# jneem/nnnoiseless

Hardware: AMD Instinct MI355X
Metric: 480-sample frames/sec (whole node) at N concurrent streams (higher is better)
Workload: dtype f32; 1 GPU; configs[2]: 65536 concurrent streams on one GPU, built-in weights.rnn, GRU as batched MFMA GEMM, synthetic 48 kHz sine+noise, 48 frame(s) per stream per step; parity=oracle pinned by the reference's golden pair (built-in model), model=built-in weights.rnn, boundary_format=f32 planar (process_frame's own), streams_per_gpu=65536, streams_total=65536, inputs_ready=True, schedule=stages, lanes=2, parallelism=streams sharded x1, one process per GPU, no data-path collective

## Files before the change

### include/nnn_batch.h

```cpp
#ifndef NNN_BATCH_H
#define NNN_BATCH_H

#include <stddef.h>
#include <stdint.h>

#ifdef __cplusplus
extern "C" {
#endif

typedef struct nnn_batch nnn_batch;
#ifndef RNNOISE_H
typedef struct RNNModel RNNModel;
#endif

#define NNN_FRAME_SIZE 480

RNNModel *nnn_model_from_bytes(const uint8_t *bytes, size_t len);
RNNModel *nnn_model_default(void);
long nnn_convert_rnnoise_text(const char *text, size_t len, uint8_t *out, size_t cap);
RNNModel *nnn_model_from_rnnoise_text(const char *text, size_t len);
void nnn_model_free(RNNModel *m);
RNNModel *nnn_model_clone(const RNNModel *m);
void nnn_model_shape(const RNNModel *m, int32_t shape[12]);

nnn_batch *nnn_batch_create(const RNNModel *model, int n_streams, int device);
nnn_batch *nnn_batch_create_grouped(const RNNModel *const *models, const int *group_streams, int n_groups, int device);
typedef struct nnn_batch_opts {
    int max_group_frames;
    int reserved[7];
} nnn_batch_opts;
nnn_batch *nnn_batch_create_opts(const RNNModel *const *models, const int *group_streams, int n_groups, int device,
                                 const nnn_batch_opts *opts);
int nnn_batch_max_group_frames(const nnn_batch *b);
size_t nnn_batch_device_bytes(const nnn_batch *b);
void nnn_batch_destroy(nnn_batch *b);
int nnn_batch_num_streams(const nnn_batch *b);
int nnn_batch_reset(nnn_batch *b);

nnn_batch *nnn_batch_clone(nnn_batch *b);
size_t nnn_batch_state_bytes(const nnn_batch *b);
int nnn_batch_save_state(nnn_batch *b, void *host_dst, size_t dst_bytes);
int nnn_batch_load_state(nnn_batch *b, const void *host_src, size_t src_bytes);

#define NNN_STREAM_STATE_BYTES 11232
#define NNN_STREAM_STATE_VERSION 1
#define NNN_STREAM_STATE_MAGIC 0x3153534Eu
#define NNN_STREAM_STATE_OFF_MAGIC 0
#define NNN_STREAM_STATE_OFF_VERSION 4
#define NNN_STREAM_STATE_OFF_SIZE 8
#define NNN_STREAM_STATE_OFF_GRU_SIZES 12
#define NNN_STREAM_STATE_OFF_MEM_ID 24
#define NNN_STREAM_STATE_OFF_LAST_PERIOD 28
#define NNN_STREAM_STATE_OFF_LAST_GAIN 32
#define NNN_STREAM_STATE_OFF_MEM_HP_X 36
#define NNN_STREAM_STATE_OFF_INPUT_MEM 64
#define NNN_STREAM_STATE_OFF_SYNTHESIS_MEM 6976
#define NNN_STREAM_STATE_OFF_CEPSTRAL_MEM 8896
#define NNN_STREAM_STATE_OFF_LASTG 9600
#define NNN_STREAM_STATE_OFF_VAD_GRU 9696
#define NNN_STREAM_STATE_OFF_NOISE_GRU 10208
#define NNN_STREAM_STATE_OFF_DENOISE_GRU 10720
int nnn_batch_reset_streams(nnn_batch *b, const int *streams, int n);
int nnn_batch_export_streams(nnn_batch *b, const int *streams, int n, void *host_dst, size_t dst_bytes);
int nnn_batch_import_streams(nnn_batch *b, const int *streams, int n, const void *host_src, size_t src_bytes);
int nnn_batch_export_streams_device(nnn_batch *b, const int *streams, int n, void *d_dst, void *hip_stream);
int nnn_batch_import_streams_device(nnn_batch *b, const int *streams, int n, const void *d_src, void *hip_stream);

int nnn_batch_hold_streams(nnn_batch *b, const int *streams, int n);
int nnn_batch_resume_streams(nnn_batch *b, const int *streams, int n);
int nnn_batch_num_held(const nnn_batch *b);
int nnn_batch_held_mask(const nnn_batch *b, uint8_t *held, size_t n);

int nnn_batch_set_gain_floor(nnn_batch *b, const int *streams, int n, const float *floors, int bands);
int nnn_batch_get_gain_floor(nnn_batch *b, const int *streams, int n, float *floors );
int nnn_batch_num_floored(const nnn_batch *b);

enum nnn_link_mode { NNN_LINK_OFF = 0, NNN_LINK_MAX = 1, NNN_LINK_MIN = 2 };
int nnn_batch_set_channel_link(nnn_batch *b, int channels, int mode);
int nnn_batch_get_channel_link(const nnn_batch *b, int *channels, int *mode);

int nnn_batch_process_device(nnn_batch *b, const float *d_in, float *d_out, float *d_vad, int n_frames,
                             size_t stream_stride, size_t frame_stride, void *hip_stream);
int nnn_batch_process_host(nnn_batch *b, const float *in, float *out, float *vad, int n_frames,
                           size_t stream_stride, size_t frame_stride);
void *nnn_host_alloc(size_t bytes);
void nnn_host_free(void *p);

enum nnn_pcm_format { NNN_PCM_F32 = 0, NNN_PCM_I16 = 1, NNN_PCM_F32_UNIT = 2 };
typedef struct nnn_pcm_layout {
    int format;
    int channels;
    int discard_first;
    int reserved;
    size_t group_stride;
    size_t frame_stride;
} nnn_pcm_layout;
int nnn_batch_process_pcm_device(nnn_batch *b, const void *d_in, void *d_out, float *d_vad, int n_frames,
                                 const nnn_pcm_layout *layout, void *hip_stream);
int nnn_batch_process_pcm_host(nnn_batch *b, const void *in, void *out, float *vad, int n_frames,
                               const nnn_pcm_layout *layout);
int nnn_batch_analyze_device(nnn_batch *b, const void *d_in, float *d_features, int32_t *d_silence, int n_frames,
                             const nnn_pcm_layout *layout, void *hip_stream);
int nnn_batch_synthesize_device(nnn_batch *b, const float *d_gains, const float *d_vad, void *d_out, int n_frames,
                                const nnn_pcm_layout *layout, void *hip_stream);
int nnn_batch_analyze_host(nnn_batch *b, const void *in, float *features, int32_t *silence, int n_frames, const nnn_pcm_layout *layout);
int nnn_batch_synthesize_host(nnn_batch *b, const float *gains, const float *vad, void *out, int n_frames, const nnn_pcm_layout *layout);
int nnn_batch_pending_frames(const nnn_batch *b);
int nnn_batch_vad_device(nnn_batch *b, const void *d_in, float *d_vad, int n_frames, const nnn_pcm_layout *layout, void *hip_stream);
int nnn_batch_vad_host(nnn_batch *b, const void *in, float *vad, int n_frames, const nnn_pcm_layout *layout);
int nnn_batch_network_device(nnn_batch *b, const float *d_features, const int32_t *d_silence, float *d_gains, float *d_vad, int n_frames,
                             void *hip_stream);
int nnn_batch_network_host(nnn_batch *b, const float *features, const int32_t *silence, float *gains, float *vad, int n_frames);
int nnn_batch_synchronize(nnn_batch *b);
int nnn_batch_fault(const nnn_batch *b);
int nnn_batch_debug_withhold_flag(nnn_batch *b, int frames_ahead);
int nnn_batch_debug_schedule(nnn_batch *b, int n_frames, int32_t *out, size_t cap);
int nnn_batch_debug_host_plan(nnn_batch *b, int n_frames, const nnn_pcm_layout *layout, int has_vad, int64_t out[8]);

enum nnn_tap {
    NNN_TAP_FILTERED = 0,
    NNN_TAP_XLP,
    NNN_TAP_AC,
    NNN_TAP_LPC2,
    NNN_TAP_XCORR1,
    NNN_TAP_BEST1,
    NNN_TAP_XCORR2C,
    NNN_TAP_PITCH_SEARCH,
    NNN_TAP_PITCH,
    NNN_TAP_PITCH_GAIN,
    NNN_TAP_X,
    NNN_TAP_P,
    NNN_TAP_EX, NNN_TAP_EP, NNN_TAP_EXP,
    NNN_TAP_FEATURES,
    NNN_TAP_SILENCE,
    NNN_TAP_G_RAW,
    NNN_TAP_G,
    NNN_TAP_VAD,
    NNN_TAP_BRANCH,
    NNN_TAP_COUNT
};
int nnn_tap_info(int tap, int *len, int *is_int);
int nnn_batch_set_taps(nnn_batch *b, int on);
int nnn_batch_read_tap(nnn_batch *b, int tap, void *host_dst, size_t dst_bytes);

#define NNN_FRAME_LOG_WORDS 24
int nnn_batch_set_frame_log(nnn_batch *b, void *d_log, size_t frames);

int nnn_batch_set_profiling(nnn_batch *b, int on);
int nnn_batch_num_kernels(void);
const char *nnn_batch_kernel_name(int k);
int nnn_batch_read_kernel_times(nnn_batch *b, double *total_ms, int64_t *launches, int n);

int nnn_batch_read_stamps(nnn_batch *b, long long *dst64);

int nnn_batch_set_graph(nnn_batch *b, int on);
int nnn_batch_set_pipeline(nnn_batch *b, int on);
int nnn_batch_set_inputs_ready(nnn_batch *b, int on);
int nnn_batch_set_back_end(nnn_batch *b, int mode);
int nnn_batch_set_schedule(nnn_batch *b, int mode, int lanes);

int nnn_debug_activations(int device, int act, const float *x, float *y, int n);

int nnn_device_local_cpulist(int device, char *buf, size_t cap);

const char *nnn_last_error(void);

#ifdef __cplusplus
}
#endif
#endif
```

### nnnoiseless_amd/__init__.py

```python
import ctypes as C
import os

import numpy as np


from . import _ffi
from .build import LIB_PATH, build_library

FRAME_SIZE = 480
FREQ_SIZE = 481
NB_BANDS = 22
NB_FEATURES = 42
from ._ffi import STREAM_STATE_BYTES, STREAM_STATE_VERSION, stream_state_field

_lib = None


def attenuation_limit_db(db):
    return 10.0 ** (-float(db) / 20.0)


def library():
    global _lib
    if _lib is None:
# ... 48 lines not shown

    from_static_bytes = from_bytes

    @classmethod
    def from_rnnoise_text(cls, text, lib=None):
        lib = lib or library()
        data = text.encode() if isinstance(text, str) else bytes(text)
        h = lib.L.nnn_model_from_rnnoise_text(data, len(data))
        return cls(h, lib) if h else None

    @classmethod
    def default(cls, lib=None):
        lib = lib or library()
        return cls(lib.L.nnn_model_default(), lib)

    def clone(self):
        h = self._lib.L.nnn_model_clone(self._h)
        if not h:
            raise RuntimeError(self._lib.error())
        return RnnModel(h, self._lib)

    __copy__ = clone

    def shape(self):
        s = (C.c_int32 * 12)()
        self._lib.L.nnn_model_shape(self._h, s)
        return list(s)

    def __del__(self):
        if getattr(self, "_h", None):
            self._lib.L.nnn_model_free(self._h)
            self._h = None


class BatchDenoiser:

    def __init__(self, n_streams, model=None, device=0, lib=None, groups=None, taps=False, max_group_frames=None, _handle=None):
        self._lib = lib or library()
        self._model = model
        self.n_streams = int(n_streams)
        self.frames_done = 0
        if _handle is not None:
            self._h = _handle
            return
        if max_group_frames is not None and int(max_group_frames) < 1:
            raise ValueError("max_group_frames must be at least 1")
        if groups or max_group_frames is not None:
            groups_ = groups or [(model, self.n_streams)]
            if sum(n for _, n in groups_) != self.n_streams:
                raise ValueError("group sizes must add up to n_streams")
            if groups:
                self._model = [m for m, _ in groups_]
            hs = (C.c_void_p * len(groups_))(*[m._h if m is not None else None for m, _ in groups_])
            ns = (C.c_int * len(groups_))(*[int(n) for _, n in groups_])
            if max_group_frames is not None:
                opts = _ffi.BatchOpts(max_group_frames=int(max_group_frames))
                self._h = self._lib.L.nnn_batch_create_opts(hs, ns, len(groups_), device, C.byref(opts))
            else:
                self._h = self._lib.L.nnn_batch_create_grouped(hs, ns, len(groups_), device)
        else:
            self._h = self._lib.L.nnn_batch_create(model._h if model is not None else None, self.n_streams, device)
        if not self._h:
            raise RuntimeError("nnnoiseless_amd: " + self._lib.error())
        if taps:
            self.set_taps(True)

    def device_bytes(self):
        return int(self._lib.L.nnn_batch_device_bytes(self._h))

    def max_group_frames(self):
        return int(self._lib.L.nnn_batch_max_group_frames(self._h))

    def clone(self):
        h = self._lib.L.nnn_batch_clone(self._h)
        if not h:
            raise RuntimeError("nnnoiseless_amd: " + self._lib.error())
        c = BatchDenoiser(self.n_streams, model=self._model, lib=self._lib, _handle=h)
        c.frames_done = self.frames_done
        return c

    def save_state(self):
        buf = np.empty(self._lib.L.nnn_batch_state_bytes(self._h), np.uint8)
        self._lib.check(self._lib.L.nnn_batch_save_state(self._h, _ffi.ptr(buf), buf.nbytes))
        return buf.tobytes()

    def load_state(self, data):
        buf = np.frombuffer(data, np.uint8)
        self._lib.check(self._lib.L.nnn_batch_load_state(self._h, _ffi.ptr(buf), buf.nbytes))

    def reset_streams(self, idx):
        a, p = _ffi.stream_list(idx)
        self._lib.check(self._lib.L.nnn_batch_reset_streams(self._h, p, a.size))

    def export_streams(self, idx):
        a, p = _ffi.stream_list(idx)
        out = np.zeros((a.size, STREAM_STATE_BYTES), np.uint8)
        self._lib.check(self._lib.L.nnn_batch_export_streams(self._h, p, a.size, _ffi.ptr(out), out.nbytes))
        return out

    def import_streams(self, idx, records):
        a, p = _ffi.stream_list(idx)
        r = _ffi.stream_records(records, a.size)
        self._lib.check(self._lib.L.nnn_batch_import_streams(self._h, p, a.size, _ffi.ptr(r), r.nbytes))

    def hold_streams(self, idx):
        a, p = _ffi.stream_list(idx)
        self._lib.check(self._lib.L.nnn_batch_hold_streams(self._h, p, a.size))

    def resume_streams(self, idx):
        a, p = _ffi.stream_list(idx)
        self._lib.check(self._lib.L.nnn_batch_resume_streams(self._h, p, a.size))

    def held(self):
        m = np.zeros(self.n_streams, np.uint8)
        self._lib.check(self._lib.L.nnn_batch_held_mask(self._h, _ffi.ptr(m), m.size))
        return m.astype(bool)

    def num_held(self):
        return int(self._lib.L.nnn_batch_num_held(self._h))

    def set_gain_floor(self, idx, floors):
        a, p = _ffi.stream_list(idx)
        f, bands = _ffi.gain_floors(floors, a.size)
        self._lib.check(self._lib.L.nnn_batch_set_gain_floor(self._h, p, a.size, f.ctypes.data_as(C.POINTER(C.c_float)), bands))

    def gain_floor(self, idx=None):
        a, p = _ffi.stream_list(range(self.n_streams) if idx is None else idx)
        out = np.zeros((a.size, NB_BANDS), np.float32)
        self._lib.check(self._lib.L.nnn_batch_get_gain_floor(self._h, p, a.size, out.ctypes.data_as(C.POINTER(C.c_float))))
        return out

    def num_floored(self):
        return int(self._lib.L.nnn_batch_num_floored(self._h))

    def set_channel_link(self, channels, mode="max"):
        self._lib.check(self._lib.L.nnn_batch_set_channel_link(self._h, int(channels), _ffi.link_mode(mode)))

    def channel_link(self):
        ch, md = C.c_int32(0), C.c_int32(0)
        self._lib.check(self._lib.L.nnn_batch_get_channel_link(self._h, C.byref(ch), C.byref(md)))
        return ch.value, _ffi.link_mode_name(md.value)

    def export_streams_device(self, idx, d_dst, hip_stream=0):
        a, p = _ffi.stream_list(idx)
        self._lib.check(self._lib.L.nnn_batch_export_streams_device(self._h, p, a.size, d_dst, hip_stream))

    def import_streams_device(self, idx, d_src, hip_stream=0):
        a, p = _ffi.stream_list(idx)
        self._lib.check(self._lib.L.nnn_batch_import_streams_device(self._h, p, a.size, d_src, hip_stream))

    def set_taps(self, on):
        self._lib.check(self._lib.L.nnn_batch_set_taps(self._h, int(on)))

    def set_schedule(self, mode, lanes=0):
        self._lib.check(self._lib.L.nnn_batch_set_schedule(self._h, {"seq": 0, "lanes": 1, "stages": 2}[mode], int(lanes)))

    def process(self, x, out=None, vad=None):
        x = _ffi.as_f32(x)
        if x.ndim != 3 or x.shape[0] != self.n_streams or x.shape[2] != FRAME_SIZE:
            raise ValueError(f"process needs x of shape [{self.n_streams}, n_frames, {FRAME_SIZE}], got {x.shape}")
        S, T, F = x.shape
        out = np.empty_like(x) if out is None else out
        vad = np.empty((T, S), np.float32) if vad is None else vad
        if not (isinstance(out, np.ndarray) and out.shape == x.shape and out.dtype == np.float32 and out.flags.c_contiguous and out.flags.writeable):
            raise ValueError("process: `out` must be a writable C-contiguous float32 array of x's shape")
        if not (isinstance(vad, np.ndarray) and vad.shape == (T, S) and vad.dtype == np.float32 and vad.flags.c_contiguous and vad.flags.writeable):
            raise ValueError("process: `vad` must be a writable C-contiguous float32 array of shape [n_frames, n_streams]")
        self._lib.check(self._lib.L.nnn_batch_process_host(self._h, _ffi.ptr(x), _ffi.ptr(out), _ffi.ptr(vad), T,
                                                           T * FRAME_SIZE, FRAME_SIZE))
        self.frames_done += T
        return out, vad

    def process_pcm(self, x, fmt, channels=1, discard_first=False, out=None, vad=None):
        x = np.ascontiguousarray(x, dtype=_ffi.PCM_DTYPE[fmt])
        if x.ndim != 3 or x.shape[2] != channels or x.shape[0] * channels != self.n_streams or x.shape[1] % FRAME_SIZE:
            raise ValueError(f"process_pcm needs x of shape [n_streams / channels, n_frames * {FRAME_SIZE}, channels], got {x.shape}")
        G, N, Cc = x.shape
        T = N // FRAME_SIZE
        out = np.zeros_like(x) if out is None else out
        vad = np.empty((T, self.n_streams), np.float32) if vad is None else vad
        if not (isinstance(out, np.ndarray) and out.shape == x.shape and out.dtype == x.dtype and out.flags.c_contiguous and out.flags.writeable):
            raise ValueError("process_pcm: `out` must be a writable C-contiguous array of x's shape and dtype")
        if not (isinstance(vad, np.ndarray) and vad.shape == (T, self.n_streams) and vad.dtype == np.float32 and vad.flags.c_contiguous and vad.flags.writeable):
            raise ValueError("process_pcm: `vad` must be a writable C-contiguous float32 array of shape [n_frames, n_streams]")
        L = _ffi.PcmLayout(fmt, channels, int(bool(discard_first)), 0, N * channels, FRAME_SIZE * channels)
        fresh = self.frames_done == 0
        self._lib.check(self._lib.L.nnn_batch_process_pcm_host(self._h, _ffi.ptr(x), _ffi.ptr(out), _ffi.ptr(vad), T, C.byref(L)))
        self.frames_done += T
        n_out = T - 1 if (discard_first and fresh) else T
        return out[:, :n_out * FRAME_SIZE], vad

    def process_device(self, d_in, d_out, d_vad, n_frames, stream_stride, frame_stride, hip_stream=0):
        self._lib.check(self._lib.L.nnn_batch_process_device(self._h, d_in, d_out, d_vad, n_frames, stream_stride,
                                                             frame_stride, hip_stream))
        self.frames_done += n_frames

    def process_pcm_device(self, d_in, d_out, d_vad, n_frames, fmt, channels, group_stride, frame_stride, discard_first=False,
                           hip_stream=0):
        L = _ffi.PcmLayout(fmt, channels, int(bool(discard_first)), 0, group_stride, frame_stride)
        self._lib.check(self._lib.L.nnn_batch_process_pcm_device(self._h, d_in, d_out, d_vad, n_frames, C.byref(L), hip_stream))
        self.frames_done += n_frames

    def _pcm_shape(self, what, x, fmt, channels):
        if fmt is None:
            x = _ffi.as_f32(x)
            if x.ndim != 3 or x.shape[0] != self.n_streams or x.shape[2] != FRAME_SIZE:
                raise ValueError(f"{what} needs audio of shape [{self.n_streams}, n_frames, {FRAME_SIZE}], got {x.shape}")
            return x, _ffi.PCM_F32, 1, x.shape[1], x.shape[1] * FRAME_SIZE
        x = np.ascontiguousarray(x, dtype=_ffi.PCM_DTYPE[fmt])
        if x.ndim != 3 or x.shape[2] != channels or x.shape[0] * channels != self.n_streams or x.shape[1] % FRAME_SIZE:
            raise ValueError(f"{what} needs audio of shape [n_streams / channels, n_frames * {FRAME_SIZE}, channels], got {x.shape}")
        return x, fmt, channels, x.shape[1] // FRAME_SIZE, x.shape[1] * channels

    def analyze(self, x, fmt=None, channels=1, features=None, silence=None):
        x, fmt, channels, T, gstride = self._pcm_shape("analyze", x, fmt, channels)
        S = self.n_streams
        features = np.zeros((T, S, NB_FEATURES), np.float32) if features is None else features
        silence = np.zeros((T, S), np.int32) if silence is None else silence
        for a, shp, dt, name in ((features, (T, S, NB_FEATURES), np.float32, "features"), (silence, (T, S), np.int32, "silence")):
            if not (isinstance(a, np.ndarray) and a.shape == shp and a.dtype == dt and a.flags.c_contiguous and a.flags.writeable):
                raise ValueError(f"analyze: `{name}` must be a writable C-contiguous {np.dtype(dt).name} array of shape {list(shp)}")
        L = _ffi.PcmLayout(fmt, channels, 0, 0, gstride, FRAME_SIZE * channels)
        self._lib.check(self._lib.L.nnn_batch_analyze_host(self._h, _ffi.ptr(x), _ffi.ptr(features), _ffi.ptr(silence), T, C.byref(L)))
        return features, silence

    def synthesize(self, gains, vad=None, fmt=None, channels=1, discard_first=False, out=None):
        gains = _ffi.as_f32(gains)
        S = self.n_streams
        if gains.ndim != 3 or gains.shape[1:] != (S, NB_BANDS):
            raise ValueError(f"synthesize needs gains of shape [n_frames, {S}, {NB_BANDS}], got {gains.shape}")
        T = gains.shape[0]
        if vad is not None:
            vad = _ffi.as_f32(vad)
            if vad.shape != (T, S):
                raise ValueError(f"synthesize: `vad` must have shape [{T}, {S}], got {vad.shape}")
        if fmt is None:
            fmt_, channels, shape, dt = _ffi.PCM_F32, 1, (S, T, FRAME_SIZE), np.float32
        else:
            if channels < 1 or S % channels:
                raise ValueError("n_streams must be a multiple of channels")
            fmt_, shape, dt = fmt, (S // channels, T * FRAME_SIZE, channels), _ffi.PCM_DTYPE[fmt]
        out = np.zeros(shape, dt) if out is None else out
        if not (isinstance(out, np.ndarray) and out.shape == shape and out.dtype == dt and out.flags.c_contiguous and out.flags.writeable):
            raise ValueError(f"synthesize: `out` must be a writable C-contiguous {np.dtype(dt).name} array of shape {list(shape)}")
        L = _ffi.PcmLayout(fmt_, channels, int(bool(discard_first)), 0, T * FRAME_SIZE * channels, FRAME_SIZE * channels)
        fresh = self.frames_done == 0
        self._lib.check(self._lib.L.nnn_batch_synthesize_host(self._h, _ffi.ptr(gains), _ffi.ptr(vad), _ffi.ptr(out), T, C.byref(L)))
        self.frames_done += T
        if fmt is None:
            return out
        return out[:, :(T - 1 if (discard_first and fresh) else T) * FRAME_SIZE]

    def analyze_device(self, d_in, d_features, d_silence, n_frames, fmt, channels, group_stride, frame_stride, hip_stream=0):
        L = _ffi.PcmLayout(fmt, channels, 0, 0, group_stride, frame_stride)
        self._lib.check(self._lib.L.nnn_batch_analyze_device(self._h, d_in, d_features, d_silence, n_frames, C.byref(L), hip_stream))

    def synthesize_device(self, d_gains, d_vad, d_out, n_frames, fmt, channels, group_stride, frame_stride, discard_first=False, hip_stream=0):
        L = _ffi.PcmLayout(fmt, channels, int(bool(discard_first)), 0, group_stride, frame_stride)
        self._lib.check(self._lib.L.nnn_batch_synthesize_device(self._h, d_gains, d_vad, d_out, n_frames, C.byref(L), hip_stream))
        self.frames_done += n_frames

    def pending_frames(self):
        return int(self._lib.L.nnn_batch_pending_frames(self._h))

    def vad(self, x, fmt=None, channels=1, vad=None):
        x, fmt, channels, T, gstride = self._pcm_shape("vad", x, fmt, channels)
        S = self.n_streams
        vad = np.zeros((T, S), np.float32) if vad is None else vad
        if not (isinstance(vad, np.ndarray) and vad.shape == (T, S) and vad.dtype == np.float32 and vad.flags.c_contiguous and vad.flags.writeable):
            raise ValueError(f"vad: `vad` must be a writable C-contiguous float32 array of shape [{T}, {S}]")
        L = _ffi.PcmLayout(fmt, channels, 0, 0, gstride, FRAME_SIZE * channels)
        self._lib.check(self._lib.L.nnn_batch_vad_host(self._h, _ffi.ptr(x), _ffi.ptr(vad), T, C.byref(L)))
        self.frames_done += T
        return vad

    def vad_device(self, d_in, d_vad, n_frames, fmt, channels, group_stride, frame_stride, hip_stream=0):
        L = _ffi.PcmLayout(fmt, channels, 0, 0, group_stride, frame_stride)
        self._lib.check(self._lib.L.nnn_batch_vad_device(self._h, d_in, d_vad, n_frames, C.byref(L), hip_stream))
        self.frames_done += n_frames

    def network(self, features, silence=None, gains=None, vad=None):
        features = _ffi.as_f32(features)
        S = self.n_streams
        if features.ndim != 3 or features.shape[0] < 1 or features.shape[1:] != (S, NB_FEATURES):
            raise ValueError(f"network needs features of shape [n_frames >= 1, {S}, {NB_FEATURES}], got {features.shape}")
        T = features.shape[0]
        if silence is not None:
            silence = np.ascontiguousarray(silence, dtype=np.int32)
            if silence.shape != (T, S):
                raise ValueError(f"network: `silence` must have shape [{T}, {S}], got {silence.shape}")
        gains = np.zeros((T, S, NB_BANDS), np.float32) if gains is None else gains
        vad = np.zeros((T, S), np.float32) if vad is None else vad
        for a, shp, name in ((gains, (T, S, NB_BANDS), "gains"), (vad, (T, S), "vad")):
            if not (isinstance(a, np.ndarray) and a.shape == shp and a.dtype == np.float32 and a.flags.c_contiguous and a.flags.writeable):
                raise ValueError(f"network: `{name}` must be a writable C-contiguous float32 array of shape {list(shp)}")
        self._lib.check(self._lib.L.nnn_batch_network_host(self._h, _ffi.ptr(features), _ffi.ptr(silence), _ffi.ptr(gains), _ffi.ptr(vad), T))
        return gains, vad

    def network_device(self, d_features, d_silence, d_gains, d_vad, n_frames, hip_stream=0):
        self._lib.check(self._lib.L.nnn_batch_network_device(self._h, d_features, d_silence, d_gains, d_vad, n_frames, hip_stream))

    def synchronize(self):
        self._lib.check(self._lib.L.nnn_batch_synchronize(self._h))

    def reset(self):
        self._lib.check(self._lib.L.nnn_batch_reset(self._h))
# ... 87 lines not shown
```

### nnnoiseless_amd/_ffi.py

```python
import ctypes as C
import os

import numpy as np

FRAME_SIZE = 480

TAPS = ["filtered", "xlp", "ac", "lpc2", "xcorr1", "best1", "xcorr2c", "pitch_search", "pitch", "pitch_gain",
        "X", "P", "ex", "ep", "exp", "features", "silence", "g_raw", "g", "vad", "branch"]

BATCH_SYMBOLS = [
    "nnn_model_from_bytes", "nnn_model_default", "nnn_model_free", "nnn_model_clone", "nnn_model_shape",
    "nnn_convert_rnnoise_text", "nnn_model_from_rnnoise_text",
    "nnn_batch_create", "nnn_batch_create_grouped", "nnn_batch_destroy", "nnn_batch_num_streams", "nnn_batch_reset",
    "nnn_batch_process_device", "nnn_batch_process_host", "nnn_batch_process_pcm_device", "nnn_batch_process_pcm_host",
    "nnn_batch_synchronize", "nnn_batch_clone", "nnn_batch_state_bytes", "nnn_batch_save_state", "nnn_batch_load_state",
    "nnn_batch_set_taps", "nnn_batch_set_schedule", "nnn_batch_set_inputs_ready", "nnn_debug_activations",
    "nnn_tap_info", "nnn_batch_read_tap", "nnn_batch_set_profiling", "nnn_batch_num_kernels",
    "nnn_batch_kernel_name", "nnn_batch_read_kernel_times", "nnn_batch_set_graph", "nnn_batch_set_pipeline", "nnn_batch_read_stamps",
    "nnn_host_alloc", "nnn_host_free", "nnn_last_error", "nnn_batch_fault", "nnn_batch_debug_withhold_flag", "nnn_batch_debug_schedule", "nnn_batch_debug_host_plan", "nnn_batch_set_frame_log",
    "nnn_batch_create_opts", "nnn_batch_max_group_frames", "nnn_batch_device_bytes", "nnn_batch_set_back_end", "nnn_device_local_cpulist",
    "nnn_batch_reset_streams", "nnn_batch_export_streams", "nnn_batch_import_streams", "nnn_batch_export_streams_device",
    "nnn_batch_import_streams_device", "nnn_batch_hold_streams", "nnn_batch_resume_streams", "nnn_batch_num_held", "nnn_batch_held_mask",
    "nnn_batch_analyze_device", "nnn_batch_synthesize_device", "nnn_batch_analyze_host", "nnn_batch_synthesize_host", "nnn_batch_pending_frames",
    "nnn_batch_vad_device", "nnn_batch_vad_host", "nnn_batch_network_device", "nnn_batch_network_host",
    "nnn_batch_set_gain_floor", "nnn_batch_get_gain_floor", "nnn_batch_num_floored",
    "nnn_batch_set_channel_link", "nnn_batch_get_channel_link",
]
TRAIN_SYMBOLS = [
    "nnn_train_create", "nnn_train_destroy", "nnn_train_reset", "nnn_train_process_device", "nnn_train_process_host",
]
RESAMPLE_SYMBOLS = [
    "nnn_resampler_create", "nnn_resampler_destroy", "nnn_resampler_reset", "nnn_resampler_max_output",
    "nnn_resampler_process_device", "nnn_resampler_process_host",
]
RATE_SYMBOLS = [
    "nnn_rate_create", "nnn_rate_destroy", "nnn_rate_reset", "nnn_rate_reset_streams", "nnn_rate_max_output", "nnn_rate_max_frames",
    "nnn_rate_carried", "nnn_rate_process_device", "nnn_rate_process_host", "nnn_rate_debug_tables",
]
PACK_SYMBOLS = [
    "nnn_pack_create", "nnn_pack_destroy", "nnn_pack_plan", "nnn_pack_run_device", "nnn_pack_run_host", "nnn_pack_last_summary",
    "nnn_pack_debug_kernels",
]
SIM_SYMBOLS = [
    "nnn_sim_create", "nnn_sim_destroy", "nnn_sim_load", "nnn_sim_adopt_device", "nnn_sim_set_params", "nnn_sim_get_params", "nnn_sim_reset",
    "nnn_sim_process_device", "nnn_sim_process_host", "nnn_sim_signals_device", "nnn_sim_signals_host", "nnn_sim_fault", "nnn_sim_debug_kernel",
]
FIT_SYMBOLS = [
    "nnn_fit_create", "nnn_fit_destroy", "nnn_fit_get", "nnn_fit_set", "nnn_fit_get_step", "nnn_fit_set_step", "nnn_fit_get_settings",
    "nnn_fit_set_settings", "nnn_fit_export_rnn", "nnn_fit_forward_device", "nnn_fit_loss_device", "nnn_fit_grad_device", "nnn_fit_step",
    "nnn_fit_losses", "nnn_fit_forward_host", "nnn_fit_loss_host", "nnn_fit_grad_host", "nnn_fit_debug_recurrence",
]
SCORE_SYMBOLS = [
    "nnn_score_create", "nnn_score_destroy", "nnn_score_set_delay", "nnn_score_get_delay", "nnn_score_reset", "nnn_score_accumulate_device",
    "nnn_score_accumulate_host", "nnn_score_totals", "nnn_score_totals_device",
]
SCORE_MAX_DELAY, SCORE_SUMS = 960, 4
GATE_SYMBOLS = [
    "nnn_gate_create", "nnn_gate_destroy", "nnn_gate_set_params", "nnn_gate_get_params", "nnn_gate_reset", "nnn_gate_apply_device",
    "nnn_gate_apply_pcm_device", "nnn_gate_apply_host", "nnn_gate_state_bytes", "nnn_gate_export_streams", "nnn_gate_import_streams",
]
GATE_MAX_LOOKBACK, GATE_MAX_GRACE, GATE_NEVER = 8, 6000, 0x7fffffff
GATE_STATE_BYTES, GATE_STATE_VERSION, GATE_STATE_MAGIC = 48 + 8 * 480 * 4, 1, 0x3147564E
GATE_PARAMS_DTYPE = np.dtype([("threshold", "<f4"), ("grace", "<i4"), ("lookback", "<i4"), ("level", "<f4")])
GATE_STATE_DTYPE = np.dtype([("magic", "<u4"), ("version", "<u4"), ("size", "<u4"), ("threshold", "<f4"), ("grace", "<i4"), ("lookback", "<i4"),
                             ("level", "<f4"), ("since", "<i4"), ("was_open", "<u4"), ("zero", "<u4", 3), ("history", "<f4", (8, 480))])
MIX_SYMBOLS = [
    "nnn_mix_create", "nnn_mix_destroy", "nnn_mix_set_rooms", "nnn_mix_get_rooms", "nnn_mix_set_gains", "nnn_mix_get_gains", "nnn_mix_reset",
    "nnn_mix_apply_device", "nnn_mix_apply_pcm_device", "nnn_mix_apply_host",
]
MIX_MAX_GAIN, MIX_TILE, MIX_REG_TALKERS = 16, 32, 8
PICK_SYMBOLS = [
    "nnn_pick_create", "nnn_pick_destroy", "nnn_pick_set_rooms", "nnn_pick_get_rooms", "nnn_pick_set_pinned", "nnn_pick_get_pinned",
    "nnn_pick_set_policy", "nnn_pick_get_policy", "nnn_pick_reset", "nnn_pick_select_device", "nnn_pick_select_pcm_device", "nnn_pick_select_host",
]
PICK_MAX_K, PICK_MAX_STICK, PICK_SEG_ROOM, PICK_WAVE_ROOM = 8, 16, 8, 64
FIT_PARAMS, FIT_RNN_BYTES, FIT_TILE = 87503, 87521, 4
FIT_SEL_PARAMS, FIT_SEL_GRAD, FIT_SEL_ADAM_M, FIT_SEL_ADAM_V = 0, 1, 2, 3
FIT_TENSORS = {
    "input_dense.W": (0, (42, 24)), "input_dense.b": (1008, (24,)),
    "vad_gru.W": (1032, (24, 72)), "vad_gru.U": (2760, (24, 72)), "vad_gru.b": (4488, (72,)),
    "noise_gru.W": (4560, (90, 144)), "noise_gru.U": (17520, (48, 144)), "noise_gru.b": (24432, (144,)),
    "denoise_gru.W": (24576, (114, 288)), "denoise_gru.U": (57408, (96, 288)), "denoise_gru.b": (85056, (288,)),
    "denoise_output.W": (85344, (96, 22)), "denoise_output.b": (87456, (22,)),
    "vad_output.W": (87478, (24, 1)), "vad_output.b": (87502, (1,)),
}
NODE_SYMBOLS = [
    "nnn_node_create", "nnn_node_destroy", "nnn_node_num_streams", "nnn_node_num_shards", "nnn_node_shard", "nnn_node_batch", "nnn_node_reset",
    "nnn_node_process_host", "nnn_node_process_pcm_host", "nnn_node_process_device", "nnn_node_process_device_streams", "nnn_node_synchronize",
    "nnn_node_fault", "nnn_node_shard_cpus", "nnn_node_reset_streams", "nnn_node_export_streams", "nnn_node_import_streams",
    "nnn_node_hold_streams", "nnn_node_resume_streams", "nnn_node_num_held",
    "nnn_node_set_gain_floor", "nnn_node_get_gain_floor", "nnn_node_num_floored",
    "nnn_node_set_channel_link", "nnn_node_get_channel_link",
]
RNNOISE_SYMBOLS = [
    "rnnoise_get_frame_size", "rnnoise_get_size", "rnnoise_init", "rnnoise_create", "rnnoise_destroy",
    "rnnoise_process_frame", "rnnoise_model_from_file", "rnnoise_model_free",
]


PCM_F32, PCM_I16, PCM_F32_UNIT = 0, 1, 2
PACK_I24, PACK_I32, PACK_F32_WAV = 16, 17, 18
PACK_ELEM_BYTES = {PCM_F32: 4, PCM_I16: 2, PACK_I24: 3, PACK_I32: 4, PACK_F32_WAV: 4}
LINK_OFF, LINK_MAX, LINK_MIN = 0, 1, 2
LINK_MODES = {"off": LINK_OFF, "max": LINK_MAX, "min": LINK_MIN}

STREAM_STATE_BYTES = 11232
STREAM_STATE_VERSION = 1
STREAM_STATE_MAGIC = 0x3153534E
STREAM_STATE_FIELDS = {
    "magic": (0, np.uint32, 1), "version": (4, np.uint32, 1), "size": (8, np.uint32, 1), "gru_sizes": (12, np.int32, 3),
    "mem_id": (24, np.int32, 1), "last_period": (28, np.int32, 1), "last_gain": (32, np.float32, 1), "mem_hp_x": (36, np.float32, 2),
    "input_mem": (64, np.float32, 1728), "synthesis_mem": (6976, np.float32, 480), "cepstral_mem": (8896, np.float32, 176),
    "lastg": (9600, np.float32, 22), "vad_gru": (9696, np.float32, 128), "noise_gru": (10208, np.float32, 128),
    "denoise_gru": (10720, np.float32, 128),
}


def stream_state_field(records, name):
    off, dt, cnt = STREAM_STATE_FIELDS[name]
    r = np.ascontiguousarray(records, dtype=np.uint8)
    a = r[..., off:off + cnt * np.dtype(dt).itemsize].view(dt)
    return a.reshape(r.shape[:-1] + (cnt,))
PCM_DTYPE = {PCM_F32: np.float32, PCM_I16: np.int16, PCM_F32_UNIT: np.float32}


class PcmLayout(C.Structure):
    _fields_ = [("format", C.c_int), ("channels", C.c_int), ("discard_first", C.c_int), ("reserved", C.c_int),
                ("group_stride", C.c_size_t), ("frame_stride", C.c_size_t)]


class PackFile(C.Structure):
    _fields_ = [("in_off", C.c_uint64), ("n_frames_samples", C.c_uint64), ("out_off", C.c_uint64), ("vad_off", C.c_uint64)]


class SimParams(C.Structure):
    _fields_ = [("signal_gain", C.c_float), ("noise_gain", C.c_float), ("sig_a", C.c_float * 2), ("sig_b", C.c_float * 2),
                ("noise_a", C.c_float * 2), ("noise_b", C.c_float * 2), ("band_lp", C.c_int32)]


SIM_PARAMS_DTYPE = np.dtype([("signal_gain", "<f4"), ("noise_gain", "<f4"), ("sig_a", "<f4", 2), ("sig_b", "<f4", 2),
                             ("noise_a", "<f4", 2), ("noise_b", "<f4", 2), ("band_lp", "<i4")])


class FitSettings(C.Structure):
    _fields_ = [("lr", C.c_float), ("beta1", C.c_float), ("beta2", C.c_float), ("epsilon", C.c_float), ("reg", C.c_float), ("clip", C.c_float)]


class FitRows(C.Structure):
    _fields_ = [("rows", C.c_void_p), ("frame_stride", C.c_size_t), ("seq_stride", C.c_size_t), ("w", C.c_void_p),
                ("w_frame_stride", C.c_size_t), ("w_seq_stride", C.c_size_t), ("n_seq", C.c_int), ("window", C.c_int)]


class BatchOpts(C.Structure):
    _fields_ = [("max_group_frames", C.c_int), ("reserved", C.c_int * 7)]


class Library:

    def __init__(self, path):
        if not os.path.exists(path):
            raise RuntimeError(
                f"nnnoiseless_amd: HIP library not found at {path}. Build it with "
                "`python -c 'import __graft_entry__ as g; g.build()'` (needs hipcc); there is no CPU fallback.")
        self.path = path
        L = self.L = C.CDLL(path)
        vp, sz, i32 = C.c_void_p, C.c_size_t, C.c_int
        L.nnn_model_from_bytes.restype = vp
        L.nnn_model_from_bytes.argtypes = [C.c_char_p, sz]
        L.nnn_model_default.restype = vp
        L.nnn_model_free.argtypes = [vp]
        L.nnn_model_clone.restype = vp
        L.nnn_model_clone.argtypes = [vp]
        L.nnn_model_shape.argtypes = [vp, C.POINTER(C.c_int32)]
        L.nnn_convert_rnnoise_text.restype = C.c_long
        L.nnn_convert_rnnoise_text.argtypes = [C.c_char_p, sz, vp, sz]
        L.nnn_model_from_rnnoise_text.restype = vp
        L.nnn_model_from_rnnoise_text.argtypes = [C.c_char_p, sz]
        L.nnn_batch_create_grouped.restype = vp
        L.nnn_batch_create_grouped.argtypes = [C.POINTER(vp), C.POINTER(i32), i32, i32]
        L.nnn_batch_create.restype = vp
        L.nnn_batch_create.argtypes = [vp, i32, i32]
        L.nnn_batch_destroy.argtypes = [vp]
        L.nnn_batch_num_streams.argtypes = [vp]
        L.nnn_batch_reset.argtypes = [vp]
        L.nnn_batch_process_device.argtypes = [vp, vp, vp, vp, i32, sz, sz, vp]
        L.nnn_batch_process_host.argtypes = [vp, vp, vp, vp, i32, sz, sz]
        L.nnn_batch_process_pcm_device.argtypes = [vp, vp, vp, vp, i32, C.POINTER(PcmLayout), vp]
        L.nnn_batch_process_pcm_host.argtypes = [vp, vp, vp, vp, i32, C.POINTER(PcmLayout)]
        L.nnn_batch_synchronize.argtypes = [vp]
        L.nnn_host_alloc.restype = vp
        L.nnn_host_alloc.argtypes = [sz]
        L.nnn_host_free.restype = None
        L.nnn_host_free.argtypes = [vp]
        L.nnn_tap_info.argtypes = [i32, C.POINTER(i32), C.POINTER(i32)]
        L.nnn_batch_read_tap.argtypes = [vp, i32, vp, sz]
        L.nnn_batch_set_profiling.argtypes = [vp, i32]
        L.nnn_batch_kernel_name.restype = C.c_char_p
        L.nnn_batch_kernel_name.argtypes = [i32]
        L.nnn_batch_read_kernel_times.argtypes = [vp, C.POINTER(C.c_double), C.POINTER(C.c_int64), i32]
        L.nnn_batch_set_graph.argtypes = [vp, i32]
        L.nnn_batch_clone.restype = vp
        L.nnn_batch_clone.argtypes = [vp]
        L.nnn_batch_state_bytes.restype = sz
        L.nnn_batch_state_bytes.argtypes = [vp]
        L.nnn_batch_save_state.argtypes = [vp, vp, sz]
        L.nnn_batch_load_state.argtypes = [vp, vp, sz]
        L.nnn_batch_set_taps.argtypes = [vp, i32]
        L.nnn_batch_set_schedule.argtypes = [vp, i32, i32]
        L.nnn_debug_activations.argtypes = [i32, i32, vp, vp, i32]
        L.nnn_batch_set_pipeline.argtypes = [vp, i32]
        L.nnn_batch_set_inputs_ready.argtypes = [vp, i32]
        for name, at in (("nnn_batch_set_frame_log", [vp, vp, sz]), ("nnn_batch_fault", [vp]), ("nnn_batch_debug_withhold_flag", [vp, i32]),
                         ("nnn_batch_debug_schedule", [vp, i32, C.POINTER(C.c_int32), sz]),
                         ("nnn_batch_debug_host_plan", [vp, i32, C.POINTER(PcmLayout), i32, C.POINTER(C.c_int64)]),
                         ("nnn_batch_create_opts", [C.POINTER(vp), C.POINTER(i32), i32, i32, C.POINTER(BatchOpts)]),
                         ("nnn_batch_max_group_frames", [vp]), ("nnn_batch_device_bytes", [vp]), ("nnn_batch_set_back_end", [vp, i32])):
            if hasattr(L, name):
                getattr(L, name).argtypes = at
        if hasattr(L, "nnn_batch_create_opts"):
            L.nnn_batch_create_opts.restype = vp
            L.nnn_batch_device_bytes.restype = sz
        if hasattr(L, "nnn_batch_reset_streams"):
            ip = C.POINTER(i32)
            L.nnn_batch_reset_streams.argtypes = [vp, ip, i32]
            L.nnn_batch_export_streams.argtypes = [vp, ip, i32, vp, sz]
            L.nnn_batch_import_streams.argtypes = [vp, ip, i32, vp, sz]
            L.nnn_batch_export_streams_device.argtypes = [vp, ip, i32, vp, vp]
            L.nnn_batch_import_streams_device.argtypes = [vp, ip, i32, vp, vp]
        if hasattr(L, "nnn_batch_hold_streams"):
            ip = C.POINTER(i32)
            L.nnn_batch_hold_streams.argtypes = [vp, ip, i32]
            L.nnn_batch_resume_streams.argtypes = [vp, ip, i32]
            L.nnn_batch_num_held.argtypes = [vp]
            L.nnn_batch_held_mask.argtypes = [vp, vp, sz]
        if hasattr(L, "nnn_batch_analyze_device"):
            lp = C.POINTER(PcmLayout)
            L.nnn_batch_analyze_device.argtypes = [vp, vp, vp, vp, i32, lp, vp]
            L.nnn_batch_synthesize_device.argtypes = [vp, vp, vp, vp, i32, lp, vp]
            L.nnn_batch_analyze_host.argtypes = [vp, vp, vp, vp, i32, lp]
            L.nnn_batch_synthesize_host.argtypes = [vp, vp, vp, vp, i32, lp]
            L.nnn_batch_pending_frames.argtypes = [vp]
        if hasattr(L, "nnn_batch_vad_device"):
            L.nnn_batch_vad_device.argtypes = [vp, vp, vp, i32, C.POINTER(PcmLayout), vp]
            L.nnn_batch_vad_host.argtypes = [vp, vp, vp, i32, C.POINTER(PcmLayout)]
        if hasattr(L, "nnn_batch_network_device"):
            L.nnn_batch_network_device.argtypes = [vp, vp, vp, vp, vp, i32, vp]
            L.nnn_batch_network_host.argtypes = [vp, vp, vp, vp, vp, i32]
        if hasattr(L, "nnn_batch_set_gain_floor"):
            ip, fp = C.POINTER(i32), C.POINTER(C.c_float)
            L.nnn_batch_set_gain_floor.argtypes = [vp, ip, i32, fp, i32]
            L.nnn_batch_get_gain_floor.argtypes = [vp, ip, i32, fp]
            L.nnn_batch_num_floored.argtypes = [vp]
        for name in ("nnn_batch_set_channel_link", "nnn_node_set_channel_link"):
            if hasattr(L, name):
                getattr(L, name).argtypes = [vp, i32, i32]
                getattr(L, name.replace("_set_", "_get_")).argtypes = [vp, C.POINTER(i32), C.POINTER(i32)]
        if hasattr(L, "nnn_node_set_gain_floor"):
            ip, fp = C.POINTER(i32), C.POINTER(C.c_float)
            L.nnn_node_set_gain_floor.argtypes = [vp, ip, i32, fp, i32]
            L.nnn_node_get_gain_floor.argtypes = [vp, ip, i32, fp]
            L.nnn_node_num_floored.argtypes = [vp]
        if hasattr(L, "nnn_node_hold_streams"):
            ip = C.POINTER(i32)
            L.nnn_node_hold_streams.argtypes = [vp, ip, i32]
            L.nnn_node_resume_streams.argtypes = [vp, ip, i32]
            L.nnn_node_num_held.argtypes = [vp]
        if hasattr(L, "nnn_node_reset_streams"):
            ip = C.POINTER(i32)
            L.nnn_node_reset_streams.argtypes = [vp, ip, i32]
            L.nnn_node_export_streams.argtypes = [vp, ip, i32, vp, sz]
            L.nnn_node_import_streams.argtypes = [vp, ip, i32, vp, sz]
        if hasattr(L, "nnn_node_create"):
            L.nnn_node_create.restype = vp
            L.nnn_node_create.argtypes = [vp, i32, C.POINTER(i32), i32, C.POINTER(BatchOpts)]
            L.nnn_node_destroy.argtypes = [vp]
            L.nnn_node_num_streams.argtypes = [vp]
            L.nnn_node_num_shards.argtypes = [vp]
            L.nnn_node_shard.argtypes = [vp, i32, C.POINTER(i32), C.POINTER(i32), C.POINTER(i32)]
            L.nnn_node_batch.restype = vp
            L.nnn_node_batch.argtypes = [vp, i32]
            L.nnn_node_reset.argtypes = [vp]
            L.nnn_node_process_host.argtypes = [vp, vp, vp, vp, i32, sz, sz]
            L.nnn_node_process_pcm_host.argtypes = [vp, vp, vp, vp, i32, C.POINTER(PcmLayout)]
            L.nnn_node_process_device.argtypes = [vp, C.POINTER(vp), C.POINTER(vp), C.POINTER(vp), i32, sz, sz]
            L.nnn_node_process_device_streams.argtypes = [vp, C.POINTER(vp), C.POINTER(vp), C.POINTER(vp), C.POINTER(vp), i32, i32, sz, sz]
            L.nnn_node_shard_cpus.restype = C.c_char_p
            L.nnn_node_shard_cpus.argtypes = [vp, i32]
            L.nnn_node_synchronize.argtypes = [vp]
            L.nnn_node_fault.argtypes = [vp]
        L.nnn_train_create.restype = vp
        L.nnn_train_create.argtypes = [i32, i32]
        L.nnn_train_destroy.argtypes = [vp]
        L.nnn_train_reset.argtypes = [vp]
        L.nnn_train_process_device.argtypes = [vp, vp, vp, vp, vp, vp, vp, i32, sz, sz, vp]
        L.nnn_train_process_host.argtypes = [vp, vp, vp, vp, vp, vp, vp, i32]
        L.nnn_resampler_create.restype = vp
        L.nnn_resampler_create.argtypes = [i32, C.c_double, i32]
        L.nnn_resampler_destroy.argtypes = [vp]
        L.nnn_resampler_reset.argtypes = [vp]
        L.nnn_resampler_max_output.restype = C.c_long
        L.nnn_resampler_max_output.argtypes = [vp, C.c_long]
        L.nnn_resampler_process_device.argtypes = [vp, vp, C.c_long, sz, vp, C.c_long, sz, C.POINTER(C.c_long), vp]
        L.nnn_resampler_process_host.argtypes = [vp, vp, C.c_long, vp, C.c_long, C.POINTER(C.c_long)]
        if hasattr(L, "nnn_rate_create"):
            lp = C.POINTER(C.c_long)
            L.nnn_rate_create.restype = vp
            L.nnn_rate_create.argtypes = [vp, C.c_double, C.c_long]
            L.nnn_rate_destroy.restype = None
            L.nnn_rate_destroy.argtypes = [vp]
            L.nnn_rate_reset.argtypes = [vp]
            L.nnn_rate_reset_streams.argtypes = [vp, C.POINTER(i32), i32]
            L.nnn_rate_max_output.restype = C.c_long
            L.nnn_rate_max_output.argtypes = [vp, C.c_long]
            L.nnn_rate_max_frames.argtypes = [vp, C.c_long]
            L.nnn_rate_carried.restype = C.c_long
            L.nnn_rate_carried.argtypes = [vp]
            L.nnn_rate_process_device.argtypes = [vp, vp, C.c_long, sz, vp, C.c_long, sz, lp, vp, i32, C.POINTER(i32), i32, vp]
            L.nnn_rate_process_host.argtypes = [vp, vp, C.c_long, vp, C.c_long, lp, vp, i32, C.POINTER(i32), i32]
            L.nnn_rate_debug_tables.argtypes = [vp, lp, C.POINTER(C.c_double)]
        if hasattr(L, "nnn_pack_create"):
            u64, fp_ = C.c_uint64, C.POINTER(PackFile)
            L.nnn_pack_create.restype = vp
            L.nnn_pack_create.argtypes = [vp, i32, i32]
            L.nnn_pack_destroy.restype = None
            L.nnn_pack_destroy.argtypes = [vp]
            L.nnn_pack_plan.argtypes = [i32, i32, C.POINTER(u64), i32, C.POINTER(C.c_int32), C.POINTER(C.c_int32), C.POINTER(C.c_int64)]
            L.nnn_pack_run_device.argtypes = [vp, vp, u64, i32, vp, u64, i32, vp, u64, fp_, i32, vp]
            L.nnn_pack_run_host.argtypes = [vp, vp, u64, i32, vp, u64, i32, vp, u64, fp_, i32]
            L.nnn_pack_last_summary.argtypes = [vp, C.POINTER(C.c_int64)]
            L.nnn_pack_debug_kernels.argtypes = [vp, i32, vp, i32, vp, i32, i32, i32, vp]
        if hasattr(L, "nnn_sim_create"):
            u64, ip = C.c_uint64, C.POINTER(i32)
            L.nnn_sim_create.restype = vp
            L.nnn_sim_create.argtypes = [vp]
            L.nnn_sim_destroy.restype = None
            L.nnn_sim_destroy.argtypes = [vp]
            L.nnn_sim_load.argtypes = [vp, i32, vp, u64]
            L.nnn_sim_adopt_device.argtypes = [vp, i32, vp, u64]
            L.nnn_sim_set_params.argtypes = [vp, ip, i32, vp]
            L.nnn_sim_get_params.argtypes = [vp, ip, i32, vp]
            L.nnn_sim_reset.argtypes = [vp]
            L.nnn_sim_process_device.argtypes = [vp, vp, vp, vp, i32, vp]
            L.nnn_sim_process_host.argtypes = [vp, vp, vp, vp, i32]
            L.nnn_sim_signals_device.argtypes = [vp, vp, vp, vp, vp, vp, vp, vp, i32, sz, sz, vp]
            L.nnn_sim_signals_host.argtypes = [vp, vp, vp, vp, vp, vp, vp, vp, i32]
            L.nnn_sim_fault.argtypes = [vp]
            L.nnn_sim_debug_kernel.argtypes = [vp, vp, vp, i32, i32, vp]
        if hasattr(L, "nnn_fit_create"):
            rp, fp = C.POINTER(FitRows), C.POINTER(C.c_float)
            L.nnn_fit_create.restype = vp
            L.nnn_fit_create.argtypes = [C.c_char_p, sz, i32, i32, i32]
            L.nnn_fit_destroy.restype = None
            L.nnn_fit_destroy.argtypes = [vp]
            L.nnn_fit_get.argtypes = [vp, i32, vp]
            L.nnn_fit_set.argtypes = [vp, i32, vp]
            L.nnn_fit_get_step.argtypes = [vp, C.POINTER(C.c_int64)]
            L.nnn_fit_set_step.argtypes = [vp, C.c_int64]
            L.nnn_fit_get_settings.argtypes = [vp, C.POINTER(FitSettings)]
            L.nnn_fit_set_settings.argtypes = [vp, C.POINTER(FitSettings)]
            L.nnn_fit_export_rnn.argtypes = [vp, vp, sz]
            L.nnn_fit_forward_device.argtypes = [vp, rp, vp, vp, vp]
            L.nnn_fit_loss_device.argtypes = [vp, rp, vp]
            L.nnn_fit_grad_device.argtypes = [vp, rp, vp]
            L.nnn_fit_step.argtypes = [vp, vp]
            L.nnn_fit_losses.argtypes = [vp, fp]
            L.nnn_fit_forward_host.argtypes = [vp, vp, i32, i32, vp, vp]
            L.nnn_fit_loss_host.argtypes = [vp, vp, vp, i32, i32]
            L.nnn_fit_grad_host.argtypes = [vp, vp, vp, i32, i32]
            L.nnn_fit_debug_recurrence.argtypes = [vp, i32, i32, i32, i32, i32, vp]
# ... 120 lines not shown
```

### nnnoiseless_amd/build.py

```python
import os
import subprocess

HERE = os.path.dirname(os.path.abspath(__file__))
CSRC = os.path.join(HERE, "csrc")
INCLUDE = os.path.join(os.path.dirname(HERE), "include")
LIB_DIR = os.path.join(HERE, "lib")
LIB_PATH = os.path.join(LIB_DIR, "libnnnoiseless_mi355x.so")
WEIGHTS = os.path.join(HERE, "data", "weights.rnn")
SOURCES = ["nnn_batch.hip", "nnn_resample.hip", "nnn_model.cpp", "rnnoise_capi.cpp", "nnn_node.cpp"]
HP_SOURCE = "nnn_hp.hip"


def _stale():
    if not os.path.exists(LIB_PATH):
        return True
    t = os.path.getmtime(LIB_PATH)
    deps = [os.path.join(d, f) for d in (CSRC, INCLUDE) for f in os.listdir(d) if f.endswith((".hip", ".h", ".hpp", ".cpp"))]
    deps += [WEIGHTS, os.path.abspath(__file__)]
    return any(os.path.getmtime(d) > t for d in deps)


def build_library(force=False, verbose=False):
    if not force and not _stale():
        return LIB_PATH
    os.makedirs(LIB_DIR, exist_ok=True)
    hipcc = os.environ.get("HIPCC", "/opt/rocm/bin/hipcc")
    common = [hipcc, "--offload-arch=gfx950", "-O3", "-std=c++17", "-ffp-contract=off", "-fPIC", "-Wno-unused-value", "-I", CSRC,
              f'-DNNN_WEIGHTS_PATH="{WEIGHTS}"']
    hp_obj = os.path.join(LIB_DIR, f"nnn_hp.{os.getpid()}.o")
    tmp_lib = os.path.join(LIB_DIR, f"libnnnoiseless_mi355x.{os.getpid()}.so")
    cmds = [common + ["-DNNN_HP_UNIT", "-Wno-pragma-once-outside-header", "-c", "-x", "hip", os.path.join(CSRC, HP_SOURCE), "-o", hp_obj],
            common + ["-fno-slp-vectorize", "-DNNN_HP_EXTERN", "-shared", "-x", "hip"] + [os.path.join(CSRC, s) for s in SOURCES]
            + ["-x", "none", hp_obj, "-o", tmp_lib]]
    try:
        for cmd in cmds:
            if verbose:
                print(" ".join(cmd))
            subprocess.check_call(cmd)
        os.replace(tmp_lib, LIB_PATH)
    finally:
        for f in (hp_obj, tmp_lib):
            if os.path.exists(f):
                os.remove(f)
    return LIB_PATH
```

### nnnoiseless_amd/csrc/nnn_batch_core.hip

```cpp
#pragma once

static thread_local std::string g_err;
static std::recursive_mutex g_rt_mu;
constexpr int MARK_DEVICES = 64;
static std::atomic<uint64_t> g_call_mark[MARK_DEVICES];
static std::atomic<uint64_t> g_next_batch_id{1};
#define NNN_RT_LOCK std::lock_guard<std::recursive_mutex> rt_lock_(g_rt_mu)
extern "C" const char *nnn_last_error(void) { return g_err.c_str(); }
extern "C" int nnn_device_local_cpulist(int device, char *buf, size_t cap)
{
    if (!buf || cap < 2) return 1;
    buf[0] = 0;
    char id[64] = {0};
    if (hipDeviceGetPCIBusId(id, (int)sizeof(id), device) != hipSuccess || !id[0]) return 1;
    for (char *p = id; *p; p++)
        if (*p >= 'A' && *p <= 'F') *p = (char)(*p - 'A' + 'a');
    char path[160];
    snprintf(path, sizeof(path), "/sys/bus/pci/devices/%s/local_cpulist", id);
    FILE *f = fopen(path, "r");
    if (!f) return 1;
    const bool ok = fgets(buf, (int)cap, f) != nullptr;
    fclose(f);
    if (!ok) { buf[0] = 0; return 1; }
    for (char *p = buf; *p; p++)
        if (*p == '\n' || *p == '\r') *p = 0;
    return buf[0] ? 0 : 1;
}
static int fail(const char *fmt, ...)
{
    char buf[512];
    va_list ap;
    va_start(ap, fmt);
    vsnprintf(buf, sizeof(buf), fmt, ap);
    va_end(ap);
    g_err = buf;
    return 1;
}
int nnn_set_error(const char *msg) { return fail("%s", msg); }
#define HIPCHK(expr)                                                                       \
    do {                                                                                   \
        hipError_t e_ = (expr);                                                            \
        if (e_ != hipSuccess) return fail("%s failed: %s", #expr, hipGetErrorString(e_));  \
    } while (0)


static const char *knob(const char *name) { return getenv(name); }
#ifdef NNN_DEV_KNOBS
static const char *dev_knob(const char *name) { return getenv(name); }
#else
static const char *dev_knob(const char *) { return nullptr; }
#endif

enum KernelId { K_HP, K_LPC, K_PITCH, K_FFT_XP, K_RNN, K_SYNTH, K_BACK, K_COUNT };
static const char *kKernelNames[K_COUNT] = {"k_hp", "k_lpc", "k_pitch", "k_fft_xp", "k_rnn", "k_synth", "k_back"};

enum Stage { ST_HP, ST_PITCH, ST_FFT, ST_RNN, ST_SYN, ST_COUNT };
enum SplitStage { ST_FEAT = ST_COUNT, ST_GAINS, ST_FFT_FEAT, ST_VAD };
struct SplitIo {
    float *features = nullptr;
    int *silence = nullptr;
    const float *gains = nullptr;
    const float *vad = nullptr;
};
constexpr int NSTREAMS = 5;
constexpr int EVR = 16;
enum SchedMode { SCHED_SEQ = 0, SCHED_LANES = 1, SCHED_STAGES = 2 };
constexpr int AUTO_BIG = 16384;
constexpr long long HANDOFF_TICKS = 10000ll * 100000ll;

struct Paths {
    int sched = SCHED_LANES;
    bool sched_auto = true;
    int n_lanes = 1;
    int host_chunk = -1;
    int wf_min_g = 0;
    int rnn_rows = 0;
    int hp_split = -1;
    int lpc_head = -1;
    int pitch_chain = 1;
    int hp_tpb = 0;
    int x_rides = -1;
    int lpc_wide = -1;
    int lpc_fc = 0;
    int back_mode = -1;
    bool use_pipeline = true;
    bool inputs_ready = false;
};
static Paths read_paths()
{
    Paths p;
    if (const char *e = knob("NNN_HOST_CHUNK")) p.host_chunk = atoi(e);
    if (const char *e = knob("NNN_RNN_WF_MIN_G")) p.wf_min_g = atoi(e);
    if (const char *e = knob("NNN_HP_SPLIT")) p.hp_split = atoi(e);
    if (const char *e = dev_knob("NNN_HP_TPB")) p.hp_tpb = atoi(e);
    if (const char *e = knob("NNN_LPC_HEAD")) p.lpc_head = atoi(e);
    if (const char *e = dev_knob("NNN_X_RIDES")) p.x_rides = atoi(e);
    if (const char *e = knob("NNN_PITCH_CHAIN")) p.pitch_chain = atoi(e);
    if (const char *e = dev_knob("NNN_LPC_WIDE")) p.lpc_wide = atoi(e);
    if (const char *e = dev_knob("NNN_LPC_FC")) p.lpc_fc = atoi(e);
    if (const char *e = knob("NNN_SCHED")) {
        if (!strcmp(e, "seq")) p.sched = SCHED_SEQ;
        else if (!strcmp(e, "lanes")) p.sched = SCHED_LANES;
        else if (!strcmp(e, "stages")) p.sched = SCHED_STAGES;
        p.sched_auto = false;
    }
    if (const char *e = knob("NNN_LANES")) {
        const int v = atoi(e);
        if (v >= 1 && v <= NSTREAMS - 1) p.n_lanes = v;
        p.sched_auto = false;
    }
    if (const char *e = knob("NNN_RNN_ROWS")) {
        const int v = atoi(e);
        if (v == 16 || v == 32) p.rnn_rows = v;
    }
    return p;
}

enum BackEnd { BACK_UNFUSED = 0, BACK_RNN_ALONE = 1, BACK_FUSED = 2 };
enum RnnKernel : uint8_t { RK_BACK, RK_WF_BUILTIN, RK_WF_ANY, RK_PLAIN };
struct GroupPlan {
    int g = 0;
    BackEnd back = BACK_UNFUSED;
    int hp = 0;
    bool held = false;
    bool floor = false;
    bool link = false;
    bool head = false;
    bool lpc_in_pitch = false;
    int lpc_fc = 0;
    bool chain = false;
    bool riders = false;
    uint8_t *rnn = nullptr;
};

enum MemKind : uint8_t { MEM_DEVICE, MEM_PINNED, MEM_MAPPED };
template <class T> struct GrowBuf {
    T *p = nullptr;
    size_t cap = 0;
    MemKind kind = MEM_DEVICE;
    int release()
    {
        if (p) HIPCHK(kind == MEM_DEVICE ? hipFree(p) : hipHostFree(p));
        p = nullptr, cap = 0;
        return 0;
    }
    hipError_t alloc(size_t n) { return kind == MEM_DEVICE ? hipMalloc((void **)&p, n) : hipHostMalloc((void **)&p, n, kind == MEM_MAPPED ? hipHostMallocMapped : 0); }
};

struct nnn_batch {
    Buffers b[NSET];
    ModelDims md;
    struct ModelGroup {
        RnnPlan plan;
        const uint4 *wq = nullptr;
        const float *fpar = nullptr;
        size_t rnn_lds = 0;
        bool wf = false;
        bool shape_builtin = false;
        WfPlan wp;
        size_t wf_lds = 0;
        int rows = 32;
        int tile0 = 0, ntiles = 0;
        size_t back_lds = 0, rnn16_lds = 0;
        BkActs acts = {};
        int vad_rows = 0, vad_mb = 0;
        size_t vad_lds = 0;
        int net_rows = 0;
        size_t net_lds = 0;
    };
    Paths paths;
    Paths created;
    GroupPlan plan;
    std::vector<ModelGroup> groups;
    std::vector<RNNModel> models;
    std::vector<int> group_streams;
    int device = 0;
    int S = 0, S_pad = 0, NT = 0;
    uint64_t frame_count = 0;
    int depth = 1;
    int gmax = GROUP;
    int nset = GROUP, nslot = slots_for(GROUP, 1);
    size_t device_bytes = 0;
    uint64_t group_count = 0;
    int last_set = 0;
    std::vector<void *> allocs;
    std::vector<std::pair<void *, size_t>> state_bufs;
    GrowBuf<char> stage;
    GrowBuf<float> stage_vad;
    std::vector<char> stage_host;
    GrowBuf<char> zc_host{nullptr, 0, MEM_MAPPED};
    char *zc_dev = nullptr;
    hipStream_t copy_in = nullptr, copy_out = nullptr;
    std::vector<hipEvent_t> ev_up, ev_run;
    GrowBuf<StepParams> sp_tab;
    hipStream_t stream = nullptr;
    hipStream_t pool[NSTREAMS] = {};
    hipEvent_t ev[2][ST_COUNT][EVR] = {};
    hipEvent_t ev_done[2] = {};
    bool have_done[2] = {false, false};
    bool prev_pipe = false;
    hipStream_t prev_st = nullptr;
    uint64_t prev_frame0 = 0;
    int prev_par = 0;
    std::vector<int> prev_first;
    volatile int *fault_host = nullptr;
    unsigned tickets = 0;
    unsigned *frame_log = nullptr;
    size_t frame_log_left = 0;
    uint64_t id = 0, other_seen_us = 0;
    bool beside_others = false;
    bool host_call = false;
    hipEvent_t ev_in = nullptr;
    hipEvent_t ev_last = nullptr;
    hipStream_t last_stream = nullptr;
    bool have_last = false;
    uint64_t call_count = 0;
    bool taps_alloc = false;
    bool profiling = false;
    std::vector<hipEvent_t> evp;
    std::vector<int> evp_kernel;
    double k_ms[K_COUNT] = {0};
    int64_t k_launches[K_COUNT] = {0};
    int *ss_dims = nullptr;
    int *ss_flag = nullptr;
    volatile int *ss_bad_host = nullptr;
    int *ss_bad_dev = nullptr;
    GrowBuf<int> ss_idx;
    GrowBuf<int> ss_idx_pin{nullptr, 0, MEM_PINNED};
    hipEvent_t ev_ss_idx = nullptr;
    bool ss_idx_busy = false;
    GrowBuf<char> ss_stage;
    unsigned *park = nullptr;
    unsigned long long *live = nullptr;
    std::vector<uint8_t> held;
    int n_held = 0;
    float *gfloor = nullptr;
    std::vector<float> gfloor_host;
    int n_floored = 0;
    GrowBuf<char> fl_stage;
    GrowBuf<char> fl_pin{nullptr, 0, MEM_PINNED};
    hipEvent_t ev_fl = nullptr;
    bool fl_busy = false;
    int link_ch = 1, link_mode = 0;
    int pending = 0, pending_set0 = 0, pending_slot = 0;
    GrowBuf<float> split_stage;
};

static int refuse_pending(const nnn_batch *h, const char *what)
{
    if (!h || !h->pending) return 0;
    return fail("%s refused: %d frames are pending (analysed by nnn_batch_analyze_* and not yet synthesised); "
                "nnn_batch_synthesize_* of the same n_frames comes first (nnn_batch_reset drops them)", what, h->pending);
}

extern "C" int nnn_batch_fault(const nnn_batch *h) { return h && h->fault_host && *h->fault_host ? 1 : 0; }
static int report_fault(const nnn_batch *h)
{
    if (!nnn_batch_fault(h)) return 0;
    return fail("a pitch workgroup gave up waiting for the previous frame's result (frame hand-off flag never set): the state of the "
                "affected streams is invalid from that frame on; nnn_batch_reset or nnn_batch_load_state clears the condition "
                "(NNN_PITCH_CHAIN=0 runs the frames of a group in a loop instead of side by side)");
}

static int quiesce(nnn_batch *h)
{
    HIPCHK(hipSetDevice(h->device));
    if (h->have_last) HIPCHK(hipEventSynchronize(h->ev_last));
    HIPCHK(hipStreamSynchronize(h->stream));
    for (int i = 0; i < NSTREAMS; i++)
        if (h->pool[i]) HIPCHK(hipStreamSynchronize(h->pool[i]));
    return 0;
}

template <class A, class B = char> static int grow(nnn_batch *h, bool drain, GrowBuf<A> &a, size_t a_bytes, size_t cap, GrowBuf<B> *b = nullptr, size_t b_bytes = 0)
{
    NNN_RT_LOCK;
    if (int rc = drain ? quiesce(h) : 0) return rc;
    if (int rc = a.release()) return rc;
    if (int rc = b ? b->release() : 0) return rc;
    HIPCHK(a.alloc(a_bytes));
    if (b) HIPCHK(b->alloc(b_bytes));
    a.cap = cap;
    if (b) b->cap = cap;
    return 0;
}

template <class T> static hipError_t dalloc(nnn_batch *h, T **p, size_t count, bool is_state)
{
    size_t bytes = count * sizeof(T);
    hipError_t e = hipMalloc((void **)p, bytes ? bytes : 4);
    if (e != hipSuccess) return e;
    h->allocs.push_back(*p);
    h->device_bytes += bytes ? bytes : 4;
    e = hipMemset(*p, 0, bytes);
    if (is_state) h->state_bufs.push_back({(void *)*p, bytes});
    return e;
}
template <class T> static hipError_t upload(nnn_batch *h, const T **p, const std::vector<T> &v)
{
    T *d = nullptr;
    hipError_t e = dalloc(h, &d, v.size(), false);
    if (e != hipSuccess) return e;
    *p = d;
    return hipMemcpy(d, v.data(), v.size() * sizeof(T), hipMemcpyHostToDevice);
}

extern "C" void *nnn_host_alloc(size_t bytes)
{
    void *p = nullptr;
    if (hipHostMalloc(&p, bytes ? bytes : 1, hipHostMallocDefault) != hipSuccess) {
        fail("nnn_host_alloc: %zu bytes of page-locked memory not available", bytes);
        return nullptr;
    }
    return p;
}
extern "C" void nnn_host_free(void *p)
{
    if (p) hipHostFree(p);
}
```

### nnnoiseless_amd/csrc/nnn_batch_create.hip

```cpp
#pragma once

static void make_tables(std::vector<float> &window, std::vector<float> &dct, std::vector<float2> &tw,
                        std::vector<float> &tansig, std::vector<float> &bin_frac, std::vector<int> &bin_band, float &wnorm)
{
    const double pi = 3.14159265358979323846;
    window.resize(WINDOW);
    for (int i = 0; i < FRAME; i++) {
        double s = sin(0.5 * pi * ((double)i + 0.5) / (double)FRAME);
        float w = (float)sin(0.5 * pi * s * s);
        window[i] = w;
        window[WINDOW - 1 - i] = w;
    }
    float acc = 0.0f;
    for (int i = 0; i < WINDOW; i++) acc += window[i] * window[i];
    wnorm = 1.0f / acc;
    dct.resize(NB * NB);
    for (int i = 0; i < NB; i++)
        for (int j = 0; j < NB; j++) {
            float v = (float)cos(((double)i + 0.5) * (double)j * pi / (double)NB);
            if (j == 0) v *= sqrtf(0.5f);
            dct[i * NB + j] = v;
        }
    tw.resize(WINDOW);
    for (int k = 0; k < WINDOW; k++) {
        tw[k].x = (float)cos(-2.0 * pi * k / (double)WINDOW);
        tw[k].y = (float)sin(-2.0 * pi * k / (double)WINDOW);
    }
    tansig.resize(201);
    for (int i = 0; i <= 200; i++) tansig[i] = (float)(floor(tanh(0.04 * (double)i) * 1e6 + 0.5) / 1e6);
    tansig[70] = 0.992631f;
    tansig[170] = 0.999997f;
    tansig[190] = 1.000000f;
    const int *E = kEbandHost;
    bin_frac.assign(400, 0.0f);
    bin_band.assign(400, 0);
    for (int i = 0; i < NB - 1; i++) {
        int band_size = (E[i + 1] - E[i]) << 2;
        for (int j = 0; j < band_size; j++) {
            bin_frac[(E[i] << 2) + j] = (float)j / (float)band_size;
            bin_band[(E[i] << 2) + j] = i;
        }
    }
}

extern "C" void nnn_batch_destroy(nnn_batch *h)
{
    if (!h) return;
    NNN_RT_LOCK;
    hipSetDevice(h->device);
    hipDeviceSynchronize();
    for (int p = 0; p < 2; p++) {
        for (int s = 0; s < ST_COUNT; s++)
            for (int i = 0; i < EVR; i++)
                if (h->ev[p][s][i]) hipEventDestroy(h->ev[p][s][i]);
        if (h->ev_done[p]) hipEventDestroy(h->ev_done[p]);
    }
    if (h->ev_in) hipEventDestroy(h->ev_in);
    if (h->ev_last) hipEventDestroy(h->ev_last);
    for (hipEvent_t e : h->evp) hipEventDestroy(e);
    for (void *p : h->allocs) hipFree(p);
    if (h->fault_host) hipHostFree((void *)h->fault_host);
    h->sp_tab.release();
    for (hipEvent_t e : h->ev_up) hipEventDestroy(e);
    for (hipEvent_t e : h->ev_run) hipEventDestroy(e);
    if (h->copy_in) hipStreamDestroy(h->copy_in);
    if (h->copy_out) hipStreamDestroy(h->copy_out);
    h->stage.release();
    h->stage_vad.release();
    h->split_stage.release();
    h->zc_host.release();
    if (h->ss_dims) hipFree(h->ss_dims);
    if (h->ss_flag) hipFree(h->ss_flag);
    if (h->ss_bad_host) hipHostFree((void *)h->ss_bad_host);
    h->ss_idx.release();
    h->ss_idx_pin.release();
    if (h->ev_ss_idx) hipEventDestroy(h->ev_ss_idx);
    h->ss_stage.release();
    h->fl_stage.release();
    h->fl_pin.release();
    if (h->ev_fl) hipEventDestroy(h->ev_fl);
    delete[] h->plan.rnn;
    for (int i = 0; i < NSTREAMS; i++)
        if (h->pool[i]) hipStreamDestroy(h->pool[i]);
    if (h->stream) hipStreamDestroy(h->stream);
    delete h;
}

constexpr size_t kLdsMax = 160 * 1024;
constexpr int RNN_SMALL_BATCH_BLOCKS = 128;

static nnn_batch::ModelGroup plan_model_group(const RnnPlan &pl, int ntiles, const Paths &paths)
{
    nnn_batch::ModelGroup G;
    G.plan = pl;
    G.ntiles = ntiles;
    G.rows = 0;
    for (int rows = 32; rows >= 16 && !G.rows; rows /= 2)
        if ((size_t)rnn_lds(G.plan, rows).total <= kLdsMax) G.rows = rows;
    if (!G.rows) return G;
    while (G.rows > 16 && G.ntiles * (TILE / G.rows) < RNN_SMALL_BATCH_BLOCKS) G.rows /= 2;
    if (paths.rnn_rows && (size_t)rnn_lds(G.plan, paths.rnn_rows).total <= kLdsMax) G.rows = paths.rnn_rows;
    G.rnn_lds = (size_t)rnn_lds(G.plan, G.rows).total;
    for (int half = 2; half >= 1 && !G.vad_rows; half--)
        for (int rows = TILE; rows >= 16 && !G.vad_rows; rows /= 2)
            if ((size_t)vad_lds(vad_plan_view(G.plan), rows).total <= kLdsMax / half && vad_gru_mb(G.plan, rows)) G.vad_rows = rows;
    if (G.vad_rows) {
        G.vad_mb = vad_gru_mb(G.plan, G.vad_rows);
        G.vad_lds = (size_t)vad_lds(vad_plan_view(G.plan), G.vad_rows).total;
    }
    G.net_rows = paths.rnn_rows && (size_t)net_lds(G.plan, paths.rnn_rows).total <= kLdsMax ? paths.rnn_rows : 16;
    G.net_lds = (size_t)net_lds(G.plan, G.net_rows).total;
    G.wp = wf_plan_of(G.plan);
    G.wf_lds = (size_t)wf_lds(G.wp).total;
    {
        constexpr RnnPlan cls = BkShapeBuiltin::plan();
        const bool shape_ok = pl.dense.n == cls.dense.n && pl.vad.n == cls.vad.n && pl.noise.n == cls.noise.n && pl.dn.n == cls.dn.n;
        G.shape_builtin = shape_ok;
        const size_t fb = (size_t)back_lds(G.plan, true).total, rb = (size_t)back_lds(G.plan, false).total;
        G.back_lds = shape_ok && fb <= kLdsMax ? fb : 0;
        G.rnn16_lds = shape_ok && rb <= kLdsMax ? rb : 0;
        G.acts = BkActs{G.plan.dense.act, G.plan.vad.act, G.plan.noise.act, G.plan.dn.act, G.plan.out.act, G.plan.act_vo};
    }
    G.wf = !paths.rnn_rows && G.plan.dense.nb <= 2 && G.plan.vad.nb <= 2 && G.plan.noise.nb <= 3 && G.plan.dn.nb <= 6 && G.plan.vad.rec.ksteps <= WF_KS_REC &&
           G.plan.noise.rec.ksteps <= WF_KS_REC && G.plan.dn.rec.ksteps <= WF_KS_REC && G.wf_lds <= kLdsMax;
    return G;
}

static int create_check_args(nnn_batch *h, const int *group_streams, int n_groups, int device, int gmax, int &n_streams)
{
    h->gmax = gmax < 1 ? 1 : (gmax > GROUP ? GROUP : gmax);
    n_streams = 0;
    for (int g = 0; g < n_groups; g++) {
        if (group_streams[g] <= 0) return fail("group %d: stream count must be positive", g);
        if (g + 1 < n_groups && group_streams[g] % TILE) return fail("group %d: every group but the last must be a multiple of %d streams", g, TILE);
        n_streams += group_streams[g];
    }
    int ndev = 0;
    HIPCHK(hipGetDeviceCount(&ndev));
    if (device < 0 || device >= ndev) return fail("no HIP device %d (found %d)", device, ndev);
    if (device >= MARK_DEVICES) return fail("device %d: the library keeps per-device call marks for devices 0 .. %d only", device, MARK_DEVICES - 1);
    HIPCHK(hipSetDevice(device));
    h->device = device;
    return 0;
}
static int create_streams_and_events(nnn_batch *h)
{
    HIPCHK(hipStreamCreateWithFlags(&h->stream, hipStreamNonBlocking));
    HIPCHK(hipEventCreateWithFlags(&h->ev_in, hipEventDisableTiming));
    HIPCHK(hipEventCreateWithFlags(&h->ev_last, hipEventDisableTiming));
    for (int p = 0; p < 2; p++) {
        for (int s = 0; s < ST_COUNT; s++)
            for (int i = 0; i < EVR; i++) HIPCHK(hipEventCreateWithFlags(&h->ev[p][s][i], hipEventDisableTiming));
        HIPCHK(hipEventCreateWithFlags(&h->ev_done[p], hipEventDisableTiming));
    }
    return 0;
}
static int create_model_groups(nnn_batch *h, const RNNModel *const *models, const int *group_streams, int n_groups, const Paths &paths,
                               std::vector<std::vector<uint16_t>> &wqs, std::vector<std::vector<float>> &fpars)
{
    wqs.resize(n_groups);
    fpars.resize(n_groups);
    h->groups.resize(n_groups);
    h->group_streams.assign(group_streams, group_streams + n_groups);
    memset(&h->md, 0, sizeof(h->md));
    for (int g = 0, tile0 = 0; g < n_groups; g++) {
        const RNNModel *model = models ? models[g] : nullptr;
        RNNModel *own = nullptr;
        if (!model) {
            size_t len;
            const uint8_t *w = nnn_builtin_weights(&len);
            own = nnn_model_parse(w, len);
            if (!own) return fail("built-in weights failed to parse");
            model = own;
        }
        h->models.push_back(*model);
        RnnPlan plan;
        ModelDims md;
        nnn_model_pack(*model, wqs[g], fpars[g], plan, md);
        delete own;
        nnn_batch::ModelGroup &G = h->groups[g];
        G = plan_model_group(plan, (group_streams[g] + TILE - 1) / TILE, paths);
        if (!G.rows) return fail("model too large for the RNN kernel's LDS operand matrices");
        G.tile0 = tile0;
        tile0 += G.ntiles;
        h->md.nd = md.nd > h->md.nd ? md.nd : h->md.nd;
        h->md.nv = md.nv > h->md.nv ? md.nv : h->md.nv;
        h->md.nn = md.nn > h->md.nn ? md.nn : h->md.nn;
        h->md.ndn = md.ndn > h->md.ndn ? md.ndn : h->md.ndn;
    }
    h->plan.rnn = new uint8_t[n_groups]();
    return 0;
}
static int create_state_arrays(nnn_batch *h)
{
    const size_t Sp = (size_t)h->S_pad;
    const ModelDims &md = h->md;
    Buffers &b = h->b[0];
    memset(&b, 0, sizeof(b));
    b.S = h->S; b.S_pad = h->S_pad; b.NT = h->NT;
    b.nslot = h->nslot;
    b.gru_v_w = md.nv; b.gru_n_w = md.nn; b.gru_dn_w = md.ndn;
    HIPCHK(dalloc(h, &b.hist, Sp * hist_stride(h->nslot), true));
    HIPCHK(dalloc(h, &b.hp_mem, Sp * 2, true));
    HIPCHK(dalloc(h, &b.hp_last, Sp, true));
    HIPCHK(dalloc(h, &b.dec, Sp * dec_len(h->nslot), true));
    HIPCHK(dalloc(h, &b.xlp0, Sp * h->nslot, true));
    HIPCHK(dalloc(h, &b.lpc_head, (size_t)h->NT * 5 * TILE, false));
    HIPCHK(dalloc(h, &b.lpc, Sp * h->nslot * 10, false));
    HIPCHK(dalloc(h, &b.ceps_mem, Sp * CEPS_MEM * NB, true));
    HIPCHK(dalloc(h, &b.mem_id, Sp, true));
    HIPCHK(dalloc(h, &b.synth_mem, Sp * FRAME, true));
    HIPCHK(dalloc(h, &b.lastg, Sp * NB, true));
    HIPCHK(dalloc(h, &b.last_period, Sp, true));
    HIPCHK(dalloc(h, &b.last_gain, Sp, true));
    HIPCHK(dalloc(h, &b.gru_v, Sp * md.nv, true));
    HIPCHK(dalloc(h, &b.gru_n, Sp * md.nn, true));
    HIPCHK(dalloc(h, &b.gru_dn, Sp * md.ndn, true));
    HIPCHK(dalloc(h, &b.stamps, 64, false));
    {
        void *hp = nullptr, *dp = nullptr;
        HIPCHK(hipHostMalloc(&hp, sizeof(int), hipHostMallocMapped));
        *(volatile int *)hp = 0;
        HIPCHK(hipHostGetDevicePointer(&dp, hp, 0));
        h->fault_host = (volatile int *)hp;
        b.fault = (int *)dp;
    }
    HIPCHK(dalloc(h, &b.ticket, 1, false));
    b.handoff_ticks = HANDOFF_TICKS;
    return grow(h, false, h->sp_tab, 2 * 64 * sizeof(StepParams), 64);
}
static int create_tables(nnn_batch *h, const std::vector<std::vector<uint16_t>> &wqs, const std::vector<std::vector<float>> &fpars)
{
    Buffers &b = h->b[0];
    std::vector<float> window, dct, tansig, bin_frac;
    std::vector<float2> tw;
    std::vector<int> bin_band;
    make_tables(window, dct, tw, tansig, bin_frac, bin_band, b.wnorm);
    HIPCHK(upload(h, &b.window, window));
    {
        std::vector<float> wa(WINDOW), ws(WINDOW);
        for (int i = 0; i < WINDOW; i++) { wa[i] = window[i] * 0.5f; ws[i] = window[i] * 0.5f; }
        HIPCHK(upload(h, &b.window_a, wa));
        HIPCHK(upload(h, &b.window_s, ws));
    }
    HIPCHK(upload(h, &b.dct, dct));
    HIPCHK(upload(h, &b.tw960, tw));
    HIPCHK(upload(h, &b.tansig, tansig));
    HIPCHK(upload(h, &b.bin_frac, bin_frac));
    HIPCHK(upload(h, &b.bin_band, bin_band));
    {
        const int *E = kEbandHost;
        std::vector<int> seg(192, 0);
        int ns = 0;
        for (int i = 0; i < NB - 1; i++) {
            int k = E[i] << 2, end = E[i + 1] << 2;
            const int need = (end - k + 7) / 8;
            if (need > 16) return fail("band interval too long for a row of lanes");
            if ((ns & 15) + need > 16) ns = (ns + 15) & ~15;
            seg[128 + i] = ns;
            while (k < end) {
                int c = end - k < 8 ? end - k : 8;
                if (ns >= 64) return fail("band segmentation overflow");
                seg[ns] = k;
                seg[64 + ns] = c;
                ns++;
                k += c;
            }
            seg[160 + i] = ns - seg[128 + i];
        }
        if (ns > 64) return fail("band segmentation overflow");
        HIPCHK(upload(h, &b.seg, seg));
        std::vector<FftLds> img(1);
        fft_tables_image(img[0], tw.data(), bin_frac.data(), bin_band.data(), seg.data(), dct.data());
        const FftLds *dimg = nullptr;
        HIPCHK(upload(h, &dimg, img));
        b.fft_img = dimg;
    }
    for (size_t g = 0; g < h->groups.size(); g++) {
        const uint16_t *dq = nullptr;
        HIPCHK(upload(h, &dq, wqs[g]));
        h->groups[g].wq = (const uint4 *)dq;
        HIPCHK(upload(h, &h->groups[g].fpar, fpars[g]));
    }
    return 0;
}
#define NNN_ALLOC_ONE(name, len) HIPCHK(dalloc(h, &h->b[0].name, (size_t)h->S_pad * (size_t)(len) * h->nset, false));
#define NNN_ALLOC_SETS(FIELDS)                                                              \
    do {                                                                                    \
        FIELDS(NNN_ALLOC_ONE)                                                               \
        for (int set = 1; set < h->nset; set++) h->b[set] = frame_view(h->b[0], set);       \
    } while (0)
static int create_scratch_sets(nnn_batch *h)
{
    NNN_ALLOC_SETS(NNN_WORK_FIELDS);
    h->state_bufs.push_back({(void *)h->b[0].pflag, (size_t)h->S_pad * h->nset * sizeof(int)});
// ... 123 lines not shown
```

### nnnoiseless_amd/csrc/nnn_batch_debug.hip

```cpp
#pragma once

struct TapDesc { int len; int is_int; int layout;  int sub_ofs; int sub_len; int needs_taps; };
static int last_slot(const nnn_batch *h) { return h ? (int)((h->frame_count + h->nslot - 1) % h->nslot) : 0; }
static bool tap_desc(const nnn_batch *h, int tap, TapDesc &d, const void **ptr)
{
    const Buffers *b = h ? &h->b[h->last_set] : nullptr;
#define TP(field) (b ? (const void *)b->field : nullptr)
    switch (tap) {
    case NNN_TAP_FILTERED: d = {FRAME, 0, 3, 0, FRAME, 0}; *ptr = TP(hist); return true;
    case NNN_TAP_XLP: d = {XLP, 0, 0, 0, XLP, 1}; *ptr = TP(xlp_ti); return true;
    case NNN_TAP_AC: d = {5, 0, 0, last_slot(h) * 10, (h ? h->nslot : 0) * 10, 0}; *ptr = TP(lpc); return true;
    case NNN_TAP_LPC2: d = {5, 0, 0, last_slot(h) * 10 + 5, (h ? h->nslot : 0) * 10, 0}; *ptr = TP(lpc); return true;
    case NNN_TAP_XCORR1: d = {NLAG1, 0, 0, 0, NLAG1, 1}; *ptr = TP(xc1); return true;
    case NNN_TAP_BEST1: d = {2, 1, 0, 0, 2, 1}; *ptr = TP(best1); return true;
    case NNN_TAP_XCORR2C: d = {10, 0, 0, 0, 10, 1}; *ptr = TP(xc2); return true;
    case NNN_TAP_PITCH_SEARCH: d = {1, 1, 0, 0, 1, 1}; *ptr = TP(psearch); return true;
    case NNN_TAP_PITCH: d = {1, 1, 0, 0, 1, 0}; *ptr = TP(pitch); return true;
    case NNN_TAP_PITCH_GAIN: d = {1, 0, 0, 0, 1, 0}; *ptr = TP(pgain); return true;
    case NNN_TAP_X: d = {2 * FREQ, 0, 2, 0, 2 * FREQ, 1}; *ptr = TP(X); return true;
    case NNN_TAP_P: d = {2 * FREQ, 0, 4, 0, 2 * FREQ, 1}; *ptr = TP(P); return true;
    case NNN_TAP_EX: d = {NB, 0, 0, 0, NB, 0}; *ptr = TP(ex); return true;
    case NNN_TAP_EP: d = {NB, 0, 0, 0, NB, 0}; *ptr = TP(ep); return true;
    case NNN_TAP_EXP: d = {NB, 0, 0, 0, NB, 0}; *ptr = TP(exp_); return true;
    case NNN_TAP_FEATURES: d = {NFEAT, 0, 0, 0, NFEAT, 1}; *ptr = TP(feat); return true;
// ... 41 lines not shown
    if (d.needs_taps && !h->b[0].taps) return fail("tap %d is only stored after nnn_batch_set_taps(batch, 1)", tap);
    if (dst_bytes < (size_t)h->S * d.len * 4) return fail("tap buffer too small");
    if (int rc = quiesce(h)) return rc;
    HIPCHK(hipDeviceSynchronize());
    uint32_t *dst = (uint32_t *)host_dst;
    const size_t Sp = (size_t)h->S_pad;
    if (d.layout == 0) {
        std::vector<uint32_t> tmp(Sp * d.sub_len);
        HIPCHK(hipMemcpy(tmp.data(), p, tmp.size() * 4, hipMemcpyDeviceToHost));
        for (int s = 0; s < h->S; s++)
            for (int i = 0; i < d.len; i++)
                dst[(size_t)s * d.len + i] = tmp[((size_t)(s / TILE) * d.sub_len + d.sub_ofs + i) * TILE + s % TILE];
    } else if (d.layout == 2 || d.layout == 4) {
        std::vector<uint32_t> tmp(Sp * 2 * FSTR);
        HIPCHK(hipMemcpy(tmp.data(), p, tmp.size() * 4, hipMemcpyDeviceToHost));
        for (int s = 0; s < h->S; s++)
            for (int k = 0; k < FREQ; k++) {
                const size_t at = (size_t)s * 2 * FSTR + 2 * (size_t)(d.layout == 4 ? spectrum_index_p(k) : spectrum_index(k));
                dst[(size_t)s * d.len + 2 * k] = tmp[at];
                dst[(size_t)s * d.len + 2 * k + 1] = tmp[at + 1];
            }
    } else {
        const size_t hstr = (size_t)hist_stride(h->nslot);
        std::vector<uint32_t> tmp(Sp * hstr);
        HIPCHK(hipMemcpy(tmp.data(), p, tmp.size() * 4, hipMemcpyDeviceToHost));
        int slot = last_slot(h);
        for (int s = 0; s < h->S; s++) memcpy(dst + (size_t)s * FRAME, tmp.data() + (size_t)s * hstr + slot * FRAME, FRAME * 4);
    }
    return 0;
}

extern "C" int nnn_batch_read_stamps(nnn_batch *h, long long *dst64)
{
    NNN_RT_LOCK;
    if (!h) return fail("null batch");
    HIPCHK(hipSetDevice(h->device));
    HIPCHK(hipDeviceSynchronize());
    HIPCHK(hipMemcpy(dst64, h->b[0].stamps, 64 * sizeof(long long), hipMemcpyDeviceToHost));
    return 0;
}

extern "C" int nnn_debug_activations(int device, int act, const float *x, float *y, int n)
{
    NNN_RT_LOCK;
    if (!x || !y || n < 0 || act < 0 || act > 2) return fail("bad argument");
    HIPCHK(hipSetDevice(device));
    std::vector<float> window, dct, tansig, bin_frac;
    std::vector<float2> tw;
    std::vector<int> bin_band;
    float wnorm;
    make_tables(window, dct, tw, tansig, bin_frac, bin_band, wnorm);
    float *d = nullptr;
    HIPCHK(hipMalloc((void **)&d, (size_t)(2 * n + 256) * sizeof(float)));
    float *dx = d + 256, *dy = dx + n;
    hipError_t e = hipMemcpy(d, tansig.data(), 201 * sizeof(float), hipMemcpyHostToDevice);
    if (e == hipSuccess) e = hipMemcpy(dx, x, (size_t)n * sizeof(float), hipMemcpyHostToDevice);
    if (e == hipSuccess && n) {
        hipLaunchKernelGGL(k_activation_kat, dim3((n + 255) / 256), dim3(256), 0, (hipStream_t) nullptr, (const float *)d, (const float *)dx, dy, act, n);
        e = hipDeviceSynchronize();
    }
    if (e == hipSuccess) e = hipMemcpy(y, dy, (size_t)n * sizeof(float), hipMemcpyDeviceToHost);
    hipFree(d);
    if (e != hipSuccess) return fail("activation sweep failed: %s", hipGetErrorString(e));
    return 0;
}

extern "C" int nnn_batch_set_profiling(nnn_batch *h, int on)
{
    if (!h) return fail("null batch");
    h->profiling = on != 0;
    return 0;
}
extern "C" int nnn_batch_num_kernels(void) { return K_COUNT; }
extern "C" const char *nnn_batch_kernel_name(int k) { return (k >= 0 && k < K_COUNT) ? kKernelNames[k] : ""; }
extern "C" int nnn_batch_read_kernel_times(nnn_batch *h, double *total_ms, int64_t *launches, int n)
{
    if (!h) return fail("null batch");
    for (int k = 0; k < n && k < K_COUNT; k++) {
        total_ms[k] = h->k_ms[k];
        launches[k] = h->k_launches[k];
        h->k_ms[k] = 0;
        h->k_launches[k] = 0;
    }
    return 0;
}
extern "C" int nnn_batch_set_graph(nnn_batch *h, int on)
{
    (void)on;
    if (!h) return fail("null batch");
    return 0;
}
extern "C" int nnn_batch_set_inputs_ready(nnn_batch *h, int on)
{
    if (!h) return fail("null batch");
    h->paths.inputs_ready = on != 0;
    return 0;
}
extern "C" int nnn_batch_set_frame_log(nnn_batch *h, void *d_log, size_t frames)
{
    if (!h) return fail("null batch");
    h->frame_log = (unsigned *)d_log;
    h->frame_log_left = d_log ? frames : 0;
    return 0;
}
extern "C" int nnn_batch_debug_withhold_flag(nnn_batch *h, int frames_ahead)
{
    if (!h) return fail("null batch");
    const int seq = frames_ahead < 0 ? 0 : (int)((h->frame_count + (uint64_t)frames_ahead) & 0x3fffffffu) + 1;
    for (int set = 0; set < h->nset; set++) {
        h->b[set].dbg_withhold = seq;
        h->b[set].handoff_ticks = seq ? 20000000ll : HANDOFF_TICKS;
    }
    return 0;
}
extern "C" int nnn_batch_debug_schedule(nnn_batch *h, int n_frames, int32_t *out, size_t cap)
{
    if (!h || !out) return fail("null argument");
    if (n_frames < 1) return fail("n_frames must be at least 1");
    CallPlan cp = plan_call(h, n_frames, h->stream);
    if ((size_t)n_frames > h->sp_tab.cap) cp.early_hp = false;
    const Schedule sc = plan_schedule(h, cp);
    constexpr size_t HEAD = 8, PER_NODE = 8 + 3 * MAX_WAITS;
    if (cap < HEAD + PER_NODE * sc.nodes.size()) return fail("schedule buffer too small: %zu entries needed", HEAD + PER_NODE * sc.nodes.size());
    const int32_t head[HEAD] = {(int32_t)sc.nodes.size(), (int32_t)cp.sizes.size(), cp.pipe, cp.sched, cp.lanes, sc.fill, sc.fill_after_done, sc.last_syn};
    memcpy(out, head, sizeof(head));
    out += HEAD;
    for (const Node &n : sc.nodes) {
        const int32_t v[8] = {n.stage, n.group, n.frames, n.first, n.stream, n.first_use, n.record, n.n_waits};
        memcpy(out, v, sizeof(v));
        for (int w = 0; w < MAX_WAITS; w++) {
            const Wait x = w < n.n_waits ? n.waits[w] : Wait{-1, -1, -1};
            out[8 + 3 * w] = x.origin, out[9 + 3 * w] = x.stage, out[10 + 3 * w] = x.group;
        }
        out += PER_NODE;
    }
    return 0;
}
extern "C" int nnn_batch_debug_host_plan(nnn_batch *h, int n_frames, const nnn_pcm_layout *L, int has_vad, int64_t out[8])
{
    if (!h || !out || n_frames < 1) return fail("null argument or no frames");
    if (int rc = check_layout(h, L)) return rc;
    const HostPlan p = plan_host_call(h, n_frames, *L, has_vad != 0);
    const int64_t v[8] = {p.route, p.chunk, p.n_chunks, (int64_t)p.span, (int64_t)p.vbytes, (int64_t)p.vofs, p.drop, p.vad_masked};
    memcpy(out, v, sizeof(v));
    return 0;
}
extern "C" int nnn_batch_set_back_end(nnn_batch *h, int mode)
{
    if (!h) return fail("null batch");
    if (mode < -1 || mode > 4) return fail("unknown back-end mode %d", mode);
    h->paths.back_mode = mode;
    return 0;
}
extern "C" int nnn_batch_set_pipeline(nnn_batch *h, int on)
{
    if (!h) return fail("null batch");
    h->paths.use_pipeline = on != 0;
    return 0;
}
extern "C" int nnn_batch_set_schedule(nnn_batch *h, int mode, int lanes)
{
    if (!h) return fail("null batch");
    if (mode < SCHED_SEQ || mode > SCHED_STAGES) return fail("unknown schedule %d", mode);
    h->paths.sched = mode;
    if (lanes >= 1 && lanes <= NSTREAMS - 1) h->paths.n_lanes = lanes;
    h->paths.sched_auto = false;
    return 0;
}
```

### nnnoiseless_amd/csrc/nnn_batch_launch.hip

```cpp
#pragma once

struct Launcher {
    nnn_batch *h;
    hipStream_t st;
    bool prof;
    template <class K, class... A> void go(int id, K kern, dim3 grid, dim3 block, size_t lds, A... args)
    {
        hipEvent_t e0 = nullptr, e1 = nullptr;
        if (prof) {
            hipEventCreate(&e0);
            hipEventCreate(&e1);
            hipEventRecord(e0, st);
        }
        hipLaunchKernelGGL(kern, grid, block, lds, st, args...);
        if (prof) {
            hipEventRecord(e1, st);
            h->evp.push_back(e0);
            h->evp.push_back(e1);
            h->evp_kernel.push_back(id);
        }
    }
};


static int lpc_launch(const nnn_batch *h, int g)
{
    const Paths &p = h->paths;
    const unsigned NT = (unsigned)h->NT, ug = (unsigned)g;
    if (p.lpc_wide >= 0 ? p.lpc_wide != 0 : NT * ug < 512u) return 0;
    int fc = LPC_FC;
    while (fc > 1 && NT * ((ug + fc - 1) / fc) < 2048u) fc /= 2;
    if (p.lpc_fc > 0) fc = p.lpc_fc < LPC_FC ? p.lpc_fc : LPC_FC;
    return fc;
}
static bool pitch_chained(const nnn_batch *h, int g)
{
    const int pc = h->paths.pitch_chain;
    return pc > 0 && g > 1 && (pc > 1 || (unsigned)h->S_pad / PK_SPB < 1024u);
}

static void plan_group(const nnn_batch *h, int g, GroupPlan &p)
{
    const Paths &k = h->paths;
    p.g = g;
    const int m = k.back_mode >= 0 ? k.back_mode : g > 1 ? 0 : ((h->S_pad <= 8192 && !h->beside_others) ? 1 : 3);
    const bool fused = m == 1 || m == 2, all_g = m == 2 || m == 4;
    p.back = m == 0 || (g > 1 && !all_g) ? BACK_UNFUSED : (fused ? BACK_FUSED : BACK_RNN_ALONE);
    for (const nnn_batch::ModelGroup &G : h->groups)
        if ((fused ? G.back_lds : G.rnn16_lds) == 0) p.back = BACK_UNFUSED;
    const bool split = k.hp_split >= 0 ? k.hp_split != 0 : h->NT <= 256;
    p.hp = !split ? 0 : ((k.hp_tpb ? k.hp_tpb == 2 : (g > 1 && h->NT >= 8)) ? 2 : 1);
    p.floor = h->n_floored > 0;
    p.link = h->link_ch > 1;
    p.held = h->n_held > 0;
    p.lpc_in_pitch = g == 1 && h->S_pad <= (split ? 8192 : 6144) && k.lpc_wide < 0 && k.lpc_fc == 0;
    p.head = p.lpc_in_pitch && split && k.lpc_head != 0;
    p.lpc_fc = p.lpc_in_pitch ? 0 : lpc_launch(h, g);
    p.chain = pitch_chained(h, g);
    p.riders = g == 1 && p.back == BACK_FUSED && (k.x_rides >= 0 ? k.x_rides != 0 : h->S_pad <= 8192);
    for (size_t i = 0; i < h->groups.size(); i++) {
        const nnn_batch::ModelGroup &G = h->groups[i];
        const int min_g = k.wf_min_g > 0 ? k.wf_min_g : ((G.ntiles * (TILE / WF_ROWS) >= 1024 || h->beside_others) ? 2 : 1);
        p.rnn[i] = p.back == BACK_RNN_ALONE ? RK_BACK : !(G.wf && g >= min_g) ? RK_PLAIN : G.shape_builtin ? RK_WF_BUILTIN : RK_WF_ANY;
    }
}

using RnnWfKernel = decltype(&k_rnn_wf<WfShapeAny>);
using BackKernel = decltype(&k_back<true, BkShapeBuiltin>);
using RnnPlainKernel = decltype(&k_rnn<false>);
static const RnnPlainKernel kRnnKernels[2] = {k_rnn<false>, k_rnn<true>};
static const auto kVadKernel = &k_vad;
static const auto kNetKernel = &k_net;
static const RnnWfKernel kRnnWfKernels[2] = {k_rnn_wf<WfShapeAny>, k_rnn_wf<BkShapeBuiltin>};
#define NNN_BK(F, XR, HELD, FLOOR) {k_back<F, BkShapeBuiltin, XR, HELD, FLOOR, false>, k_back<F, BkShapeBuiltin, XR, HELD, FLOOR, true>}
static const BackKernel kBackFused[2][2][2][2] = {
    {{NNN_BK(true, false, false, false), NNN_BK(true, false, false, true)}, {NNN_BK(true, false, true, false), NNN_BK(true, false, true, true)}},
    {{NNN_BK(true, true, false, false), NNN_BK(true, true, false, true)}, {NNN_BK(true, true, true, false), NNN_BK(true, true, true, true)}}};
static const BackKernel kBackRnnAlone[2][2][2] = {
    {NNN_BK(false, false, false, false), NNN_BK(false, false, false, true)},
    {NNN_BK(false, false, true, false), NNN_BK(false, false, true, true)}};
#undef NNN_BK
static std::vector<const void *> big_lds_kernels()
{
    std::vector<const void *> v;
    for (RnnPlainKernel k : kRnnKernels) v.push_back((const void *)k);
    for (RnnWfKernel k : kRnnWfKernels) v.push_back((const void *)k);
    for (const auto &by_held : kBackFused)
        for (const auto &by_floor : by_held)
            for (const auto &by_link : by_floor)
                for (BackKernel k : by_link) v.push_back((const void *)k);
    for (const auto &by_floor : kBackRnnAlone)
        for (const auto &by_link : by_floor)
            for (BackKernel k : by_link) v.push_back((const void *)k);
    v.push_back((const void *)kVadKernel);
    v.push_back((const void *)kNetKernel);
    return v;
}

static void launch_stage(nnn_batch *h, int s, int set0, const GroupPlan &p, const StepParams *sp0, hipStream_t st, bool prof, bool plain_out, const StepParams *call = nullptr, int fill = 0,
                         const SplitIo *io = nullptr)
{
    const int g = p.g;
    if (g <= 0) return;
    const unsigned NT = (unsigned)h->NT, Sp = (unsigned)h->S_pad, ug = (unsigned)g;
    const Buffers &b = h->b[set0];
    Launcher L{h, st, prof};
    switch (s) {
    case ST_HP:
        if (p.hp == 2)
            L.go(K_HP, p.held ? k_hp2<2, true> : k_hp2<2, false>, dim3((NT + 1) / 2 + (p.head ? (5 * NT + 3) / 4 : 0)), dim3(256), 0, b, sp0, g, call ? *call : StepParams{}, call ? fill : 0, p.head ? 1 : 0);
        else if (p.hp == 1)
            L.go(K_HP, p.held ? k_hp2<1, true> : k_hp2<1, false>, dim3(NT + (p.head ? (5 * NT + 1) / 2 : 0)), dim3(128), 0, b, sp0, g, call ? *call : StepParams{}, call ? fill : 0, p.head ? 1 : 0);
        else L.go(K_HP, p.held ? k_hp<true> : k_hp<false>, dim3(NT), dim3(64), 0, b, sp0, g, call ? *call : StepParams{}, call ? fill : 0);
        if (p.lpc_in_pitch) break;
        if (!p.lpc_fc) L.go(K_LPC, k_lpc_wide, dim3(NT * ug), dim3(320), 0, b, sp0, g);
        else L.go(K_LPC, k_lpc, dim3(NT * ((ug + p.lpc_fc - 1) / p.lpc_fc)), dim3(64), 0, b, sp0, g, p.lpc_fc);
        break;
    case ST_PITCH: {
        const int chain = p.chain ? 1 : 0, seq0 = (int)(h->frame_count & 0x3fffffffu) + 1;
        const unsigned grid = Sp / PK_SPB * (chain ? ug : 1u);
        if (p.lpc_in_pitch)
            L.go(K_PITCH, p.held ? k_pitch<true, true> : k_pitch<true, false>, dim3(grid + (p.riders ? Sp / 8 : 0u)), dim3(PK_T), 0, b, sp0, g, chain, seq0, h->tickets, p.head ? 2 : 1, p.riders ? (int)grid : 0);
        else
            L.go(K_PITCH, p.held ? k_pitch<false, true> : k_pitch<false, false>, dim3(grid + (p.riders ? Sp / 8 : 0u)), dim3(PK_T), 0, b, sp0, g, chain, seq0, h->tickets, 0, p.riders ? (int)grid : 0);
        if (chain) h->tickets += grid;
        break;
    }
    case ST_FFT:
        if (p.back == BACK_FUSED) {
            for (const nnn_batch::ModelGroup &G : h->groups)
                L.go(K_BACK, kBackFused[p.riders][p.held][p.floor][p.link], dim3((unsigned)(G.ntiles * (TILE / BK_ROWS))), dim3(BK_T), G.back_lds, b, sp0, G.acts, G.wq, G.fpar, G.tile0, g);
            break;
        }
        L.go(K_FFT_XP, k_fft_xp, dim3(Sp * ug / FFT_SPB), dim3(64 * FFT_SPB), 0, b, sp0, g);
        break;
    case ST_RNN:
        if (p.back == BACK_FUSED) break;
        for (size_t i = 0; i < h->groups.size(); i++) {
            const nnn_batch::ModelGroup &G = h->groups[i];
            if (p.rnn[i] == RK_BACK)
                L.go(K_RNN, kBackRnnAlone[p.held][p.floor][p.link], dim3((unsigned)(G.ntiles * (TILE / BK_ROWS))), dim3(BK_T), G.rnn16_lds, b, sp0, G.acts, G.wq, G.fpar, G.tile0, g);
            else if (p.rnn[i] == RK_WF_BUILTIN || p.rnn[i] == RK_WF_ANY)
                L.go(K_RNN, kRnnWfKernels[p.rnn[i] == RK_WF_BUILTIN], dim3((unsigned)(G.ntiles * (TILE / WF_ROWS))), dim3(64 * WF_WAVES), G.wf_lds, b, G.plan, G.wp,
                     G.wq, G.fpar, G.tile0, g);
            else
                L.go(K_RNN, kRnnKernels[p.link], dim3((unsigned)(G.ntiles * (TILE / G.rows))), dim3(64 * RNN_WAVES), G.rnn_lds, b, G.plan, G.wq, G.fpar,
                     G.tile0, G.rows, g);
        }
        break;
    case ST_SYN:
        if (p.back == BACK_FUSED) break;
        if (plain_out) L.go(K_SYNTH, k_synth<true>, dim3(Sp / FFT_SPB), dim3(64 * FFT_SPB), 0, b, sp0, g);
        else L.go(K_SYNTH, k_synth<false>, dim3(Sp / FFT_SPB), dim3(64 * FFT_SPB), 0, b, sp0, g);
        break;
    case ST_FEAT:
        hipLaunchKernelGGL(k_features, dim3(NT), dim3(64 * FEAT_WAVES), 0, st, b, g);
        hipLaunchKernelGGL(k_features_out, dim3(NT * ug), dim3(FOUT_T), 0, st, b, io->features, io->silence, g);
        break;
    case ST_GAINS:
        hipLaunchKernelGGL(k_gains_in, dim3(NT), dim3(GIN_T), 0, st, b, io->gains, io->vad, g);
        break;
    case ST_FFT_FEAT:
        if (b.taps) hipLaunchKernelGGL(k_fft_xp, dim3(Sp * ug / FFT_SPB), dim3(64 * FFT_SPB), 0, st, b, sp0, g);
        else hipLaunchKernelGGL(k_fft_feat, dim3(Sp * ug / FFT_SPB), dim3(64 * FFT_SPB), 0, st, b, sp0, g);
        break;
    case ST_VAD:
        hipLaunchKernelGGL(k_features, dim3(NT), dim3(64 * FEAT_WAVES), 0, st, b, g);
        for (const nnn_batch::ModelGroup &G : h->groups)
            hipLaunchKernelGGL(kVadKernel, dim3((unsigned)(G.ntiles * (TILE / G.vad_rows))), dim3(64 * RNN_WAVES), G.vad_lds, st, b, sp0, G.plan, G.wq,
                               G.fpar, G.tile0, G.vad_rows, G.vad_mb, g);
        break;
    }
}

static int drain_profile(nnn_batch *h)
{
    for (size_t i = 0; i < h->evp_kernel.size(); i++) {
        float ms = 0.0f;
        HIPCHK(hipEventSynchronize(h->evp[2 * i + 1]));
        HIPCHK(hipEventElapsedTime(&ms, h->evp[2 * i], h->evp[2 * i + 1]));
        h->k_ms[h->evp_kernel[i]] += ms;
        h->k_launches[h->evp_kernel[i]] += 1;
        hipEventDestroy(h->evp[2 * i]);
        hipEventDestroy(h->evp[2 * i + 1]);
    }
    h->evp.clear();
    h->evp_kernel.clear();
    return 0;
}

struct CallPlan {
    std::vector<int> sizes;
    bool pipe;
    int sched, lanes;
    bool fold_fill, early_hp, hp_after;
    bool idle;
};
static CallPlan plan_call(const nnn_batch *h, int n_frames, hipStream_t st)
{
    const Paths &k = h->paths;
    CallPlan c;
    constexpr int PIPE_MIN = 32;
    const bool auto_big = k.sched_auto && h->S_pad > AUTO_BIG;
    c.idle = h->n_held == h->S;
    c.pipe = !c.idle && k.use_pipeline && k.sched != SCHED_SEQ && !h->profiling && n_frames >= PIPE_MIN && !(auto_big && h->depth < 2);
    if (c.pipe) {
        int n = 2;
        while ((n_frames + n - 1) / n > h->gmax) n += 2;
        if (n > n_frames) n = n_frames;
        for (int i = 0; i < n; i++) c.sizes.push_back(n_frames / n + (i < n_frames % n ? 1 : 0));
    } else {
        for (int rem = n_frames; rem > 0; rem -= c.sizes.back()) c.sizes.push_back(rem < h->gmax ? rem : h->gmax);
    }
    c.sched = auto_big ? (c.sizes.size() <= 2 ? SCHED_STAGES : SCHED_LANES) : k.sched;
    c.lanes = auto_big ? 2 : k.n_lanes;
    c.fold_fill = (!c.pipe && !h->profiling) || c.idle;
    c.early_hp = c.pipe && k.inputs_ready && !h->host_call && h->prev_pipe && h->prev_st == st && c.sched == SCHED_LANES && h->pool[0];
    c.hp_after = c.sched == SCHED_LANES && c.lanes == 1 && h->S_pad >= 8192;
    return c;
}

constexpr int MAX_WAITS = 1 + 1 + 1;
static_assert(MAX_WAITS >= 1 + 1, "hp: the pitch kernel before it (hp_after) and the ring edge; rnn, synth: previous stage and previous group; fft_xp: previous stage");
enum WaitOrigin { W_THIS = 0, W_PREV = 1, W_DONE = 2 };
enum FillWhere { FILL_FOLDED = 0, FILL_CALLER = 1, FILL_POOL0 = 2 };
struct Wait { int origin, stage, group; };
struct Node {
    int stage, group, frames, first;
    int stream;
    bool first_use;
    bool record;
    bool fill;
    int n_waits;
    Wait waits[MAX_WAITS];
};
struct Schedule {
    std::vector<Node> nodes;
    int fill = FILL_FOLDED;
    bool fill_after_done = false;
    int last_syn = -1;
};

static Schedule plan_schedule(const nnn_batch *h, const CallPlan &cp)
{
    Schedule sc;
    const int n_groups = (int)cp.sizes.size(), par = (int)((h->call_count + 1) & 1);
    sc.fill = cp.early_hp ? FILL_POOL0 : (cp.fold_fill ? FILL_FOLDED : FILL_CALLER);
    sc.fill_after_done = cp.early_hp && h->have_done[par];
    if (cp.idle) return sc;
    auto stream_of = [&](int s, int k) -> int {
        if (!cp.pipe) return -1;
        if (cp.sched == SCHED_STAGES) return s == ST_HP ? 0 : (s == ST_PITCH ? 1 : (s == ST_FFT ? 2 : (s == ST_RNN ? 3 : -1)));
        return s == ST_HP ? 0 : (k % cp.lanes) - (k % cp.lanes == 0 ? 1 : 0);
    };
    auto consumers_elsewhere = [&](int s, int k) {
        const int me = stream_of(s, k);
        if (s + 1 < ST_COUNT && stream_of(s + 1, k) != me) return true;
        if ((s == ST_HP || s == ST_PITCH || s == ST_RNN || s == ST_SYN) && k + 1 < n_groups && stream_of(s, k + 1) != me) return true;
        if (s == ST_SYN) return true;
        if (cp.hp_after && s == ST_PITCH) return true;
        return false;
    };
    bool used[NSTREAMS] = {cp.early_hp};
    const int pn = (int)h->prev_first.size();
    sc.nodes.reserve((size_t)n_groups * ST_COUNT);
    for (int k = 0, t = 0; k < n_groups; t += cp.sizes[k++]) {
        const int g = cp.sizes[k];
        for (int s = 0; s < ST_COUNT; s++) {
            Node n = {};
            const int si = stream_of(s, k);
            n.stage = s, n.group = k, n.frames = g, n.first = t, n.stream = si;
            n.first_use = si >= 0 && !used[si];
            if (si >= 0) used[si] = true;
            n.fill = cp.fold_fill && k == 0 && s == ST_HP;
            n.record = cp.pipe && consumers_elsewhere(s, k);
            auto wait = [&](int origin, int ds, int dk) { n.waits[n.n_waits++] = Wait{origin, ds, dk}; };
            auto wait_for = [&](int ds, int dk) {
                if (dk < 0 || dk < k - EVR + 1) return;
                if (stream_of(ds, dk) != si) wait(W_THIS, ds, dk);
            };
            if (s > 0) wait_for(s - 1, k);
            if (s == ST_HP || s == ST_PITCH || s == ST_RNN || s == ST_SYN) wait_for(s, k - 1);
            if (s == ST_PITCH) wait_for(ST_SYN, k - h->depth);
            if (s == ST_HP && cp.hp_after) {
                if (k > 0) wait_for(ST_PITCH, k - 1);
                else if (cp.early_hp && pn > 0) wait(W_PREV, ST_PITCH, pn - 1);
            }
            if (s == ST_HP && cp.pipe) {
                const int need = t + g - 1 + 3 - h->nslot;
                int dk = -1;
                for (int j = 0; j < k; j++)
                    if (sc.nodes[(size_t)j * ST_COUNT].first <= need) dk = j;
                wait_for(ST_SYN, dk);
                if (cp.early_hp && need < 0) {
                    const long long pf = (long long)h->frame_count + need - (long long)h->prev_frame0;
                    int pj = -1;
                    for (int j = 0; j < pn; j++)
                        if (h->prev_first[j] <= pf) pj = j;
                    if (pf >= 0 && pj >= 0 && pn - pj < EVR) wait(W_PREV, ST_SYN, pj);
                    else if (h->have_done[par]) wait(W_DONE, 0, 0);
                }
            }
            sc.nodes.push_back(n);
        }
    }
    if (stream_of(ST_SYN, n_groups - 1) >= 0) sc.last_syn = n_groups - 1;
    return sc;
}
static hipEvent_t wait_event(const nnn_batch *h, int par, const Wait &w)
{
    return w.origin == W_DONE ? h->ev_done[par] : h->ev[w.origin == W_PREV ? h->prev_par : par][w.stage][w.group % EVR];
}

static int process_frames(nnn_batch *h, const void *d_in, void *d_out, float *d_vad, int n_frames, int fmt, int channels,
                          long long group_stride, long long frame_stride, int drop, void *hip_stream)
{
    HIPCHK(hipSetDevice(h->device));
    if (int rc = report_fault(h)) return rc;
    const bool plain_out = fmt == PCM_F32 && channels == 1;
    {
        const uint64_t mask = (1ull << 44) - 1;
        const uint64_t now = (uint64_t)std::chrono::duration_cast<std::chrono::microseconds>(std::chrono::steady_clock::now().time_since_epoch()).count() & mask;
        const uint64_t prev = g_call_mark[h->device].exchange((h->id << 44) | now, std::memory_order_relaxed);
        if ((prev >> 44) != h->id && (prev >> 44) != 0 && now - (prev & mask) < 5000) h->other_seen_us = now | (1ull << 63);
        h->beside_others = (h->other_seen_us >> 63) && now - (h->other_seen_us & mask) < 20000;
        if (h->beside_others) {
            static std::atomic<bool> told{false};
            if (!getenv("GPU_MAX_HW_QUEUES") && !told.exchange(true))
                fprintf(stderr, "nnnoiseless_mi355x: several batches are being driven side by side on device %d and GPU_MAX_HW_QUEUES is not set; "
                                "the HIP runtime then maps their streams onto 4 hardware queues and they largely serialise "
                                "(export GPU_MAX_HW_QUEUES=8 before the process starts -- INTEGRATION.md; any value of the variable silences this note)\n", h->device);
        }
    }
    hipError_t e;
    hipStream_t st = call_begin(h, hip_stream, e);
    if (e != hipSuccess) return fail("hipStreamWaitEvent(st, h->ev_last, 0) failed: %s", hipGetErrorString(e));
    StepParams v0;
    v0.in = (const char *)d_in;
    v0.out = (char *)d_out;
    v0.vad = d_vad;
    v0.group_stride = group_stride;
    v0.frame_stride = frame_stride;
    v0.fmt = fmt;
    v0.channels = channels;
    v0.discard = drop;
    v0.slot = (int)(h->frame_count % h->nslot);
    v0.n_streams = h->S;
    v0.log = h->frame_log_left ? h->frame_log : nullptr;
    v0.log_frames = (int)(h->frame_log_left < (size_t)n_frames ? h->frame_log_left : (size_t)n_frames);
    if (v0.log) {
        h->frame_log += (size_t)v0.log_frames * h->S * FRAME_LOG_WORDS;
        h->frame_log_left -= (size_t)v0.log_frames;
    }
    if ((size_t)n_frames > h->sp_tab.cap) {
        const size_t cap = n_frames < 64 ? 64 : (size_t)n_frames;
        if (int rc = grow(h, true, h->sp_tab, 2 * cap * sizeof(StepParams), cap)) return rc;
        h->prev_pipe = false;
    }
    const CallPlan cp = plan_call(h, n_frames, st);
    const Schedule sc = plan_schedule(h, cp);
    const int n_groups = (int)cp.sizes.size();
    h->call_count += 1;
    const int par = (int)(h->call_count & 1);
    StepParams *const tab = h->sp_tab.p + (size_t)par * h->sp_tab.cap;
    const uint64_t frame0 = h->frame_count;
    bool ok = true;
    if (sc.fill != FILL_FOLDED) {
        hipStream_t fs = sc.fill == FILL_POOL0 ? h->pool[0] : st;
        if (sc.fill_after_done) ok &= hipStreamWaitEvent(fs, h->ev_done[par], 0) == hipSuccess;
        hipLaunchKernelGGL(k_fill_params, dim3((n_frames + 63) / 64), dim3(64), 0, fs, tab, v0, n_frames, h->nslot);
    }
    if (cp.pipe) ok &= hipEventRecord(h->ev_in, st) == hipSuccess;
    size_t i = 0;
    for (int k = 0; k < n_groups; k++) {
        const int g = cp.sizes[k], set0 = (int)(h->group_count % h->depth) * h->gmax;
        plan_group(h, g, h->plan);
        for (; i < sc.nodes.size() && sc.nodes[i].group == k; i++) {
            const Node &n = sc.nodes[i];
            if (n.stream >= 0 && !h->pool[n.stream]) ok &= hipStreamCreateWithFlags(&h->pool[n.stream], hipStreamNonBlocking) == hipSuccess;
            hipStream_t ss = n.stream < 0 ? st : h->pool[n.stream];
            if (n.first_use) ok &= hipStreamWaitEvent(ss, h->ev_in, 0) == hipSuccess;
            for (int w = 0; w < n.n_waits; w++) ok &= hipStreamWaitEvent(ss, wait_event(h, par, n.waits[w]), 0) == hipSuccess;
            launch_stage(h, n.stage, set0, h->plan, tab + n.first, ss, h->profiling, plain_out, n.fill ? &v0 : nullptr, n_frames);
            if (n.record) ok &= hipEventRecord(h->ev[par][n.stage][k % EVR], ss) == hipSuccess;
        }
        h->group_count += 1;
        h->frame_count += g;
        h->last_set = set0 + g - 1;
    }
    if (sc.last_syn >= 0) ok &= hipStreamWaitEvent(st, h->ev[par][ST_SYN][sc.last_syn % EVR], 0) == hipSuccess;
    h->prev_pipe = cp.pipe;
    if (cp.pipe) {
        h->prev_st = st;
        h->prev_frame0 = frame0;
        h->prev_par = par;
        h->prev_first.clear();
        for (int k = 0; k < n_groups; k++) h->prev_first.push_back(sc.nodes[(size_t)k * ST_COUNT].first);
    }
    ok &= hipEventRecord(h->ev_done[par], st) == hipSuccess;
    h->have_done[par] = true;
    ok &= call_end(h, st) == hipSuccess;
    if (!ok) return fail("stream/event call failed while enqueueing frames: %s", hipGetErrorString(hipGetLastError()));
    HIPCHK(hipGetLastError());
    if (h->profiling) {
        HIPCHK(hipStreamSynchronize(st));
        return drain_profile(h);
    }
    return 0;
}

static int check_layout(const nnn_batch *h, const nnn_pcm_layout *L)
{
    if (!L) return fail("null layout");
    if (L->format != NNN_PCM_F32 && L->format != NNN_PCM_I16 && L->format != NNN_PCM_F32_UNIT) return fail("unknown sample format %d", L->format);
    if (L->channels < 1 || h->S % L->channels) return fail("n_streams (%d) is not a multiple of channels (%d)", h->S, L->channels);
    if (L->frame_stride < (size_t)FRAME * L->channels) return fail("frame_stride smaller than one frame of all channels");
    return 0;
}

extern "C" int nnn_batch_process_device(nnn_batch *h, const float *d_in, float *d_out, float *d_vad, int n_frames,
                                        size_t stream_stride, size_t frame_stride, void *hip_stream)
{
    if (!h) return fail("null batch");
    if (int rc = refuse_pending(h, "nnn_batch_process_device")) return rc;
    if (n_frames <= 0) return 0;
    if (!d_in || !d_out) return fail("null buffer");
    if (n_frames > 1 && frame_stride < (size_t)FRAME) return fail("frame_stride smaller than one frame");
    return process_frames(h, d_in, d_out, d_vad, n_frames, PCM_F32, 1, (long long)stream_stride * 4, (long long)frame_stride * 4, 0,
                          hip_stream);
}

extern "C" int nnn_batch_process_pcm_device(nnn_batch *h, const void *d_in, void *d_out, float *d_vad, int n_frames,
                                            const nnn_pcm_layout *L, void *hip_stream)
{
    if (!h) return fail("null batch");
    if (int rc = refuse_pending(h, "nnn_batch_process_pcm_device")) return rc;
    if (n_frames <= 0) return 0;
    if (!d_in || !d_out) return fail("null buffer");
    if (int rc = check_layout(h, L)) return rc;
    const long long e = pcm_elem_bytes(L->format);
    const int drop = (L->discard_first && h->frame_count == 0) ? 1 : 0;
    return process_frames(h, d_in, d_out, d_vad, n_frames, L->format, L->channels, (long long)L->group_stride * e,
                          (long long)L->frame_stride * e, drop, hip_stream);
}
```

### nnnoiseless_amd/csrc/nnn_fft.hip

```cpp
#pragma once

namespace nnn {

constexpr int NFFT = 480;

__device__ __forceinline__ float2 cmulf(float2 a, float2 w)
{
    return make_float2(fmaf(a.x, w.x, -a.y * w.y), fmaf(a.x, w.y, a.y * w.x));
}
__device__ __forceinline__ float2 cadd(float2 a, float2 c) { return make_float2(a.x + c.x, a.y + c.y); }
__device__ __forceinline__ float2 csub(float2 a, float2 c) { return make_float2(a.x - c.x, a.y - c.y); }
__device__ __forceinline__ float2 mul_mi(float2 a) { return make_float2(a.y, -a.x); }

__device__ __forceinline__ void bfly2(float2 &a, float2 &c) { float2 t = csub(a, c); a = cadd(a, c); c = t; }

__device__ __forceinline__ void dft8(float2 *v)
{
    const float h = 0.70710678118654752440f;
    float2 a0 = v[0], a1 = v[1], a2 = v[2], a3 = v[3], a4 = v[4], a5 = v[5], a6 = v[6], a7 = v[7];
    bfly2(a0, a4); bfly2(a1, a5); bfly2(a2, a6); bfly2(a3, a7);
    a5 = make_float2((a5.x + a5.y) * h, (a5.y - a5.x) * h);
    a6 = mul_mi(a6);
    a7 = make_float2((a7.y - a7.x) * h, (-a7.x - a7.y) * h);
    bfly2(a0, a2); bfly2(a1, a3); bfly2(a4, a6); bfly2(a5, a7);
// ... 197 lines not shown
{
    const int e_lo = bnd >= 1 ? kEband[bnd - 1] : 0, e_mid = kEband[bnd], e_hi = bnd < NB - 1 ? kEband[bnd + 1] : 0;
    float acc = 0.0f;
    if (bnd >= 1)
        for (int k = 4 * e_lo; k < 4 * e_mid; k++) acc += bin_frac[k] * v[k];
    if (bnd < NB - 1)
        for (int k = 4 * e_mid; k < 4 * e_hi; k++) acc += (1.0f - bin_frac[k]) * v[k];
    if (bnd == 0 || bnd == NB - 1) acc *= 2.0f;
    return acc;
}

template <int NQ>
__device__ __forceinline__ void band_sums_par(const FftLds &t, const float *const (&v)[NQ], float (&out)[NQ], int lane)
{
    const short *seg = t.seg;
    const int k0 = seg[lane], cnt = seg[64 + lane], rem = seg[192 + lane];
    const int ks0 = bsk(k0);
    float pa[NQ], pb[NQ];
#pragma unroll
    for (int q = 0; q < NQ; q++) { pa[q] = 0.0f; pb[q] = 0.0f; }
#pragma unroll
    for (int u = 0; u < 8; u++) {
        const float fr = t.frac[ks0 + u], om = 1.0f - fr;
#pragma unroll
        for (int q = 0; q < NQ; q++) {
            float x = v[q][ks0 + u];
            x = u < cnt ? x : 0.0f;
            pa[q] = fmaf(om, x, pa[q]);
            pb[q] = fmaf(fr, x, pb[q]);
        }
    }
#define NNN_SUFFIX_ROUND(D)                                                          \
    _Pragma("unroll") for (int q = 0; q < NQ; q++) {                                 \
        const float ta = dpp_row_down<D>(pa[q]), tb = dpp_row_down<D>(pb[q]);        \
        pa[q] += rem >= D ? ta : 0.0f;                                               \
        pb[q] += rem >= D ? tb : 0.0f;                                               \
    }
    NNN_SUFFIX_ROUND(1) NNN_SUFFIX_ROUND(2) NNN_SUFFIX_ROUND(4) NNN_SUFFIX_ROUND(8)
#undef NNN_SUFFIX_ROUND
    const int bnd = lane < NB ? lane : 0;
    const int lo = seg[128 + (bnd >= 1 ? bnd - 1 : 0)], hi = seg[128 + (bnd < NB - 1 ? bnd : 0)];
#pragma unroll
    for (int q = 0; q < NQ; q++) {
        const float fb = wave_read(pb[q], lo), fa = wave_read(pa[q], hi);
        float o = (bnd >= 1 ? fb : 0.0f) + (bnd < NB - 1 ? fa : 0.0f);
        if (bnd == 0 || bnd == NB - 1) o *= 2.0f;
        out[q] = lane < NB ? o : 0.0f;
    }
}

__device__ __forceinline__ float dct_out(const float *x, const float *dct, int i)
{
    float sum = 0.0f;
#pragma unroll
    for (int j = 0; j < NB; j++) sum += x[j] * dct[j * NB + i];
    return (float)((double)sum * 0.30151134457776363 );
}

struct __attribute__((packed, aligned(4))) SamplePair { float x, y; };
__device__ __forceinline__ void window_load(const float *h, int ring, int rb, int lag, int lane, SamplePair (&sm)[8])
{
    int start = rb + (HIST - WINDOW) - lag;
    if (start >= ring) start -= ring;
    const int j = lane < FFT_P1 ? lane : FFT_P1 - 1;
    const unsigned x0 = 4u * (unsigned)(start + 2 * j), ring4 = 4u * (unsigned)ring;
#pragma unroll
    for (int r = 0; r < 8; r++) {
        const unsigned x = x0 + (unsigned)(8 * FFT_P1 * r), y = x - ring4;
        sm[r] = *(const SamplePair *)((const char *)h + (x < y ? x : y));
    }
}
template <bool RL = false>
__device__ __forceinline__ void window_rfft(const Buffers &b, const SamplePair (&sm)[8], const float2 (&w)[8], const FftLds &t,
                                            float2 *Z, float2 (&Y)[8], int lane, bool first)
{
    float2 v[8];
#pragma unroll
    for (int r = 0; r < 8; r++) v[r] = make_float2(sm[r].x * w[r].x, sm[r].y * w[r].y);
    if (first) __syncthreads();
    fft480_regs<RL>(v, Z, t.tw, lane);
    if (RL) lane = launder_v(lane);
    const float wn = b.wnorm;
#pragma unroll
    for (int u = 0; u < 4; u++) {
        const int k = lane + 64 * u;
        if (k <= NFFT / 2) {
            const float2 zk = Z[k], zn = Z[k ? NFFT - k : 0];
            const float2 e = make_float2(zk.x + zn.x, zk.y - zn.y);
            const float2 o = make_float2(zk.y + zn.y, -(zk.x - zn.x));
            const float2 wo = cmulf(o, t.tw[k]);
            Y[u] = make_float2((e.x + wo.x) * wn, (e.y + wo.y) * wn);
            Y[4 + u] = make_float2((e.x - wo.x) * wn, -(e.y - wo.y) * wn);
        }
    }
    wave_lds_sync();
}
__device__ __forceinline__ int rfft_slot_bin(int lane, int u)
{
    const int k = lane + 64 * (u & 3);
    if (u < 4) return k <= NFFT / 2 ? k : -1;
    return k < NFFT / 2 ? NFFT - k : -1;
}

struct XpKeep {
    float2 X[8], P[8];
    float ex, ep, xn;
    int silent;
    int sl;
    float *cnw;
    int *flag;
};
__device__ __forceinline__ void spectrum_store(float2 *row, const float2 (&S)[8], int lane)
{
#pragma unroll
    for (int u = 0; u < 4; u++)
        if (lane + 64 * u <= NFFT / 2) ((float4 *)row)[64 * u + lane] = make_float4(S[u].x, S[u].y, S[4 + u].x, S[4 + u].y);
}
__device__ __forceinline__ void spectrum_load(const float2 *row, float2 (&S)[8], int lane)
{
#pragma unroll
    for (int u = 0; u < 4; u++) {
        const float4 v = lane + 64 * u <= NFFT / 2 ? ((const float4 *)row)[64 * u + lane] : make_float4(0.0f, 0.0f, 0.0f, 0.0f);
        S[u] = make_float2(v.x, v.y);
        S[4 + u] = make_float2(v.z, v.w);
    }
}

constexpr int P_PAIRS0 = 64, P_TAIL = 64 + 2 * 177;
__device__ __forceinline__ void spectrum_store_p(float2 *row, const float2 (&S)[8], int lane, bool taps)
{
    row[lane] = S[0];
    if (taps) row[P_TAIL + lane] = S[4];
#pragma unroll
    for (int u = 1; u < 4; u++)
        if (lane + 64 * u <= NFFT / 2) ((float4 *)(row + P_PAIRS0))[64 * (u - 1) + lane] = make_float4(S[u].x, S[u].y, S[4 + u].x, S[4 + u].y);
}
__device__ __forceinline__ void spectrum_load_p(const float2 *row, float2 (&S)[8], int lane)
{
    S[0] = row[lane];
    S[4] = make_float2(0.0f, 0.0f);
#pragma unroll
    for (int u = 1; u < 4; u++) {
        const float4 v = lane + 64 * u <= NFFT / 2 ? ((const float4 *)(row + P_PAIRS0))[64 * (u - 1) + lane] : make_float4(0.0f, 0.0f, 0.0f, 0.0f);
        S[u] = make_float2(v.x, v.y);
        S[4 + u] = make_float2(v.z, v.w);
    }
}

#ifndef NNN_FH_STRIDE
#define NNN_FH_STRIDE 24
#endif
constexpr int FH_STRIDE = NNN_FH_STRIDE;
static_assert(FH_STRIDE >= NB, "");
template <bool WITH_P, bool FUSED = false, bool XR = false, bool SPECTRA = true>
__device__ __forceinline__ void transform_inputs(const Buffers &b, const StepParams *sp, int tile_in, int sub, FftLds &t, float2 *Z, float *part,
                                                 XpKeep *keep = nullptr)
{
    int tile = tile_in;
    int lane = threadIdx.x & 63;
    int sl = FUSED ? keep->sl : sub * FFT_SPB + (int)(threadIdx.x >> 6), s = tile * TILE + sl;
#define NNN_FUSED_RELAUNDER() do { if (FUSED) { lane = launder_v(lane); tile = launder_s(tile); sl = launder_s(sl); s = tile * TILE + sl; } } while (0)
    const int ring = ring_len(b.nslot), rb = ring_base(sp->slot, b.nslot);
    float2 w[8];
#pragma unroll
    for (int r = 0; r < 8; r++) w[r] = ((const float2 *)b.window_a)[(lane < FFT_P1 ? lane : FFT_P1 - 1) + FFT_P1 * r];
    const int lag = WITH_P ? NNN_TI(b.pitch, 1, tile, sl)[0] : 0;
    if (!FUSED) fft_tables_load(t, b);
    const float *h = b.hist + (size_t)__builtin_amdgcn_readfirstlane(s) * hist_stride(b.nslot);
    SamplePair sx[8], spw[8];
    if (!XR) window_load(h, ring, rb, 0, lane, sx);
    if (WITH_P && !FUSED) window_load(h, ring, rb, lag, lane, spw);
    float2 X[8];
    float2 *dx = b.X + (size_t)s * FSTR;
    if (XR) spectrum_load(dx, X, lane);
    else window_rfft<FUSED>(b, sx, w, t, Z, X, lane, !FUSED);
    if (SPECTRA && !XR && (!FUSED || b.taps)) spectrum_store(dx, X, lane);
    NNN_FUSED_RELAUNDER();
    float *vv = (float *)Z, *vc = vv + BSK_LEN;
    float exv;
    if (XR) {
        exv = lane < NB ? NNN_TI(b.ex, NB, tile, sl)[(size_t)lane * TILE] : 0.0f;
    } else {
#pragma unroll
        for (int u = 0; u < 8; u++) {
            const int k = rfft_slot_bin(lane, u);
            if (k >= 0 && k < 400) vv[bsk(k)] = fmaf(X[u].y, X[u].y, X[u].x * X[u].x);
        }
        wave_lds_sync();
        const float *const v[1] = {vv};
        float o[1];
        band_sums_par<1>(t, v, o, lane);
        exv = o[0];
        if (lane < NB) NNN_TI(b.ex, NB, tile, sl)[(size_t)lane * TILE] = exv;
    }
    if (!WITH_P) return;
    wave_lds_sync();
    NNN_FUSED_RELAUNDER();
    float2 Y[8];
    if (FUSED) window_load(b.hist + (size_t)__builtin_amdgcn_readfirstlane(s) * hist_stride(b.nslot), ring, rb, lag, lane, spw);
    if (FUSED || !SPECTRA) {
#pragma unroll
        for (int r = 0; r < 8; r++) w[r] = ((const float2 *)b.window_a)[(lane < FFT_P1 ? lane : FFT_P1 - 1) + FFT_P1 * r];
    }
    window_rfft<FUSED>(b, spw, w, t, Z, Y, lane, false);
    float2 *dp = b.P + (size_t)s * FSTR;
    if (SPECTRA && (!FUSED || b.taps)) spectrum_store_p(dp, Y, lane, b.taps != 0);
#pragma unroll
    for (int u = 0; u < 8; u++) {
        const int k = rfft_slot_bin(lane, u);
        if (k >= 0 && k < 400) {
            vv[bsk(k)] = fmaf(Y[u].y, Y[u].y, Y[u].x * Y[u].x);
            vc[bsk(k)] = fmaf(X[u].y, Y[u].y, X[u].x * Y[u].x);
        }
    }
    wave_lds_sync();
    NNN_FUSED_RELAUNDER();
    const float *const v[2] = {vv, vc};
    float o[2];
    band_sums_par<2>(t, v, o, lane);
    wave_lds_sync();
    NNN_FUSED_RELAUNDER();
    float *xc = part, *ly = part + FH_STRIDE, *exl = part + 2 * FH_STRIDE;
    float lyv = -2.0f, xnv = 0.0f;
    if (lane < NB) {
        const float xn = o[1] / sqrtf(0.001f + exv * o[0]);
        xnv = xn;
        NNN_TI(b.ep, NB, tile, sl)[(size_t)lane * TILE] = o[0];
        NNN_TI(b.exp_, NB, tile, sl)[(size_t)lane * TILE] = xn;
        xc[lane] = xn;
        exl[lane] = exv;
        lyv = log10f(1e-2f + exv);
    }
    float lfl;
    {
        float pm = lyv;
#pragma unroll
        for (int d = 1; d < 32; d *= 2) {
            const float tt = wave_read(pm, lane - d);
            pm = lane >= d ? fmaxf(pm, tt) : pm;
        }
        float m = fmaxf(fmaxf(lyv, -2.0f - 7.0f), -2.0f - 1.5f * (float)(lane + 1));
#pragma unroll
        for (int d = 1; d <= 4; d++) {
            const float tt = wave_read(lyv, lane - d) - 1.5f * (float)d;
            m = lane >= d ? fmaxf(m, tt) : m;
        }
        const float t5 = wave_read(pm, lane - 5) - 7.0f;
        lfl = lane >= 5 ? fmaxf(m, t5) : m;
    }
    if (lane < NB) ly[lane] = lfl;
    wave_lds_sync();
    if (lane == 0) {
        float e = 0.0f;
#pragma unroll
        for (int i = 0; i < NB; i++) e += exl[i];
        NNN_TI(b.silence, 1, tile, sl)[0] = e < 0.04f ? 1 : 0;
        if (FUSED) keep->flag[0] = e < 0.04f ? 1 : 0;
    }
    {
        const bool second = lane >= 32;
        const int i = second ? lane - 32 : lane;
        if (i < (second ? 6 : NB)) {
            float *cn = NNN_TI(b.cn, 28, tile, sl);
            float c = dct_out(second ? xc : ly, t.dct, i);
            if (second) c -= i == 0 ? 1.3f : (i == 1 ? 0.9f : 0.0f);
            else c -= i == 0 ? 12.0f : (i == 1 ? 4.0f : 0.0f);
            if (FUSED) keep->cnw[(second ? NB : 0) + i] = c;
            else cn[(size_t)((second ? NB : 0) + i) * TILE] = c;
        }
    }
    if (FUSED) {
#pragma unroll
        for (int u = 0; u < 8; u++) { keep->X[u] = X[u]; keep->P[u] = Y[u]; }
        keep->ex = exv;
        keep->ep = o[0];
        keep->xn = xnv;
        wave_lds_sync();
        keep->silent = keep->flag[0];
    }
#undef NNN_FUSED_RELAUNDER
}

#ifndef NNN_FFT_MINWAVES
#define NNN_FFT_MINWAVES 5
#endif
__device__ __forceinline__ void fft_block(const Buffers &b, int g, int &frame, int &tile, int &sub)
{
    xcd_tile_block_units((int)blockIdx.x, b.NT, TILE / FFT_SPB, g, frame, tile, sub);
}
__global__ void __launch_bounds__(64 * FFT_SPB, NNN_FFT_MINWAVES) k_fft_xp(Buffers b, const StepParams *sp, int g)
{
    __shared__ __attribute__((aligned(16))) char tbuf[FFT_TABLES_SHORT];
    FftLds &t = *(FftLds *)tbuf;
    __shared__ float2 Z[FFT_SPB][NFFT_BUF];
    __shared__ float part[FFT_SPB][3 * FH_STRIDE];
    int frame, tile, sub;
    fft_block(b, g, frame, tile, sub);
    if (tile * TILE + sub * FFT_SPB >= b.S) return;
    if (!live_any(b, tile, sub * FFT_SPB, FFT_SPB)) return;
    b = frame_view(b, frame);
    const int wave = threadIdx.x >> 6;
    transform_inputs<true>(b, sp + frame, tile, sub, t, Z[wave], part[wave]);
}
__global__ void __launch_bounds__(64 * FFT_SPB, NNN_FFT_MINWAVES) k_fft_feat(Buffers b, const StepParams *sp, int g)
{
    __shared__ __attribute__((aligned(16))) char tbuf[FFT_TABLES_SHORT];
    FftLds &t = *(FftLds *)tbuf;
    __shared__ float2 Z[FFT_SPB][NFFT_BUF];
    __shared__ float part[FFT_SPB][3 * FH_STRIDE];
    int frame, tile, sub;
    fft_block(b, g, frame, tile, sub);
    if (tile * TILE + sub * FFT_SPB >= b.S) return;
    if (!live_any(b, tile, sub * FFT_SPB, FFT_SPB)) return;
    b = frame_view(b, frame);
    const int wave = threadIdx.x >> 6;
    transform_inputs<true, false, false, false>(b, sp + frame, tile, sub, t, Z[wave], part[wave]);
}

struct XtLds { FftLds t; float2 Z[8][NFFT_BUF]; float part[8][4]; };
template <bool HELD> __device__ __forceinline__ void xt_rider(const Buffers &b, const StepParams *sp, int rb, void *lds)
{
    static_assert(sizeof(XtLds) <= sizeof(PkLds) && PK_T == 512 && FFT_SPB == 4, "");
    XtLds &x = *(XtLds *)lds;
    const int wave = threadIdx.x >> 6;
    if ((rb >> 3) * TILE + 8 * (rb & 7) >= b.S) return;
    if (HELD && !live_any(b, rb >> 3, 16 * ((rb & 7) >> 1), 16)) return;
    transform_inputs<false>(b, sp, rb >> 3, 2 * (rb & 7), x.t, x.Z[wave], x.part[wave]);
}

__global__ void __launch_bounds__(64 * FFT_SPB) k_fft_x(Buffers b, const StepParams *sp, int g)
{
    __shared__ FftLds t;
    __shared__ float2 Z[FFT_SPB][NFFT_BUF];
    __shared__ float part[FFT_SPB][4];
    int frame, tile, sub;
    fft_block(b, g, frame, tile, sub);
    if (tile * TILE + sub * FFT_SPB >= b.S) return;
    b = frame_view(b, frame);
    const int wave = threadIdx.x >> 6;
    transform_inputs<false>(b, sp + frame, tile, sub, t, Z[wave], part[wave]);
}

#pragma clang fp contract(off)

}
```

### nnnoiseless_amd/csrc/nnn_rnn_wf.hip

```cpp
#pragma once

namespace nnn {

constexpr int WF_ROWS = 16, WF_WAVES = 12, WF_FS_W = 72;

struct WfGru {
    f32x4 acc[3][2];
    float zz[4], sold[4];
};
constexpr int WF_KS_REC = 3;
struct WfWeights {
    Frags<2, WF_KS_REC> zr;
    Frags<1, WF_KS_REC> h;
    float bias[3];
};
__device__ __forceinline__ void wf_load_weights(WfWeights &w, const LayerDesc &L, const uint4 *__restrict__ Wq, const float *__restrict__ fpar,
                                                int nbi, int lane)
{
    const uint4 *Brec = Wq + L.rec.wofs + (size_t)nbi * 3 * L.rec.ksteps * 64;
    load_frags<2, 0, WF_KS_REC>(w.zr, L.rec, Brec, lane);
    load_frags<1, 2, WF_KS_REC>(w.h, L.rec, Brec, lane);
    const int neuron = nbi * 16 + (lane & 15);
#pragma unroll
    for (int g = 0; g < 3; g++) w.bias[g] = neuron < L.n ? fpar[L.bias + g * L.n + neuron] : 0.0f;
// ... 83 lines not shown
    const float v1 = (KIND == 0 || KIND == 3) ? r1_l[RB * rm] : 0.0f;
    const float v2 = (KIND == 0 || KIND == 2 || KIND == 3) ? r2_l[RB * rm] : 0.0f;
    const float a = KIND == 0 ? v1 : (KIND == 3 ? -(2.0f * v1) : 0.0f);
    const float c = (KIND == 0 || KIND == 3) ? v2 : (KIND == 2 ? -v2 : 0.0f);
    float v = (v0 + a) + c;
    v = silent ? 0.0f : v;
    if (b.taps) NNN_TIF(b, feat, NFEAT, f, tile, trow)[(size_t)(KB + part) * TILE] = v;
    store_split(fs_l, rm * WF_FS_W, KB, v);
}

__device__ __forceinline__ void wf_features(const Buffers &b, const WfFeatIn &in, int f, int tile, int r0, int lane, float *crs, float *dc,
                                            float *cnb, unsigned short *FS, int *live_f, int &mem_id)
{
    constexpr int rm = WF_ROWS;
    const int row = lane & 15, part = lane >> 4, trow = r0 + row;
    const int pitch = in.pitch;
    const bool silent = in.silent != 0;
    NNN_STAMPW(b, 8, f == 3);
#pragma unroll
    for (int i = 0; i < 7; i++) cnb[(7 * part + i) * rm + row] = in.mine[i];
    wave_lds_sync();
    if (part == 0) live_f[row] = silent ? 0 : 1;
    const int c0 = mem_id, c1 = mem_id < 1 ? CEPS_MEM + mem_id - 1 : mem_id - 1;
    const int c2 = mem_id < 2 ? CEPS_MEM + mem_id - 2 : mem_id - 2;
    NNN_STAMPW(b, 9, f == 3);
    if (!silent) {
        float *cm = NNN_TI(b.ceps_mem, CEPS_MEM * NB, tile, trow);
        for (int k = part; k < NB; k += 4) {
            const float v = cnb[k * rm + row];
            cm[(size_t)(c0 * NB + k) * TILE] = v;
            crs[(c0 * NB + k) * rm + row] = v;
        }
        mem_id = mem_id + 1 == CEPS_MEM ? 0 : mem_id + 1;
        NNN_STAMPW(b, 10, f == 3);
        const int ia = part, ib = part + 4 < CEPS_MEM - 1 ? part + 4 : part;
        const int ja = ia < c0 ? ia : ia + 1, jb = ib < c0 ? ib : ib + 1;
        const float *ra = crs + (ja * NB) * rm + row, *rb = crs + (jb * NB) * rm + row, *nw = cnb + row;
        float da = 0.0f, db = 0.0f;
#pragma unroll
        for (int k = 0; k < NB; k++) {
            const float x = nw[k * rm];
            const float ea = x - ra[k * rm], eb = x - rb[k * rm];
            da += ea * ea;
            db += eb * eb;
        }
        dc[pair_index(ja < c0 ? ja : c0, ja < c0 ? c0 : ja) * rm + row] = da;
        if (part + 4 < CEPS_MEM - 1) dc[pair_index(jb < c0 ? jb : c0, jb < c0 ? c0 : jb) * rm + row] = db;
    }
    NNN_STAMPW(b, 11, f == 3);
    wave_lds_sync();
    {
        const float *cnb_l = cnb + part * rm + row;
        const float *r1_l = crs + (c1 * NB + part) * rm + row, *r2_l = crs + (c2 * NB + part) * rm + row;
        unsigned short *fs_l = FS + row * WF_FS_W + part;
        wf_feature_outputs<0, 0, 0, 0, false>(b, f, tile, trow, part, silent, cnb_l, r1_l, r2_l, fs_l);
        wf_feature_outputs<0, 4, 4, 4, true>(b, f, tile, trow, part, silent, cnb_l, r1_l, r2_l, fs_l);
        wf_feature_outputs<1, 6, 6, 0, false>(b, f, tile, trow, part, silent, cnb_l, r1_l, r2_l, fs_l);
        wf_feature_outputs<1, 10, 10, 0, false>(b, f, tile, trow, part, silent, cnb_l, r1_l, r2_l, fs_l);
        wf_feature_outputs<1, 14, 14, 0, false>(b, f, tile, trow, part, silent, cnb_l, r1_l, r2_l, fs_l);
        wf_feature_outputs<1, 18, 18, 0, false>(b, f, tile, trow, part, silent, cnb_l, r1_l, r2_l, fs_l);
        wf_feature_outputs<2, NB, 0, 0, false>(b, f, tile, trow, part, silent, cnb_l, r1_l, r2_l, fs_l);
        wf_feature_outputs<2, NB + 4, 4, 4, true>(b, f, tile, trow, part, silent, cnb_l, r1_l, r2_l, fs_l);
        wf_feature_outputs<3, NB + 6, 0, 0, false>(b, f, tile, trow, part, silent, cnb_l, r1_l, r2_l, fs_l);
        wf_feature_outputs<3, NB + 10, 4, 4, true>(b, f, tile, trow, part, silent, cnb_l, r1_l, r2_l, fs_l);
        wf_feature_outputs<1, NB + 12, NB, 0, false>(b, f, tile, trow, part, silent, cnb_l, r1_l, r2_l, fs_l);
        wf_feature_outputs<1, NB + 16, NB + 4, 0, true>(b, f, tile, trow, part, silent, cnb_l, r1_l, r2_l, fs_l);
    }
    NNN_STAMPW(b, 12, f == 3);
    if (part < 2) {
        float v = part == 0 ? 0.01f * ((float)pitch - 300.0f) : spectral_variability(dc, row, rm);
        v = silent ? 0.0f : v;
        if (b.taps) NNN_TIF(b, feat, NFEAT, f, tile, trow)[(size_t)(40 + part) * TILE] = v;
        store_split(FS, rm * WF_FS_W, row * WF_FS_W + 40 + part, v);
    }
    NNN_STAMPW(b, 13, f == 3);
}

template <int KS> struct WfDenseW {
    Frags<1, KS> fr;
    float bias;
};
template <int KS>
__device__ __forceinline__ void wf_dense_load(WfDenseW<KS> &w, const LayerDesc &L, const uint4 *__restrict__ Wq, const float *__restrict__ fpar,
                                              int nbi, int lane)
{
    load_frags<1, 0, KS>(w.fr, L.in, Wq + L.in.wofs + (size_t)nbi * L.in.ksteps * 64, lane);
    const int neuron = nbi * 16 + (lane & 15);
    w.bias = neuron < L.n ? fpar[L.bias + neuron] : 0.0f;
}
template <bool QUAD = false, int KS, class Sink>
__device__ __forceinline__ void wf_dense(const LayerDesc &L, const unsigned short *Ain, int in_w, const uint4 *__restrict__ Wq, const WfDenseW<KS> &w,
                                         const float *tab, int nbi, int lane, Sink &&sink)
{
    const int neuron = nbi * 16 + (lane & 15);
    const uint4 *Bnb = Wq + L.in.wofs + (size_t)nbi * L.in.ksteps * 64;
    f32x4 acc[3][2];
    acc[0][0] = f32x4{w.bias, w.bias, w.bias, w.bias};
    gemm_acc<1, 1, 0, KS>(acc, Ain, WF_ROWS * in_w, in_w, 0, L.in, Bnb, lane, w.fr);
    if (neuron < L.n) {
        if constexpr (QUAD) {
            float v[4];
#pragma unroll
            for (int q = 0; q < 4; q++) v[q] = activate(L.act, acc[0][0][q] * (1.0f / 256.0f), tab);
            sink(4 * (lane >> 4), neuron, v);
        } else {
#pragma unroll
            for (int q = 0; q < 4; q++) sink(4 * (lane >> 4) + q, neuron, activate(L.act, acc[0][0][q] * (1.0f / 256.0f), tab));
        }
    }
}

#ifndef NNN_WF_MINWAVES
#define NNN_WF_MINWAVES 3
#endif
struct WfPlan {
    int w_v, w_n, w_dn;
    int sw_v, sw_n, sw_dn;
};

__host__ __device__ constexpr WfPlan wf_plan_of(const RnnPlan &pl)
{
    return WfPlan{32 * pl.vad.in.ksteps + 8, 32 * pl.noise.in.ksteps + 8, 32 * pl.dn.in.ksteps + 8,
                  rnn_state_w(pl.vad), rnn_state_w(pl.noise), rnn_state_w(pl.dn)};
}
struct WfLds { int tab, live, Xv, Xn, Xdn, SPv, SPn, SPdn, RSv, RSn, RSdn, FS, crs, dc, cnb, total; };
__host__ __device__ constexpr WfLds wf_lds(const WfPlan &w)
{
    constexpr int plane3 = 3 * WF_ROWS * 2;
    WfLds o{};
    int at = 0;
    o.tab = lds_take(at, 256 * 4);
    o.live = lds_take(at, 8 * WF_ROWS * 4);
    o.Xv = lds_take(at, plane3 * w.w_v);
    o.Xn = lds_take(at, 2 * plane3 * w.w_n);
    o.Xdn = lds_take(at, 3 * plane3 * w.w_dn);
    o.SPv = lds_take(at, plane3 * w.sw_v);
    o.SPn = lds_take(at, plane3 * w.sw_n);
    o.SPdn = lds_take(at, plane3 * w.sw_dn);
    o.RSv = lds_take(at, plane3 * w.sw_v);
    o.RSn = lds_take(at, plane3 * w.sw_n);
    o.RSdn = lds_take(at, plane3 * w.sw_dn);
    o.FS = lds_take(at, plane3 * WF_FS_W);
    o.crs = lds_take(at, CEPS_MEM * NB * WF_ROWS * 4);
    o.dc = lds_take(at, 28 * WF_ROWS * 4);
    o.cnb = lds_take(at, 28 * WF_ROWS * 4);
    o.total = at;
    return o;
}
static_assert(wf_lds(wf_plan_of(BkShapeBuiltin::plan())).total == 127744, "k_rnn_wf's LDS for the built-in shape class");
struct WfShapeAny { static constexpr bool fixed = false; };
template <class SH> struct WfFixed { static constexpr bool value = true; };
template <> struct WfFixed<WfShapeAny> { static constexpr bool value = false; };
template <class SH>
__global__ void __launch_bounds__(64 * WF_WAVES, NNN_WF_MINWAVES) k_rnn_wf(Buffers b, RnnPlan pl_rt, WfPlan wp_rt, const uint4 *__restrict__ Wq,
                                                            const float *__restrict__ fpar, int tile0, int g)
{
    RnnPlan pl = pl_rt;
    WfPlan wp = wp_rt;
    if constexpr (WfFixed<SH>::value) {
        constexpr RnnPlan p0 = SH::plan();
        constexpr WfPlan w0 = wf_plan_of(p0);
        pl = p0;
        pl.dense.act = pl_rt.dense.act; pl.vad.act = pl_rt.vad.act; pl.noise.act = pl_rt.noise.act; pl.dn.act = pl_rt.dn.act;
        pl.out.act = pl_rt.out.act; pl.act_vo = pl_rt.act_vo;
        wp = w0;
    }
    HIP_DYNAMIC_SHARED(float, lds_raw)
    constexpr int rm = WF_ROWS;
    const int wave0 = __builtin_amdgcn_readfirstlane((int)(threadIdx.x >> 6));
    const int lane0 = threadIdx.x & 63;
    int wave = wave0, lane = lane0;
    int tile, r0;
    if (!rnn_block_rows(b, tile0, rm, tile, r0)) return;
    if (!live_any(b, tile, r0, rm)) return;
    const bool rowl = lane0 < rm;
    const int trow = r0 + (rowl ? lane0 : 0);
    NNN_STAMP(b, 50);
    const WfLds o = wf_lds(wp);
    auto planes = [&](int at) { return (unsigned short *)(lds_raw + at / 4); };
    float *tab = lds_raw + o.tab / 4;
    int *live = (int *)(lds_raw + o.live / 4);
    unsigned short *Xv = planes(o.Xv), *Xn = planes(o.Xn), *Xdn = planes(o.Xdn);
    unsigned short *SPv = planes(o.SPv), *SPn = planes(o.SPn), *SPdn = planes(o.SPdn);
    unsigned short *RSv = planes(o.RSv), *RSn = planes(o.RSn), *RSdn = planes(o.RSdn);
    unsigned short *FS = planes(o.FS);
    float *crs = lds_raw + o.crs / 4, *dc = lds_raw + o.dc / 4, *cnb = lds_raw + o.cnb / 4;
    const int cD = pl.dense.out_col, cV = pl.cV, cF = pl.cF;
    float *sv = b.gru_v + ((size_t)tile * TILE * b.gru_v_w + (size_t)r0 * pl.vad.n),
          *sn = b.gru_n + ((size_t)tile * TILE * b.gru_n_w + (size_t)r0 * pl.noise.n),
          *sdn = b.gru_dn + ((size_t)tile * TILE * b.gru_dn_w + (size_t)r0 * pl.dn.n);
    {
        uint4 *z = (uint4 *)Xv;
        const int n16 = (int)(((char *)crs - (char *)Xv) / 16);
        for (int i = (int)threadIdx.x; i < n16; i += 64 * WF_WAVES) z[i] = make_uint4(0u, 0u, 0u, 0u);
        for (int i = (int)threadIdx.x; i < 201; i += 64 * WF_WAVES) tab[i] = b.tansig[i];
        const float *cm = NNN_TI(b.ceps_mem, CEPS_MEM * NB, tile, trow);
        constexpr int PER = (CEPS_MEM * NB + WF_WAVES - 1) / WF_WAVES;
        float stg[PER];
#pragma unroll
        for (int i = 0; i < PER; i++) {
            const int r = wave + i * WF_WAVES;
            stg[i] = (rowl && r < CEPS_MEM * NB) ? cm[(size_t)r * TILE] : 0.0f;
        }
#pragma unroll
        for (int i = 0; i < PER; i++) {
            const int r = wave + i * WF_WAVES;
            if (rowl && r < CEPS_MEM * NB) crs[r * rm + lane] = stg[i];
        }
    }
    lds_barrier();
    constexpr int T = 64 * WF_WAVES;
    gru_state_io<T>(pl.vad, rm, sv, SPv, wp.sw_v, true);
    gru_state_io<T>(pl.noise, rm, sn, SPn, wp.sw_n, true);
    gru_state_io<T>(pl.dn, rm, sdn, SPdn, wp.sw_dn, true);
    if (rowl)
        for (int p = wave; p < 28; p += WF_WAVES) dc[p * rm + lane] = pair_dist(crs, p, lane, rm);
    int mem_id = wave == WF_WAVES - 1 ? NNN_TI(b.mem_id, 1, tile, r0 + (lane & 15))[0] : 0;
    const int W_N = 6, W_V = 9, W_F = 11;
    WfWeights wts;
    if (wave < W_N) wf_load_weights(wts, pl.dn, Wq, fpar, wave < pl.dn.nb ? wave : 0, lane);
    else if (wave < W_V) wf_load_weights(wts, pl.noise, Wq, fpar, wave - W_N < pl.noise.nb ? wave - W_N : 0, lane);
    else if (wave < W_F) wf_load_weights(wts, pl.vad, Wq, fpar, wave - W_V < pl.vad.nb ? wave - W_V : 0, lane);
    else wf_load_weights(wts, pl.vad, Wq, fpar, 0, lane);
    lds_barrier();
    NNN_STAMP(b, 51);
    WfGru ua;
    if (wave == WF_WAVES - 1 && g > 0) wf_features_load(wts, b, 0, tile, r0, lane);
    if (wave0 == WF_WAVES - 1) wf_setprio_high();
    for (int t = -1; t < g + 3; t++) {
        lane = launder_v(lane0);
        wave = launder_s(wave0);
        const int fv = t, fn = t - 1, fd = t - 2, fo = t - 3, ff = t + 1;
        const bool on_v = fv >= 0 && fv < g, on_n = fn >= 0 && fn < g, on_d = fd >= 0 && fd < g, on_o = fo >= 0 && fo < g,
                   on_f = ff >= 0 && ff < g;
        unsigned short *Xn_n = Xn + (fn & 1) * 3 * rm * wp.w_n;
        unsigned short *Xdn_d = Xdn + ((fd + 3) % 3) * 3 * rm * wp.w_dn;
        const int srole = wave0 == 0 ? 0 : (wave0 == 6 ? 1 : (wave0 == 9 ? 2 : (wave0 == 11 ? 3 : -1)));
        NNN_STAMPW(b, 30 + 5 * srole, t == 2 && srole >= 0);
        if (wave < W_N) {
            if (on_d && wave < pl.dn.nb) wf_gru_a(pl.dn, Xdn_d, wp.w_dn, SPdn, RSdn, wp.sw_dn, Wq, wts, tab, wave, lane, ua);
        } else if (wave < W_V) {
            if (on_n && wave - W_N < pl.noise.nb) wf_gru_a(pl.noise, Xn_n - cV, wp.w_n, SPn, RSn, wp.sw_n, Wq, wts, tab, wave - W_N, lane, ua);
        } else if (wave < W_F) {
            WfDenseW<3> dw;
            const bool mine_o = on_o && wave - W_V < pl.out.nb;
            if (on_v && wave - W_V < pl.vad.nb) wf_gru_a(pl.vad, Xv - cD, wp.w_v, SPv, RSv, wp.sw_v, Wq, wts, tab, wave - W_V, lane, ua);
            if (mine_o) {
                const int *lv = live + 16 * (fo & 7);
                wf_dense_load(dw, pl.out, Wq, fpar, wave - W_V, lane);
                wf_dense<true>(pl.out, SPdn, wp.sw_dn, Wq, dw, tab, wave - W_V, lane, [&](int lrow, int band, const float (&v)[4]) {
                    if (b.link) {
                        rnn_gain_out4(b, fo, tile, r0 + lrow, band, lv + lrow, v);
                    } else {
#pragma unroll
                        for (int q = 0; q < 4; q++) rnn_gain_out(b, fo, tile, r0 + lrow + q, band, lv[lrow + q] != 0, v[q]);
                    }
                });
            }
        } else {
            if (on_f) wf_features(b, wf_features_in(wts), ff, tile, r0, lane, crs, dc, cnb, FS, live + 16 * (ff & 7), mem_id);
            if (ff + 1 >= 0 && ff + 1 < g) wf_features_load(wts, b, ff + 1, tile, r0, lane);
        }
        NNN_STAMPW(b, 31 + 5 * srole, t == 2 && srole >= 0);
#if defined(NNN_STAMPS) && NNN_WFSTAMP_PHASE == 1
        NNN_STAMPW(b, 14 + wave0, t == 2);
#endif
        lds_barrier();
        NNN_STAMPW(b, 32 + 5 * srole, t == 2 && srole >= 0);
        if (wave < W_N) {
            WfDenseW<2> dw;
            const bool mine_d = on_f && wave < pl.dense.nb;
            if (on_d && wave < pl.dn.nb)
                wf_gru_b(pl.dn, RSdn, wp.sw_dn, Wq, wts, tab, live + 16 * (fd & 7), wave, lane, ua,
                         [&](int row, int n, float v) { store_split(SPdn, rm * wp.sw_dn, row * wp.sw_dn + n, v); });
            if (mine_d) {
                unsigned short *Xnn = Xn + (ff & 1) * 3 * rm * wp.w_n;
                wf_dense_load(dw, pl.dense, Wq, fpar, wave, lane);
                wf_dense(pl.dense, FS - cF, WF_FS_W, Wq, dw, tab, wave, lane, [&](int row, int n, float v) {
                    store_split(Xv, rm * wp.w_v, row * wp.w_v + n, v);
                    store_split(Xnn, rm * wp.w_n, row * wp.w_n + (cD - cV) + n, v);
                });
            }
        } else if (wave < W_V) {
            if (on_n && wave - W_N < pl.noise.nb) {
                unsigned short *Xd = Xdn + (fn % 3) * 3 * rm * wp.w_dn;
                wf_gru_b(pl.noise, RSn, wp.sw_n, Wq, wts, tab, live + 16 * (fn & 7), wave - W_N, lane, ua, [&](int row, int n, float v) {
                    store_split(SPn, rm * wp.sw_n, row * wp.sw_n + n, v);
                    store_split(Xd, rm * wp.w_dn, row * wp.w_dn + n, v);
                });
            }
            if (on_f) {
                unsigned short *Xnn = Xn + (ff & 1) * 3 * rm * wp.w_n, *Xd = Xdn + (ff % 3) * 3 * rm * wp.w_dn;
                for (int i = 64 * (wave - W_N) + lane; i < 3 * rm * 6; i += 64 * (W_V - W_N)) {
                    const int plx = i / (rm * 6), rem = i - plx * rm * 6, row = rem / 6, c8 = rem - row * 6;
                    const uint4 v = *(const uint4 *)(FS + (size_t)plx * rm * WF_FS_W + row * WF_FS_W + 8 * c8);
                    *(uint4 *)(Xnn + (size_t)plx * rm * wp.w_n + row * wp.w_n + (cF - cV) + 8 * c8) = v;
                    *(uint4 *)(Xd + (size_t)plx * rm * wp.w_dn + row * wp.w_dn + cF + 8 * c8) = v;
                }
            }
        } else if (wave < W_F) {
            if (on_v && wave - W_V < pl.vad.nb) {
                unsigned short *Xnn = Xn + (fv & 1) * 3 * rm * wp.w_n, *Xd = Xdn + (fv % 3) * 3 * rm * wp.w_dn;
                wf_gru_b(pl.vad, RSv, wp.sw_v, Wq, wts, tab, live + 16 * (fv & 7), wave - W_V, lane, ua, [&](int row, int n, float v) {
                    store_split(SPv, rm * wp.sw_v, row * wp.sw_v + n, v);
                    store_split(Xnn, rm * wp.w_n, row * wp.w_n + n, v);
                    store_split(Xd, rm * wp.w_dn, row * wp.w_dn + cV + n, v);
                });
            }
        } else {
            if (on_n && rowl) {
                const unsigned short *Xv1 = Xn + (fn & 1) * 3 * rm * wp.w_n;
                NNN_TIF(b, vad, 1, fn, tile, trow)[0] = rnn_vad_out(pl, fpar, Xv1, rm * wp.w_n, wp.w_n, 0, lane, live + 16 * (fn & 7), tab);
            }
        }
        NNN_STAMPW(b, 33 + 5 * srole, t == 2 && srole >= 0);
#if defined(NNN_STAMPS) && NNN_WFSTAMP_PHASE == 2
        NNN_STAMPW(b, 14 + wave0, t == 2);
#endif
        lds_barrier();
        NNN_STAMPW(b, 34 + 5 * srole, t == 2 && srole >= 0);
    }
    gru_state_io<T>(pl.vad, rm, sv, SPv, wp.sw_v, false);
    gru_state_io<T>(pl.noise, rm, sn, SPn, wp.sw_n, false);
    gru_state_io<T>(pl.dn, rm, sdn, SPdn, wp.sw_dn, false);
    if (wave0 == WF_WAVES - 1 && rowl) NNN_TI(b.mem_id, 1, tile, trow)[0] = mem_id;
    NNN_STAMP(b, 52);
}

}
```

Before: 76.27 million frames/s.

## Run spectrum FFT as a persistent kernel beside the RNN on its own stream

Adds a new schedule stage ST_XT that computes the input-window FFT spectra for the next group in a persistent, grid-capped kernel (k_fft_xg) on a fifth HIP stream. It is sized in LDS and VGPRs so its blocks can co-reside on a CU with a k_rnn_wf block. The later fft_xp pass then reads the precomputed X spectra (k_fft_xp_xr) instead of recomputing them. The built-in k_rnn_wf is capped at 152 VGPRs so the two kernels can share CUs, and build.py now checks register and scratch use from compiler remarks. This adds cross-stream event dependencies and may cause spills or contention with the RNN kernel.

```diff
diff --git a/include/nnn_batch.h b/include/nnn_batch.h
--- a/include/nnn_batch.h
+++ b/include/nnn_batch.h
@@ -158,6 +158,7 @@
 int nnn_batch_set_inputs_ready(nnn_batch *b, int on);
 int nnn_batch_set_back_end(nnn_batch *b, int mode);
 int nnn_batch_set_schedule(nnn_batch *b, int mode, int lanes);
+int nnn_batch_set_x_beside(nnn_batch *b, int mode);
 
 int nnn_debug_activations(int device, int act, const float *x, float *y, int n);
 
diff --git a/nnnoiseless_amd/__init__.py b/nnnoiseless_amd/__init__.py
--- a/nnnoiseless_amd/__init__.py
+++ b/nnnoiseless_amd/__init__.py
@@ -224,6 +224,9 @@
     def set_taps(self, on):
         self._lib.check(self._lib.L.nnn_batch_set_taps(self._h, int(on)))
 
+    def set_x_beside(self, mode):
+        self._lib.check(self._lib.L.nnn_batch_set_x_beside(self._h, int(mode)))
+
     def set_schedule(self, mode, lanes=0):
         self._lib.check(self._lib.L.nnn_batch_set_schedule(self._h, {"seq": 0, "lanes": 1, "stages": 2}[mode], int(lanes)))
 
diff --git a/nnnoiseless_amd/_ffi.py b/nnnoiseless_amd/_ffi.py
--- a/nnnoiseless_amd/_ffi.py
+++ b/nnnoiseless_amd/_ffi.py
@@ -24,7 +24,7 @@
     "nnn_batch_analyze_device", "nnn_batch_synthesize_device", "nnn_batch_analyze_host", "nnn_batch_synthesize_host", "nnn_batch_pending_frames",
     "nnn_batch_vad_device", "nnn_batch_vad_host", "nnn_batch_network_device", "nnn_batch_network_host",
     "nnn_batch_set_gain_floor", "nnn_batch_get_gain_floor", "nnn_batch_num_floored",
-    "nnn_batch_set_channel_link", "nnn_batch_get_channel_link",
+    "nnn_batch_set_channel_link", "nnn_batch_get_channel_link", "nnn_batch_set_x_beside",
 ]
 TRAIN_SYMBOLS = [
     "nnn_train_create", "nnn_train_destroy", "nnn_train_reset", "nnn_train_process_device", "nnn_train_process_host",
@@ -214,7 +214,8 @@
                          ("nnn_batch_debug_schedule", [vp, i32, C.POINTER(C.c_int32), sz]),
                          ("nnn_batch_debug_host_plan", [vp, i32, C.POINTER(PcmLayout), i32, C.POINTER(C.c_int64)]),
                          ("nnn_batch_create_opts", [C.POINTER(vp), C.POINTER(i32), i32, i32, C.POINTER(BatchOpts)]),
-                         ("nnn_batch_max_group_frames", [vp]), ("nnn_batch_device_bytes", [vp]), ("nnn_batch_set_back_end", [vp, i32])):
+                         ("nnn_batch_max_group_frames", [vp]), ("nnn_batch_device_bytes", [vp]), ("nnn_batch_set_back_end", [vp, i32]),
+                         ("nnn_batch_set_x_beside", [vp, i32])):
             if hasattr(L, name):
                 getattr(L, name).argtypes = at
         if hasattr(L, "nnn_batch_create_opts"):
diff --git a/nnnoiseless_amd/build.py b/nnnoiseless_amd/build.py
--- a/nnnoiseless_amd/build.py
+++ b/nnnoiseless_amd/build.py
@@ -1,5 +1,7 @@
 import os
+import re
 import subprocess
+import sys
 
 HERE = os.path.dirname(os.path.abspath(__file__))
 CSRC = os.path.join(HERE, "csrc")
@@ -9,6 +11,34 @@
 WEIGHTS = os.path.join(HERE, "data", "weights.rnn")
 SOURCES = ["nnn_batch.hip", "nnn_resample.hip", "nnn_model.cpp", "rnnoise_capi.cpp", "nnn_node.cpp"]
 HP_SOURCE = "nnn_hp.hip"
+REGISTER_LIMITS = {"8k_fft_xgE": 56, "8k_rnn_wfINS_14BkShapeBuiltinEEE": 152}
+
+
+def _without_remarks(text):
+    out, held = [], []
+    for line in text.splitlines(True):
+        if line.startswith("In file included from"):
+            held.append(line)
+            continue
+        if "[-Rpass-analysis=kernel-resource-usage]" not in line:
+            out += held + [line]
+        held = []
+    return "".join(out + held)
+
+
+def _check_registers(remarks):
+    use = {}
+    for blk in re.split(r"Function Name: ", remarks)[1:]:
+        name = blk.split()[0]
+        f = lambda key: int(re.search(re.escape(key) + r":\s*(\d+)", blk).group(1))
+        use[name] = (f(" VGPRs") + f(" AGPRs"), f("ScratchSize [bytes/lane]"))
+    for frag, limit in REGISTER_LIMITS.items():
+        hits = [(n, u) for n, u in use.items() if frag in n]
+        if not hits:
+            raise RuntimeError(f"no resource remark for a kernel named *{frag}*: the register check cannot be made")
+        for n, (regs, scratch) in hits:
+            if regs > limit or scratch:
+                raise RuntimeError(f"{n}: {regs} registers per wave (at most {limit}), {scratch} bytes of scratch (none allowed)")
 
 
 def _stale():
@@ -30,13 +60,18 @@
     hp_obj = os.path.join(LIB_DIR, f"nnn_hp.{os.getpid()}.o")
     tmp_lib = os.path.join(LIB_DIR, f"libnnnoiseless_mi355x.{os.getpid()}.so")
     cmds = [common + ["-DNNN_HP_UNIT", "-Wno-pragma-once-outside-header", "-c", "-x", "hip", os.path.join(CSRC, HP_SOURCE), "-o", hp_obj],
-            common + ["-fno-slp-vectorize", "-DNNN_HP_EXTERN", "-shared", "-x", "hip"] + [os.path.join(CSRC, s) for s in SOURCES]
+            common + ["-fno-slp-vectorize", "-DNNN_HP_EXTERN", "-Rpass-analysis=kernel-resource-usage", "-fno-caret-diagnostics", "-shared", "-x", "hip"] + [os.path.join(CSRC, s) for s in SOURCES]
             + ["-x", "none", hp_obj, "-o", tmp_lib]]
     try:
         for cmd in cmds:
             if verbose:
                 print(" ".join(cmd))
-            subprocess.check_call(cmd)
+            r = subprocess.run(cmd, stderr=subprocess.PIPE, text=True)
+            sys.stderr.write(_without_remarks(r.stderr))
+            if r.returncode:
+                raise subprocess.CalledProcessError(r.returncode, cmd)
+            if "-Rpass-analysis=kernel-resource-usage" in cmd:
+                _check_registers(r.stderr)
         os.replace(tmp_lib, LIB_PATH)
     finally:
         for f in (hp_obj, tmp_lib):
diff --git a/nnnoiseless_amd/csrc/nnn_batch_core.hip b/nnnoiseless_amd/csrc/nnn_batch_core.hip
--- a/nnnoiseless_amd/csrc/nnn_batch_core.hip
+++ b/nnnoiseless_amd/csrc/nnn_batch_core.hip
@@ -54,7 +54,8 @@
 enum KernelId { K_HP, K_LPC, K_PITCH, K_FFT_XP, K_RNN, K_SYNTH, K_BACK, K_COUNT };
 static const char *kKernelNames[K_COUNT] = {"k_hp", "k_lpc", "k_pitch", "k_fft_xp", "k_rnn", "k_synth", "k_back"};
 
-enum Stage { ST_HP, ST_PITCH, ST_FFT, ST_RNN, ST_SYN, ST_COUNT };
+enum Stage { ST_HP, ST_PITCH, ST_FFT, ST_RNN, ST_SYN, ST_XT, ST_COUNT };
+constexpr int XT_STREAM = 4;
 enum SplitStage { ST_FEAT = ST_COUNT, ST_GAINS, ST_FFT_FEAT, ST_VAD };
 struct SplitIo {
     float *features = nullptr;
@@ -63,6 +64,7 @@
     const float *vad = nullptr;
 };
 constexpr int NSTREAMS = 5;
+static_assert(XT_STREAM == NSTREAMS - 1, "stages: pool[0..3]; lanes: pool[0] and pool[1 .. n_lanes - 1], n_lanes <= NSTREAMS - 1");
 constexpr int EVR = 16;
 enum SchedMode { SCHED_SEQ = 0, SCHED_LANES = 1, SCHED_STAGES = 2 };
 constexpr int AUTO_BIG = 16384;
@@ -80,6 +82,7 @@
     int pitch_chain = 1;
     int hp_tpb = 0;
     int x_rides = -1;
+    int x_beside = 0;
     int lpc_wide = -1;
     int lpc_fc = 0;
     int back_mode = -1;
@@ -96,6 +99,7 @@
     if (const char *e = knob("NNN_LPC_HEAD")) p.lpc_head = atoi(e);
     if (const char *e = dev_knob("NNN_X_RIDES")) p.x_rides = atoi(e);
     if (const char *e = knob("NNN_PITCH_CHAIN")) p.pitch_chain = atoi(e);
+    if (const char *e = dev_knob("NNN_X_BESIDE")) p.x_beside = atoi(e);
     if (const char *e = dev_knob("NNN_LPC_WIDE")) p.lpc_wide = atoi(e);
     if (const char *e = dev_knob("NNN_LPC_FC")) p.lpc_fc = atoi(e);
     if (const char *e = knob("NNN_SCHED")) {
@@ -130,6 +134,7 @@
     int lpc_fc = 0;
     bool chain = false;
     bool riders = false;
+    bool xr = false;
     uint8_t *rnn = nullptr;
 };
 
@@ -176,6 +181,7 @@
     std::vector<int> group_streams;
     int device = 0;
     int S = 0, S_pad = 0, NT = 0;
+    int n_cu = 0;
     uint64_t frame_count = 0;
     int depth = 1;
     int gmax = GROUP;
diff --git a/nnnoiseless_amd/csrc/nnn_batch_create.hip b/nnnoiseless_amd/csrc/nnn_batch_create.hip
--- a/nnnoiseless_amd/csrc/nnn_batch_create.hip
+++ b/nnnoiseless_amd/csrc/nnn_batch_create.hip
@@ -141,6 +141,11 @@
     if (device >= MARK_DEVICES) return fail("device %d: the library keeps per-device call marks for devices 0 .. %d only", device, MARK_DEVICES - 1);
     HIPCHK(hipSetDevice(device));
     h->device = device;
+#ifdef __HIPCC__
+    HIPCHK(hipDeviceGetAttribute(&h->n_cu, hipDeviceAttributeMultiprocessorCount, device));
+#else
+    h->n_cu = 8;
+#endif
     return 0;
 }
 static int create_streams_and_events(nnn_batch *h)
diff --git a/nnnoiseless_amd/csrc/nnn_batch_debug.hip b/nnnoiseless_amd/csrc/nnn_batch_debug.hip
--- a/nnnoiseless_amd/csrc/nnn_batch_debug.hip
+++ b/nnnoiseless_amd/csrc/nnn_batch_debug.hip
@@ -217,6 +217,13 @@
     h->paths.back_mode = mode;
     return 0;
 }
+extern "C" int nnn_batch_set_x_beside(nnn_batch *h, int mode)
+{
+    if (!h) return fail("null batch");
+    if (mode < -1 || mode > 1) return fail("unknown x-beside mode %d", mode);
+    h->paths.x_beside = mode;
+    return 0;
+}
 extern "C" int nnn_batch_set_pipeline(nnn_batch *h, int on)
 {
     if (!h) return fail("null batch");
diff --git a/nnnoiseless_amd/csrc/nnn_batch_launch.hip b/nnnoiseless_amd/csrc/nnn_batch_launch.hip
--- a/nnnoiseless_amd/csrc/nnn_batch_launch.hip
+++ b/nnnoiseless_amd/csrc/nnn_batch_launch.hip
@@ -39,15 +39,23 @@
     return pc > 0 && g > 1 && (pc > 1 || (unsigned)h->S_pad / PK_SPB < 1024u);
 }
 
+static BackEnd plan_back(const nnn_batch *h, int g)
+{
+    const Paths &k = h->paths;
+    const int m = k.back_mode >= 0 ? k.back_mode : g > 1 ? 0 : ((h->S_pad <= 8192 && !h->beside_others) ? 1 : 3);
+    const bool fused = m == 1 || m == 2, all_g = m == 2 || m == 4;
+    BackEnd back = m == 0 || (g > 1 && !all_g) ? BACK_UNFUSED : (fused ? BACK_FUSED : BACK_RNN_ALONE);
+    for (const nnn_batch::ModelGroup &G : h->groups)
+        if ((fused ? G.back_lds : G.rnn16_lds) == 0) back = BACK_UNFUSED;
+    return back;
+}
+
 static void plan_group(const nnn_batch *h, int g, GroupPlan &p)
 {
     const Paths &k = h->paths;
     p.g = g;
-    const int m = k.back_mode >= 0 ? k.back_mode : g > 1 ? 0 : ((h->S_pad <= 8192 && !h->beside_others) ? 1 : 3);
-    const bool fused = m == 1 || m == 2, all_g = m == 2 || m == 4;
-    p.back = m == 0 || (g > 1 && !all_g) ? BACK_UNFUSED : (fused ? BACK_FUSED : BACK_RNN_ALONE);
-    for (const nnn_batch::ModelGroup &G : h->groups)
-        if ((fused ? G.back_lds : G.rnn16_lds) == 0) p.back = BACK_UNFUSED;
+    p.xr = false;
+    p.back = plan_back(h, g);
     const bool split = k.hp_split >= 0 ? k.hp_split != 0 : h->NT <= 256;
     p.hp = !split ? 0 : ((k.hp_tpb ? k.hp_tpb == 2 : (g > 1 && h->NT >= 8)) ? 2 : 1);
     p.floor = h->n_floored > 0;
@@ -132,8 +140,14 @@
                 L.go(K_BACK, kBackFused[p.riders][p.held][p.floor][p.link], dim3((unsigned)(G.ntiles * (TILE / BK_ROWS))), dim3(BK_T), G.back_lds, b, sp0, G.acts, G.wq, G.fpar, G.tile0, g);
             break;
         }
-        L.go(K_FFT_XP, k_fft_xp, dim3(Sp * ug / FFT_SPB), dim3(64 * FFT_SPB), 0, b, sp0, g);
-        break;
+        L.go(K_FFT_XP, p.xr ? k_fft_xp_xr : k_fft_xp, dim3(Sp * ug / FFT_SPB), dim3(64 * FFT_SPB), 0, b, sp0, g);
+        break;
+    case ST_XT: {
+        unsigned grid = Sp / FFT_SPB < (unsigned)h->n_cu ? Sp / FFT_SPB : (unsigned)h->n_cu;
+        if (grid > 8) grid &= ~7u;
+        L.go(K_FFT_XP, k_fft_xg, dim3(grid), dim3(64 * FFT_SPB), 0, b, sp0, g);
+        break;
+    }
     case ST_RNN:
         if (p.back == BACK_FUSED) break;
         for (size_t i = 0; i < h->groups.size(); i++) {
@@ -195,6 +209,7 @@
     int sched, lanes;
     bool fold_fill, early_hp, hp_after;
     bool idle;
+    int x_from;
 };
 static CallPlan plan_call(const nnn_batch *h, int n_frames, hipStream_t st)
 {
@@ -217,6 +232,10 @@
     c.fold_fill = (!c.pipe && !h->profiling) || c.idle;
     c.early_hp = c.pipe && k.inputs_ready && !h->host_call && h->prev_pipe && h->prev_st == st && c.sched == SCHED_LANES && h->pool[0];
     c.hp_after = c.sched == SCHED_LANES && c.lanes == 1 && h->S_pad >= 8192;
+    bool builtin = !h->groups.empty();
+    for (const nnn_batch::ModelGroup &G : h->groups) builtin &= G.wf && G.shape_builtin;
+    const bool x_beside = !c.idle && (k.x_beside >= 0 ? k.x_beside != 0 : (c.pipe && h->S_pad > AUTO_BIG && builtin));
+    c.x_from = !x_beside ? (int)c.sizes.size() : (k.x_beside > 0 ? 0 : 1);
     return c;
 }
 
@@ -248,14 +267,19 @@
     sc.fill = cp.early_hp ? FILL_POOL0 : (cp.fold_fill ? FILL_FOLDED : FILL_CALLER);
     sc.fill_after_done = cp.early_hp && h->have_done[par];
     if (cp.idle) return sc;
+    auto has_x = [&](int k) { return k >= cp.x_from && k < n_groups && plan_back(h, cp.sizes[k]) != BACK_FUSED; };
     auto stream_of = [&](int s, int k) -> int {
         if (!cp.pipe) return -1;
+        if (s == ST_XT) return XT_STREAM;
         if (cp.sched == SCHED_STAGES) return s == ST_HP ? 0 : (s == ST_PITCH ? 1 : (s == ST_FFT ? 2 : (s == ST_RNN ? 3 : -1)));
         return s == ST_HP ? 0 : (k % cp.lanes) - (k % cp.lanes == 0 ? 1 : 0);
     };
     auto consumers_elsewhere = [&](int s, int k) {
         const int me = stream_of(s, k);
-        if (s + 1 < ST_COUNT && stream_of(s + 1, k) != me) return true;
+        if (s == ST_XT) return stream_of(ST_FFT, k) != me;
+        if (s + 1 <= ST_SYN && stream_of(s + 1, k) != me) return true;
+        if (s == ST_HP && has_x(k) && stream_of(ST_XT, k) != me) return true;
+        if (s == ST_FFT && has_x(k + 1) && stream_of(ST_XT, k + 1) != me) return true;
         if ((s == ST_HP || s == ST_PITCH || s == ST_RNN || s == ST_SYN) && k + 1 < n_groups && stream_of(s, k + 1) != me) return true;
         if (s == ST_SYN) return true;
         if (cp.hp_after && s == ST_PITCH) return true;
@@ -264,9 +288,13 @@
     bool used[NSTREAMS] = {cp.early_hp};
     const int pn = (int)h->prev_first.size();
     sc.nodes.reserve((size_t)n_groups * ST_COUNT);
+    std::vector<int> first_of((size_t)n_groups);
+    static const int order[ST_COUNT] = {ST_HP, ST_XT, ST_PITCH, ST_FFT, ST_RNN, ST_SYN};
     for (int k = 0, t = 0; k < n_groups; t += cp.sizes[k++]) {
         const int g = cp.sizes[k];
-        for (int s = 0; s < ST_COUNT; s++) {
+        first_of[(size_t)k] = t;
+        for (int s : order) {
+            if (s == ST_XT && !has_x(k)) continue;
             Node n = {};
             const int si = stream_of(s, k);
             n.stage = s, n.group = k, n.frames = g, n.first = t, n.stream = si;
@@ -279,9 +307,14 @@
                 if (dk < 0 || dk < k - EVR + 1) return;
                 if (stream_of(ds, dk) != si) wait(W_THIS, ds, dk);
             };
-            if (s > 0) wait_for(s - 1, k);
+            if (s > 0 && s != ST_XT) wait_for(s - 1, k);
             if (s == ST_HP || s == ST_PITCH || s == ST_RNN || s == ST_SYN) wait_for(s, k - 1);
-            if (s == ST_PITCH) wait_for(ST_SYN, k - h->depth);
+            if (s == ST_PITCH || s == ST_XT) wait_for(ST_SYN, k - h->depth);
+            if (s == ST_XT) {
+                wait_for(ST_HP, k);
+                if (cp.pipe) wait_for(ST_FFT, k - 1);
+            }
+            if (s == ST_FFT && has_x(k)) wait_for(ST_XT, k);
             if (s == ST_HP && cp.hp_after) {
                 if (k > 0) wait_for(ST_PITCH, k - 1);
                 else if (cp.early_hp && pn > 0) wait(W_PREV, ST_PITCH, pn - 1);
@@ -290,7 +323,7 @@
                 const int need = t + g - 1 + 3 - h->nslot;
                 int dk = -1;
                 for (int j = 0; j < k; j++)
-                    if (sc.nodes[(size_t)j * ST_COUNT].first <= need) dk = j;
+                    if (first_of[(size_t)j] <= need) dk = j;
                 wait_for(ST_SYN, dk);
                 if (cp.early_hp && need < 0) {
                     const long long pf = (long long)h->frame_count + need - (long long)h->prev_frame0;
@@ -375,6 +408,7 @@
     for (int k = 0; k < n_groups; k++) {
         const int g = cp.sizes[k], set0 = (int)(h->group_count % h->depth) * h->gmax;
         plan_group(h, g, h->plan);
+        for (size_t j = i; j < sc.nodes.size() && sc.nodes[j].group == k; j++) h->plan.xr |= sc.nodes[j].stage == ST_XT;
         for (; i < sc.nodes.size() && sc.nodes[i].group == k; i++) {
             const Node &n = sc.nodes[i];
             if (n.stream >= 0 && !h->pool[n.stream]) ok &= hipStreamCreateWithFlags(&h->pool[n.stream], hipStreamNonBlocking) == hipSuccess;
@@ -395,7 +429,7 @@
         h->prev_frame0 = frame0;
         h->prev_par = par;
         h->prev_first.clear();
-        for (int k = 0; k < n_groups; k++) h->prev_first.push_back(sc.nodes[(size_t)k * ST_COUNT].first);
+        for (int k = 0, t = 0; k < n_groups; t += cp.sizes[k++]) h->prev_first.push_back(t);
     }
     ok &= hipEventRecord(h->ev_done[par], st) == hipSuccess;
     h->have_done[par] = true;
diff --git a/nnnoiseless_amd/csrc/nnn_fft.hip b/nnnoiseless_amd/csrc/nnn_fft.hip
--- a/nnnoiseless_amd/csrc/nnn_fft.hip
+++ b/nnnoiseless_amd/csrc/nnn_fft.hip
@@ -373,12 +373,13 @@
 #endif
 constexpr int FH_STRIDE = NNN_FH_STRIDE;
 static_assert(FH_STRIDE >= NB, "");
-template <bool WITH_P, bool FUSED = false, bool XR = false, bool SPECTRA = true>
+template <bool WITH_P, bool FUSED = false, bool XR = false, bool SPECTRA = true, bool TABLES = true>
 __device__ __forceinline__ void transform_inputs(const Buffers &b, const StepParams *sp, int tile_in, int sub, FftLds &t, float2 *Z, float *part,
                                                  XpKeep *keep = nullptr)
 {
     int tile = tile_in;
     int lane = threadIdx.x & 63;
+    if constexpr (!TABLES) lane = launder_v(lane);
     int sl = FUSED ? keep->sl : sub * FFT_SPB + (int)(threadIdx.x >> 6), s = tile * TILE + sl;
 #define NNN_FUSED_RELAUNDER() do { if (FUSED) { lane = launder_v(lane); tile = launder_s(tile); sl = launder_s(sl); s = tile * TILE + sl; } } while (0)
     const int ring = ring_len(b.nslot), rb = ring_base(sp->slot, b.nslot);
@@ -386,7 +387,7 @@
 #pragma unroll
     for (int r = 0; r < 8; r++) w[r] = ((const float2 *)b.window_a)[(lane < FFT_P1 ? lane : FFT_P1 - 1) + FFT_P1 * r];
     const int lag = WITH_P ? NNN_TI(b.pitch, 1, tile, sl)[0] : 0;
-    if (!FUSED) fft_tables_load(t, b);
+    if (!FUSED && TABLES) fft_tables_load(t, b);
     const float *h = b.hist + (size_t)__builtin_amdgcn_readfirstlane(s) * hist_stride(b.nslot);
     SamplePair sx[8], spw[8];
     if (!XR) window_load(h, ring, rb, 0, lane, sx);
@@ -394,7 +395,7 @@
     float2 X[8];
     float2 *dx = b.X + (size_t)s * FSTR;
     if (XR) spectrum_load(dx, X, lane);
-    else window_rfft<FUSED>(b, sx, w, t, Z, X, lane, !FUSED);
+    else window_rfft<FUSED>(b, sx, w, t, Z, X, lane, !FUSED && TABLES);
     if (SPECTRA && !XR && (!FUSED || b.taps)) spectrum_store(dx, X, lane);
     NNN_FUSED_RELAUNDER();
     float *vv = (float *)Z, *vc = vv + BSK_LEN;
@@ -423,7 +424,7 @@
 #pragma unroll
         for (int r = 0; r < 8; r++) w[r] = ((const float2 *)b.window_a)[(lane < FFT_P1 ? lane : FFT_P1 - 1) + FFT_P1 * r];
     }
-    window_rfft<FUSED>(b, spw, w, t, Z, Y, lane, false);
+    window_rfft<FUSED>(b, spw, w, t, Z, Y, lane, XR && !FUSED && TABLES);
     float2 *dp = b.P + (size_t)s * FSTR;
     if (SPECTRA && (!FUSED || b.taps)) spectrum_store_p(dp, Y, lane, b.taps != 0);
 #pragma unroll
@@ -523,6 +524,20 @@
     const int wave = threadIdx.x >> 6;
     transform_inputs<true>(b, sp + frame, tile, sub, t, Z[wave], part[wave]);
 }
+__global__ void __launch_bounds__(64 * FFT_SPB, NNN_FFT_MINWAVES) k_fft_xp_xr(Buffers b, const StepParams *sp, int g)
+{
+    __shared__ __attribute__((aligned(16))) char tbuf[FFT_TABLES_SHORT];
+    FftLds &t = *(FftLds *)tbuf;
+    __shared__ float2 Z[FFT_SPB][NFFT_BUF];
+    __shared__ float part[FFT_SPB][3 * FH_STRIDE];
+    int frame, tile, sub;
+    fft_block(b, g, frame, tile, sub);
+    if (tile * TILE + sub * FFT_SPB >= b.S) return;
+    if (!live_any(b, tile, sub * FFT_SPB, FFT_SPB)) return;
+    b = frame_view(b, frame);
+    const int wave = threadIdx.x >> 6;
+    transform_inputs<true, false, true>(b, sp + frame, tile, sub, t, Z[wave], part[wave]);
+}
 __global__ void __launch_bounds__(64 * FFT_SPB, NNN_FFT_MINWAVES) k_fft_feat(Buffers b, const StepParams *sp, int g)
 {
     __shared__ __attribute__((aligned(16))) char tbuf[FFT_TABLES_SHORT];
@@ -562,6 +577,35 @@
     transform_inputs<false>(b, sp + frame, tile, sub, t, Z[wave], part[wave]);
 }
 
+constexpr int XG_LDS = FFT_TABLES_SHORT + FFT_SPB * NFFT_BUF * (int)sizeof(float2);
+constexpr int XG_LDS_MAX = 163840 - 127744, XG_VGPR_MAX = 56;
+static_assert(XG_LDS <= XG_LDS_MAX, "k_fft_xg must fit beside a k_rnn_wf block");
+#ifdef __HIPCC__
+#define NNN_XG_VGPR_CAP __attribute__((amdgpu_num_vgpr(XG_VGPR_MAX / 2)))
+#else
+#define NNN_XG_VGPR_CAP
+#endif
+__global__ void __launch_bounds__(64 * FFT_SPB) NNN_XG_VGPR_CAP k_fft_xg(Buffers b, const StepParams *sp, int g)
+{
+    __shared__ __attribute__((aligned(16))) char tbuf[FFT_TABLES_SHORT];
+    FftLds &t = *(FftLds *)tbuf;
+    __shared__ float2 Z[FFT_SPB][NFFT_BUF];
+    fft_tables_load(t, b);
+    __syncthreads();
+    const int wave = threadIdx.x >> 6;
+    const int nq = b.NT * (TILE / FFT_SPB);
+    for (int q = (int)blockIdx.x; q < nq; q += (int)gridDim.x) {
+        int tile, sub;
+        xcd_tile_block(q, b.NT, TILE / FFT_SPB, tile, sub);
+        if (tile * TILE + sub * FFT_SPB >= b.S) continue;
+        if (!live_any(b, tile, sub * FFT_SPB, FFT_SPB)) continue;
+        for (int f = 0; f < g; f++) {
+            transform_inputs<false, false, false, true, false>(frame_view(b, f), sp + f, tile, sub, t, Z[wave], nullptr);
+            wave_lds_sync();
+        }
+    }
+}
+
 #pragma clang fp contract(off)
 
 }
diff --git a/nnnoiseless_amd/csrc/nnn_rnn_wf.hip b/nnnoiseless_amd/csrc/nnn_rnn_wf.hip
--- a/nnnoiseless_amd/csrc/nnn_rnn_wf.hip
+++ b/nnnoiseless_amd/csrc/nnn_rnn_wf.hip
@@ -259,8 +259,7 @@
 template <class SH> struct WfFixed { static constexpr bool value = true; };
 template <> struct WfFixed<WfShapeAny> { static constexpr bool value = false; };
 template <class SH>
-__global__ void __launch_bounds__(64 * WF_WAVES, NNN_WF_MINWAVES) k_rnn_wf(Buffers b, RnnPlan pl_rt, WfPlan wp_rt, const uint4 *__restrict__ Wq,
-                                                            const float *__restrict__ fpar, int tile0, int g)
+__device__ __forceinline__ void rnn_wf(Buffers b, RnnPlan pl_rt, WfPlan wp_rt, const uint4 *__restrict__ Wq, const float *__restrict__ fpar, int tile0, int g)
 {
     RnnPlan pl = pl_rt;
     WfPlan wp = wp_rt;
@@ -433,5 +432,23 @@
     if (wave0 == WF_WAVES - 1 && rowl) NNN_TI(b.mem_id, 1, tile, trow)[0] = mem_id;
     NNN_STAMP(b, 52);
 }
-
-}
+template <class SH>
+__global__ void __launch_bounds__(64 * WF_WAVES, NNN_WF_MINWAVES) k_rnn_wf(Buffers b, RnnPlan pl_rt, WfPlan wp_rt, const uint4 *__restrict__ Wq,
+                                                            const float *__restrict__ fpar, int tile0, int g)
+{
+    rnn_wf<SH>(b, pl_rt, wp_rt, Wq, fpar, tile0, g);
+}
+#ifdef __HIPCC__
+#define NNN_WF_VGPR_CAP __attribute__((amdgpu_num_vgpr(76)))
+#else
+#define NNN_WF_VGPR_CAP
+#endif
+constexpr int WF_BUILTIN_VGPR_MAX = 152;
+template <>
+__global__ void __launch_bounds__(64 * WF_WAVES, NNN_WF_MINWAVES) NNN_WF_VGPR_CAP k_rnn_wf<BkShapeBuiltin>(Buffers b, RnnPlan pl_rt, WfPlan wp_rt, const uint4 *__restrict__ Wq,
+                                                                                            const float *__restrict__ fpar, int tile0, int g)
+{
+    rnn_wf<BkShapeBuiltin>(b, pl_rt, wp_rt, Wq, fpar, tile0, g);
+}
+
+}
```

Result: no change. 75.73 million frames/s (-0.7%).
